# FireflyRenderEngine/GPUPathTracer

Hardware: AMD Instinct MI355X
Metric: Mrays/s (path segments = closest-hit queries, device-counted) at 1080p, 8 bounces, 1024 spp (higher is better)
Workload: dtype f32; 1 GPU; C2 wahoo.obj+cube.obj Cornell box (5184 triangles, 6 planes), 1920x1080, 8 bounces, 1024 spp, camera=inside, trace=bvh, seed 1234; scene=c2, rays_per_frame=11019120206, rays_untraversed=2123366400, rays_cut_last=721266356, primary_hits_kept_between_frames=False, partition=1080-row strips round-robin over 1 rank(s), gather=none

## Files before the change

gpupathtracer_amd/csrc/ff_api.cpp:

```cpp
#include <algorithm>
#include <chrono>
#include <cmath>
#include <cstdio>
#include <cstdlib>
#include <cstring>
#include <new>
#include <vector>

#include <hip/hip_runtime.h>
#include <hip/hip_gl_interop.h>

#include "ff_state.h"

using namespace ff;

namespace {

void free_scene(FfState* s)
{
    s->primary_valid = s->last_key_valid = false;
    if (s->d_geoms) (void)hipFree(s->d_geoms);
    if (s->d_tris) (void)hipFree(s->d_tris);
    if (s->d_normals) (void)hipFree(s->d_normals);
    if (s->d_uvs) (void)hipFree(s->d_uvs);
    if (s->d_nodes) (void)hipFree(s->d_nodes);
    if (s->d_nodes4) (void)hipFree(s->d_nodes4);
    s->top_count = s->top_depth = 0;
    s->num_scan = 0;
    if (s->d_parent) (void)hipFree(s->d_parent);
    if (s->d_role) (void)hipFree(s->d_role);
    s->d_nodes4 = nullptr;
    s->num_nodes4 = s->max_depth4 = 0;
    s->scene_block_threads = s->lds_cap = 0;
    s->d_geoms = nullptr;
    s->d_tris = nullptr;
    s->d_normals = nullptr;
    s->d_uvs = nullptr;
    s->d_nodes = nullptr;
    s->d_parent = nullptr;
    s->d_role = nullptr;
    s->h_geoms.clear();
    s->slots.clear();
    s->node_capacity = 0;
    s->has_scene = false;
    s->num_geoms = s->num_nodes = s->max_depth = 0;
    s->num_tris = 0;
}

hipError_t scene_alloc(FfState* s, void** ptr, size_t bytes)
{
    if (s->alloc_countdown >= 0 && s->alloc_countdown-- == 0) {
        *ptr = nullptr;
        return hipErrorOutOfMemory;
    }
    return hipMalloc(ptr, bytes);
}

}

namespace ff {

int ensure_bytes(void** ptr, size_t* cap, size_t need)
{
    if (*cap >= need && *ptr) return FF_OK;
    if (*ptr) (void)hipFree(*ptr);
    *ptr = nullptr;
    *cap = 0;
    hipError_t e = hipMalloc(ptr, need);
    if (e != hipSuccess) return fail(e == hipErrorOutOfMemory ? FF_ERR_OOM : FF_ERR_HIP, "hipMalloc(%zu) failed: %s", need, hipGetErrorString(e));
    *cap = need;
    return FF_OK;
}

int map_pbo(FfState* s, size_t need_bytes, void** out_ptr)
{
    size_t nbytes = 0;
    FF_HIP(hipGraphicsMapResources(1, &s->pbo_resource, s->stream));
    hipError_t e = hipGraphicsResourceGetMappedPointer(out_ptr, &nbytes, s->pbo_resource);
    if (e == hipSuccess && nbytes < need_bytes) e = hipErrorInvalidValue;
    if (e == hipSuccess) return FF_OK;
    const int st = fail(FF_ERR_HIP, "mapping the pixel buffer failed: %s", hipGetErrorString(e));
    (void)hipGraphicsUnmapResources(1, &s->pbo_resource, s->stream);
    return st;
}

int unmap_pbo(FfState* s, int status)
{
    const hipError_t ue = hipGraphicsUnmapResources(1, &s->pbo_resource, s->stream);
    if (status == FF_OK && ue != hipSuccess) return fail(FF_ERR_HIP, "hipGraphicsUnmapResources failed: %s", hipGetErrorString(ue));
    return status;
}

}

namespace {

int check_params(const FfRenderParams* p)
{
    if (!p) return fail(FF_ERR_INVALID_ARG, "render params are null");
    if (p->width <= 0 || p->height <= 0) return fail(FF_ERR_INVALID_ARG, "image size %dx%d is invalid", p->width, p->height);
    if (p->width > 65535 || p->height > 65535) return fail(FF_ERR_INVALID_ARG, "image size %dx%d exceeds 65535 per side", p->width, p->height);
    if (p->bounces < 1 || p->bounces > 255) return fail(FF_ERR_INVALID_ARG, "bounces must be in 1..255 (got %d)", p->bounces);
    if (p->spp < 1 || p->spp >= (1 << 24)) return fail(FF_ERR_INVALID_ARG, "spp must be in 1..2^24-1 (got %d)", p->spp);
    if (p->trace_mode != FF_TRACE_BRUTE_FORCE && p->trace_mode != FF_TRACE_BVH) return fail(FF_ERR_INVALID_ARG, "unknown trace_mode %d", p->trace_mode);
    if (p->shade_mode != FF_SHADE_NORMAL_DEBUG && p->shade_mode != FF_SHADE_DIFFUSE_PATH && p->shade_mode != FF_SHADE_DIFFUSE_PATH_SMOOTH &&
        p->shade_mode != FF_SHADE_DIFFUSE_PATH_NEE) return fail(FF_ERR_INVALID_ARG, "unknown shade_mode %d", p->shade_mode);
    if (p->grid_mode != FF_GRID_FULL && p->grid_mode != FF_GRID_REFERENCE_FLOOR) return fail(FF_ERR_INVALID_ARG, "unknown grid_mode %d", p->grid_mode);
    if (p->spp_per_launch < 0) return fail(FF_ERR_INVALID_ARG, "spp_per_launch must be >= 0");
    return FF_OK;
}

}

extern "C" int ff_check_render_params(const FfRenderParams* params)
{
    clear_error();
    return check_params(params);
}

namespace ff {

int check_render_call(const FfState* s, const FfCamera* camera, const FfRenderParams* params, const char* who)
{
    if (!s) return fail(FF_ERR_INVALID_ARG, "%s: state is null", who);
    if (!camera) return fail(FF_ERR_INVALID_ARG, "%s: camera is null", who);
    const int st = check_params(params);
    if (st != FF_OK) return st;
    if (!s->has_scene) return fail(FF_ERR_NO_SCENE, "%s: no scene uploaded", who);
    return FF_OK;
}

}

namespace {

int lds_records(const FfState* s) { return s->num_geoms > kMaxLdsRecords ? 0 : s->num_geoms; }

int bvh_block_threads(const FfState* s, int preferred, int stack_levels)
{
    const int sizes[3] = { 1024, 768, 512 };
    for (int b : sizes) {
        if (b > preferred) continue;
        if (bvh_lds_bytes(0, stack_levels, b, lds_records(s)) + (s->use_pool ? pool_lds_bytes(b) : 0) <= (size_t)kLdsBudgetBytes) return b;
    }
    return 0;
}

int finalize_layout(FfState* s)
{
    int nodes4 = 0, depth4 = 0;
    for (size_t i = 0; i < s->slots.size(); ++i) {
        if (s->h_geoms[i].type != FF_GEOM_TRIANGLEMESH || s->slots[i].node4_count == 0) continue;
        nodes4 += s->slots[i].node4_count;
        depth4 = std::max(depth4, s->slots[i].depth4);
    }
    s->num_nodes4 = nodes4;
    s->max_depth4 = depth4;
    s->top_count = s->top_depth = 0;
    if (s->num_geoms > kChunkGeometries) {
        std::vector<BvhNode> top2;
        std::vector<Bvh4Node> top4;
        s->num_scan = s->sw.no_scan_planes ? 0 : count_scan_planes(s->h_geoms, s->num_quads);
        build_geometry_tree(s->h_geoms, top2, s->num_scan);
        s->top_depth = collapse_geometry_tree(top2, top4);
        s->top_count = (int)top4.size();
        if (top4.size() > (size_t)s->num_geoms) return fail(FF_ERR_HIP, "geometry tree of %zu nodes for %d geometries", top4.size(), s->num_geoms);
        FF_HIP(hipMemcpyAsync(s->d_nodes4 + s->node_capacity, top4.data(), top4.size() * sizeof(Bvh4Node), hipMemcpyHostToDevice, s->stream));
        FF_HIP(hipStreamSynchronize(s->stream));
    }
    build_wall_table(s->h_geoms.data(), s->sw.no_wall_table ? 0 : (s->num_geoms > kChunkGeometries ? s->num_scan : s->num_quads), s->walls, !s->sw.no_wall_pairs);
    if (s->num_geoms <= kChunkGeometries) add_mesh_boxes(s->h_geoms.data(), s->num_planes, s->num_geoms, s->walls);
    s->stack_entries = depth4 + 1 + (s->top_depth > 0 ? s->top_depth + 1 : 0);
    if (!s->setup_threshold_forced) {
        int biggest = 1;
        for (size_t i = 0; i < s->slots.size(); ++i) biggest = std::max(biggest, s->slots[i].node4_count);
        s->setup_threshold = std::max(4, std::min(24, (int)std::lround(1.5 * std::log((double)biggest) / std::log(4.0) - 0.7)));
        s->setup_threshold = std::min(32, s->setup_threshold + 2 * s->top_depth);
    }
    s->use_pool = s->sw.pool > 0 && s->num_geoms <= kChunkGeometries && nodes4 > 0;
    constexpr int kPoolStackLevels = 5;
    const int pool_levels = std::min(s->stack_entries, s->sw.pool_stack_levels > 0 ? s->sw.pool_stack_levels : kPoolStackLevels);
    s->scene_block_threads = bvh_block_threads(s, s->block_threads, s->use_pool ? pool_levels : s->stack_entries);
    if (s->use_pool && s->scene_block_threads != 1024) {
        s->use_pool = false;
        s->scene_block_threads = bvh_block_threads(s, s->block_threads, s->stack_entries);
    }
    const int block = s->scene_block_threads > 0 ? s->scene_block_threads : kBlockThreads;
    constexpr int kMinLdsStack = 4;
    const size_t reserve = s->use_pool ? pool_lds_bytes(block) : 0;
    s->stack_lds_levels = s->stack_entries;
    if (s->use_pool) {
        s->stack_lds_levels = pool_levels;
        while (s->stack_lds_levels < s->stack_entries && max_lds_nodes(s->stack_lds_levels + 1, block, lds_records(s), reserve) >= nodes4) ++s->stack_lds_levels;
    } else if (s->scene_block_threads > 0 && !s->sw.no_stack_spill) {
        const int want = nodes4 + s->top_count;
        if (want > max_lds_nodes(s->stack_entries, block, lds_records(s))) {
            int levels = s->stack_entries;
            while (levels > kMinLdsStack && max_lds_nodes(levels, block, lds_records(s)) < want) --levels;
            if (max_lds_nodes(levels, block, lds_records(s)) >= want) s->stack_lds_levels = levels;
        }
    }
    int cap = s->scene_block_threads > 0 ? std::max(0, max_lds_nodes(s->stack_lds_levels, block, lds_records(s), reserve)) : 0;
    if (s->sw.lds_node_cap >= 0) cap = std::min(cap, s->sw.lds_node_cap);
    s->lds_cap = std::min(cap, nodes4 + s->top_count);
    s->top_lds_count = std::min(s->top_count, cap);
    const int mesh_cap = cap - s->top_lds_count;
    constexpr int kSmallTree = 8;
    std::vector<int> share(s->h_geoms.size(), 0);
    int left = mesh_cap, wanting = 0;
    for (size_t i = 0; i < s->h_geoms.size(); ++i) {
        if (s->h_geoms[i].type != FF_GEOM_TRIANGLEMESH || s->slots[i].node4_count == 0) continue;
        share[i] = std::min(std::min(s->slots[i].node4_count, kSmallTree), left);
        left -= share[i];
        wanting += s->slots[i].node4_count - share[i];
    }
    const int pool = left;
    for (size_t i = 0; i < s->h_geoms.size() && wanting > 0; ++i) {
        if (s->h_geoms[i].type != FF_GEOM_TRIANGLEMESH || s->slots[i].node4_count == 0) continue;
        const int want = s->slots[i].node4_count - share[i];
        share[i] += wanting <= pool ? want : (int)((int64_t)pool * want / wanting);
    }
    int next = s->top_lds_count;
    for (size_t i = 0; i < s->h_geoms.size(); ++i) {
        GeomRecord& r = s->h_geoms[i];
        r.node4_first = 0;
        r.lds_nodes = 0;
        r.wmin[3] = 0.0f;
        if (r.type != FF_GEOM_TRIANGLEMESH || s->slots[i].node4_count == 0) continue;
        r.node4_first = s->slots[i].node_first;
        r.lds_nodes = std::min(s->slots[i].node4_count, share[i]);
        std::memcpy(&r.wmin[3], &next, sizeof(int));
        next += r.lds_nodes;
    }
    FF_HIP(hipMemcpyAsync(s->d_geoms, s->h_geoms.data(), s->h_geoms.size() * sizeof(GeomRecord), hipMemcpyHostToDevice, s->stream));
    FF_HIP(hipStreamSynchronize(s->stream));
    return FF_OK;
}

int collapse_slot(FfState* s, size_t gi, bool with_info)
{
    FfState::MeshSlot& slot = s->slots[gi];
    if (slot.node_count <= 0) return FF_OK;
    int st = FF_OK;
    if (!slot.parents_linked) {
        st = gpu_link_parents(s->stream, s->d_nodes, slot.node_first, slot.node_count, s->d_parent + slot.node_first);
        if (st != FF_OK) return st;
        slot.parents_linked = true;
    }
    Collapse4Info info;
    st = gpu_collapse_mesh(s->stream, s->scratch, s->d_nodes, slot.node_first, slot.node_count, s->d_parent + slot.node_first, s->d_nodes4, slot.node_first, s->d_role + slot.node_first,
                           with_info ? &info : nullptr);
    if (st != FF_OK) return st;
    if (with_info) {
        if (info.node_count >= (1 << 22)) return fail(FF_ERR_UNSUPPORTED, "a mesh's tree has %d 4-wide nodes; the traversal stack encodes at most %d", info.node_count, (1 << 22) - 1);
        slot.node4_count = info.node_count;
        slot.depth4 = info.depth;
    }
    return FF_OK;
}

int fill_frame_mapping(const FfState* s, KParams& k, const FfCamera* camera, int W, int H, int grid_mode, int strip_rows, int part, int num_parts,
                       int local_rows, int x0, int y0, int win_w, int num_blocks, const char* who)
{
    FfMat4 cm;
    ff_camera_ray_matrix_jittered(camera, s->jitter_x, s->jitter_y, &cm);
    std::memcpy(k.cam_c0, &cm.m[0], 16);
    std::memcpy(k.cam_c1, &cm.m[4], 16);
    std::memcpy(k.cam_c2, &cm.m[8], 16);
    std::memcpy(k.cam_c3, &cm.m[12], 16);
    k.cam_pos[0] = camera->m_position.x;
    k.cam_pos[1] = camera->m_position.y;
    k.cam_pos[2] = camera->m_position.z;
    k.far_clip = camera->m_farClip;
    k.screen_w = camera->m_screenWidth;
    k.screen_h = camera->m_screenHeight;
    k.width = W;
    k.height = H;
    k.xlim = W;
    k.ylim = H;
    if (grid_mode == FF_GRID_REFERENCE_FLOOR) {
        k.xlim = (W / 16) * 16;
        k.ylim = (H / 16) * 16;
    }
    k.strip_rows = strip_rows;
    k.part = part;
    k.num_parts = num_parts;
    k.local_rows = local_rows;
    k.x0 = x0;
    k.y0 = y0;
    k.local_width = win_w;
    k.tiles_per_row = (win_w + 7) / 8;
    const uint64_t tiles = (uint64_t)k.tiles_per_row * (uint64_t)((local_rows + 7) / 8);
    if (tiles * 64 * (uint64_t)(num_blocks + 64) >= (1ull << 31)) return fail(FF_ERR_INVALID_ARG, "%simage too large for the work queue", who);
    k.pix_items = (unsigned)(tiles * 64);
    return FF_OK;
}

void fill_scene(const FfState* s, KParams& k, bool smooth, int lds_block_threads)
{
    k.setup_threshold = s->setup_threshold;
    k.leaf_threshold = s->leaf_threshold;
    k.num_geoms = s->num_geoms;
    k.num_planes = s->num_planes;
    k.num_quads = s->num_quads;
    k.has_specular = s->has_specular ? 1 : 0;
    k.geoms = s->d_geoms;
    k.tris = s->d_tris;
    k.trinormals = smooth ? reinterpret_cast<const float4*>(s->d_normals) : nullptr;
    k.nodes4 = s->d_nodes4;
    if (s->sw.lds_fill && lds_block_threads > 0) {
        const size_t bytes = bvh_lds_bytes(s->lds_cap, s->stack_lds_levels, lds_block_threads, lds_records(s));
        k.debug_lds_words = (unsigned)std::min<size_t>(s->sw.lds_fill_words, bytes / 4);
        k.debug_lds_pattern = (unsigned)s->sw.lds_fill_pattern;
    }
    k.stack_depth = s->stack_lds_levels;
    k.stack_spill = nullptr;
    k.lds_nodes = s->lds_cap;
    k.top_first = (int)s->node_capacity;
    k.top_lds_first = 0;
    k.top_lds_count = s->top_lds_count;
    k.num_scan = s->num_scan;
    k.walls = s->walls;
}

int attach_stack_spill(FfState* s, KParams& k, int grid, int block_threads)
{
    if (s->stack_lds_levels >= s->stack_entries) return FF_OK;
    const int st = ensure_bytes((void**)&s->d_stack_spill, &s->stack_spill_bytes,
                                (size_t)(s->stack_entries - s->stack_lds_levels) * (size_t)grid * (size_t)block_threads * sizeof(int));
    if (st == FF_OK) k.stack_spill = s->d_stack_spill;
    return st;
}

void size_work_queue(const FfState* s, KParams& k, int grid, int block_threads, int tail_per_wave)
{
    k.queue_counters = std::min(kQueueCountersDefault, grid);
    if (s->sw.queue_counters > 0) k.queue_counters = std::min(std::min(kQueueCounters, grid), s->sw.queue_counters);
    const int waves_per_counter = (grid * (block_threads / 64) + k.queue_counters - 1) / k.queue_counters;
    k.queue_tail_items = (unsigned)(waves_per_counter * (s->sw.queue_tail >= 0 ? s->sw.queue_tail : tail_per_wave));
}

FfState::PrimaryKey primary_key(const KParams& k, bool smooth)
{
    FfState::PrimaryKey key;
    std::memset(&key, 0, sizeof key);
    std::memcpy(key.cam, k.cam_c0, 16 * sizeof(float));
    std::memcpy(key.cam + 16, k.cam_pos, 3 * sizeof(float));
    key.cam[19] = k.far_clip; key.cam[20] = k.screen_w; key.cam[21] = k.screen_h;
    const int dims[12] = { k.width, k.height, k.xlim, k.ylim, k.strip_rows, k.part, k.num_parts, k.local_rows, k.x0, k.y0, k.local_width, smooth ? 1 : 0 };
    std::memcpy(key.dims, dims, sizeof dims);
    key.pix_items = k.pix_items;
    return key;
}

int enqueue_prepass(FfState* s, const KParams& k, float4* hits, unsigned long long* mask_out, int frame_blocks, int grid, int block_threads)
{
    KParams kp = k;
    kp.shade_mode = kShadePrimaryPass;
    kp.primary_hits = hits;
    kp.bounces = 1;
    kp.spp_total = 1;
    kp.block_spp = 1;
    kp.num_blocks = 1;
    kp.block_begin = 0;
    kp.block_end = 1;
    kp.whole_blocks = 1u;
    kp.total_items = kp.pix_items;
    kp.tail_block = -1;
    kp.cull_mask = nullptr;
    kp.cull_mask_out = mask_out;
    kp.frame_blocks = frame_blocks;
    kp.cut_last = 0;
    kp.timeline = nullptr;
    kp.queue_chunk = 32u;
    if (s->sw.queue_chunk > 0) kp.queue_chunk = (unsigned)s->sw.queue_chunk;
    FF_HIP(launch_trace(kp, FF_TRACE_BVH, false, grid, block_threads, s->stream, nullptr, false, true));
    FF_HIP(hipMemsetAsync(s->d_queue, 0, (size_t)k.queue_counters * kQueueStride * sizeof(unsigned), s->stream));
    return FF_OK;
}

}

namespace ff {

int render_enqueue(FfState* s, const FfCamera* camera, const FfRenderParams* prm, int strip_rows, int part, int num_parts, int local_rows,
                   unsigned char* rgb8_dev, float* radiance_dev, int x0, int y0, int win_w)
{
    const int W = prm->width, H = prm->height;
    if (win_w < 0) win_w = W;
    const size_t local_pixels = (size_t)local_rows * (size_t)win_w;
    s->stats = FfStats();
    s->pending = false;
    if (local_pixels == 0) return FF_OK;

    const bool debug = prm->shade_mode == FF_SHADE_NORMAL_DEBUG;
    const bool env = s->env_set && !debug;
    if (env && prm->shade_mode == FF_SHADE_DIFFUSE_PATH_SMOOTH)
        return fail(FF_ERR_UNSUPPORTED, "FF_SHADE_DIFFUSE_PATH_SMOOTH does not render under an environment light (ff_set_environment); "
                    "clear it or use FF_SHADE_DIFFUSE_PATH / FF_SHADE_DIFFUSE_PATH_NEE");
    const bool tex = s->tex_bound > 0 && !debug;
    if (tex && prm->shade_mode == FF_SHADE_DIFFUSE_PATH_SMOOTH)
        return fail(FF_ERR_UNSUPPORTED, "FF_SHADE_DIFFUSE_PATH_SMOOTH does not render albedo textures (ff_set_albedo_texture); "
                    "unbind them or use FF_SHADE_DIFFUSE_PATH / FF_SHADE_DIFFUSE_PATH_NEE");
    const bool glossy = s->glossy_applied > 0 && !debug;
    if (glossy && prm->shade_mode == FF_SHADE_DIFFUSE_PATH_SMOOTH)
// ... 1048 lines not shown
            if (st != FF_OK) return st;
            rgb8_dev = s->d_rgb8;
        }
    }
    if (radiance) {
        if (radiance_on_device) rad_dev = radiance;
        else {
            st = ensure_bytes((void**)&s->d_radiance, &s->radiance_bytes, pixels * 3 * sizeof(float) + 16);
            if (st != FF_OK) return st;
            rad_dev = s->d_radiance;
        }
    }
    st = render_local(s, camera, params, h, 0, 1, h, rgb8_dev, rad_dev, x0, y0, w);
    if (st != FF_OK) return st;
    if (rgb8 && !rgb8_on_device) FF_HIP(hipMemcpy(rgb8, rgb8_dev, pixels * 3, hipMemcpyDeviceToHost));
    if (radiance && !radiance_on_device) FF_HIP(hipMemcpy(radiance, rad_dev, pixels * 3 * sizeof(float), hipMemcpyDeviceToHost));
    s->stats.total_ms = std::chrono::duration<double, std::milli>(std::chrono::steady_clock::now() - t0).count();
    return FF_OK;
}

int ff_render(FfState* s, const FfCamera* camera, const FfRenderParams* params, void* rgb8, int rgb8_on_device, float* radiance,
              int radiance_on_device)
{
    const int h = params ? params->height : 1;
    return ff_render_strips(s, camera, params, h > 0 ? h : 1, 0, 1, rgb8, rgb8_on_device, radiance, radiance_on_device, nullptr);
}

int ff_deinterleave_strips(FfState* s, const void* src_dev, void* dst_dev, int width, int height, int strip_rows, int num_parts, int elem_bytes)
{
    clear_error();
    if (!s || !src_dev || !dst_dev) return fail(FF_ERR_INVALID_ARG, "ff_deinterleave_strips: null argument");
    if (width <= 0 || height <= 0 || strip_rows <= 0 || num_parts <= 0 || elem_bytes <= 0) return fail(FF_ERR_INVALID_ARG, "ff_deinterleave_strips: bad geometry");
    FF_HIP(hipSetDevice(s->device));
    FF_HIP(launch_deinterleave(src_dev, dst_dev, width, height, strip_rows, num_parts, elem_bytes, s->stream));
    FF_HIP(hipStreamSynchronize(s->stream));
    return FF_OK;
}

int ff_intersect_rays(FfState* s, const FfRay* rays, int n, FfIntersect* out, int trace_mode)
{
    clear_error();
    if (!s || !rays || !out) return fail(FF_ERR_INVALID_ARG, "ff_intersect_rays: null argument");
    if (n < 0) return fail(FF_ERR_INVALID_ARG, "ff_intersect_rays: negative count");
    if (trace_mode != FF_TRACE_BRUTE_FORCE && trace_mode != FF_TRACE_BVH) return fail(FF_ERR_INVALID_ARG, "unknown trace_mode %d", trace_mode);
    if (!s->has_scene) return fail(FF_ERR_NO_SCENE, "ff_intersect_rays: no scene uploaded");
    if (n == 0) return FF_OK;
    if (trace_mode == FF_TRACE_BVH && s->scene_block_threads == 0)
        return fail(FF_ERR_UNSUPPORTED, "ff_intersect_rays: 4-wide BVH of depth %d does not fit the LDS traversal stack; use FF_TRACE_BRUTE_FORCE or a host-built tree", s->max_depth4);
    FF_HIP(hipSetDevice(s->device));
    FfRay* d_rays = nullptr;
    FfIntersect* d_out = nullptr;
    FF_HIP(hipMalloc((void**)&d_rays, (size_t)n * sizeof(FfRay)));
    hipError_t e = hipMalloc((void**)&d_out, (size_t)n * sizeof(FfIntersect));
    if (e != hipSuccess) {
        (void)hipFree(d_rays);
        return fail(FF_ERR_HIP, "hipMalloc failed: %s", hipGetErrorString(e));
    }
    RayBatchParams p;
    p.rays = d_rays;
    p.out = d_out;
    p.n = n;
    p.num_geoms = s->num_geoms;
    p.num_planes = s->num_planes;
    p.num_quads = s->num_quads;
    p.geoms = s->d_geoms;
    p.tris = s->d_tris;
    p.nodes4 = s->d_nodes4;
    p.stack_depth = s->stack_lds_levels;
    p.stack_spill = nullptr;
    if (trace_mode == FF_TRACE_BVH && s->stack_lds_levels < s->stack_entries) {
        const size_t threads = (size_t)((n + kBlockThreads - 1) / kBlockThreads) * (size_t)kBlockThreads;
        const int sst = ensure_bytes((void**)&s->d_stack_spill, &s->stack_spill_bytes, (size_t)(s->stack_entries - s->stack_lds_levels) * threads * sizeof(int));
        if (sst != FF_OK) {
            (void)hipFree(d_rays);
            (void)hipFree(d_out);
            return sst;
        }
        p.stack_spill = s->d_stack_spill;
    }
    p.top_first = (int)s->node_capacity;
    p.top_lds_first = 0;
    p.top_lds_count = s->top_lds_count;
    p.num_scan = s->num_scan;
    p.walls = s->walls;
    p.guard_hits = s->d_counters;
    e = hipMemsetAsync(s->d_counters, 0, sizeof(unsigned long long), s->stream);
    p.lds_nodes = s->lds_cap;
    if (e == hipSuccess) e = hipMemcpy(d_rays, rays, (size_t)n * sizeof(FfRay), hipMemcpyHostToDevice);
    if (e == hipSuccess) e = launch_ray_batch(p, trace_mode, s->stream);
    if (e == hipSuccess) e = hipStreamSynchronize(s->stream);
    unsigned long long cut = 0;
    if (e == hipSuccess) e = hipMemcpy(&cut, s->d_counters, sizeof cut, hipMemcpyDeviceToHost);
    if (e == hipSuccess) e = hipMemcpy(out, d_out, (size_t)n * sizeof(FfIntersect), hipMemcpyDeviceToHost);
    (void)hipFree(d_rays);
    (void)hipFree(d_out);
    if (e != hipSuccess) return fail(FF_ERR_HIP, "ff_intersect_rays failed: %s", hipGetErrorString(e));
    if (cut != 0) return fail(FF_ERR_HIP, "ff_intersect_rays: the traversal loop guard cut %llu queries short (a malformed or absurdly deep tree)", cut);
    return FF_OK;
}


int ff_register_gl_pbo(FfState* s, unsigned int pbo, int width, int height)
{
    clear_error();
    if (!s) return fail(FF_ERR_INVALID_ARG, "ff_register_gl_pbo: state is null");
    if (width <= 0 || height <= 0) return fail(FF_ERR_INVALID_ARG, "ff_register_gl_pbo: bad size");
    (void)hipSetDevice(s->device);
    if (s->pbo_resource) {
        (void)hipGraphicsUnregisterResource(s->pbo_resource);
        s->pbo_resource = nullptr;
    }
    hipGraphicsResource* res = nullptr;
    hipError_t e = hipGraphicsGLRegisterBuffer(&res, (GLuint)pbo, hipGraphicsRegisterFlagsWriteDiscard);
    if (e != hipSuccess || !res) {
        (void)hipGetLastError();
        return fail(FF_ERR_GL_UNAVAILABLE, "hipGraphicsGLRegisterBuffer(%u) failed: %s (is a GL context current on this thread?)", pbo, hipGetErrorString(e));
    }
    s->pbo_resource = res;
    s->pbo_width = width;
    s->pbo_height = height;
    return FF_OK;
}

int ff_unregister_gl_pbo(FfState* s)
{
    clear_error();
    if (!s) return fail(FF_ERR_INVALID_ARG, "ff_unregister_gl_pbo: state is null");
    if (!s->pbo_resource) return FF_OK;
    (void)hipSetDevice(s->device);
    hipError_t e = hipGraphicsUnregisterResource(s->pbo_resource);
    s->pbo_resource = nullptr;
    if (e != hipSuccess) return fail(FF_ERR_HIP, "hipGraphicsUnregisterResource failed: %s", hipGetErrorString(e));
    return FF_OK;
}

int ff_render_to_pbo(FfState* s, const FfCamera* camera, const FfRenderParams* params)
{
    clear_error();
    const auto t0 = std::chrono::steady_clock::now();
    if (s && !s->pbo_resource) return fail(FF_ERR_GL_UNAVAILABLE, "ff_render_to_pbo: no pixel buffer registered");
    int st = check_render_call(s, camera, params, "ff_render_to_pbo");
    if (st != FF_OK) return st;
    if (params->width != s->pbo_width || params->height != s->pbo_height)
        return fail(FF_ERR_INVALID_ARG, "ff_render_to_pbo: params are %dx%d but the registered buffer is %dx%d", params->width, params->height, s->pbo_width, s->pbo_height);
    FF_HIP(hipSetDevice(s->device));
    void* dptr = nullptr;
    st = map_pbo(s, (size_t)params->width * (size_t)params->height * 3, &dptr);
    if (st == FF_OK) {
        st = render_local(s, camera, params, params->height, 0, 1, params->height, (unsigned char*)dptr, nullptr);
        st = unmap_pbo(s, st);
    }
    s->stats.total_ms = std::chrono::duration<double, std::milli>(std::chrono::steady_clock::now() - t0).count();
    return st;
}


namespace {

int progressive_frame(FfState* s, const FfCamera* camera, const FfRenderParams* params, int frame_index, unsigned char* rgb8_dev, float* mean_dev)
{
    if (frame_index < 0) return fail(FF_ERR_INVALID_ARG, "ff_render_progressive: frame index %d", frame_index);
    if (frame_index > 0 && (params->width != s->accum_width || params->height != s->accum_height || frame_index != s->accum_frames))
        return fail(FF_ERR_INVALID_ARG, "ff_render_progressive: frame %d does not continue the running sequence (%d frames of %dx%d); restart with frame 0",
                    frame_index, s->accum_frames, s->accum_width, s->accum_height);
    const size_t values = (size_t)params->width * (size_t)params->height * 3;
    int st = ensure_bytes((void**)&s->d_frame, &s->frame_bytes, values * sizeof(float) + 16);
    if (st == FF_OK) st = ensure_bytes((void**)&s->d_accum, &s->accum_bytes, values * sizeof(float) + 16);
// ... 133 lines not shown
```

gpupathtracer_amd/csrc/ff_internal.h:

```cpp
#pragma once

#include <cstdarg>
#include <cstdint>
#include <string>
#include <vector>

#include "../../include/firefly/ff_api.h"
#include "ff_texture.h"

namespace ff {

int fail(int status, const char* fmt, ...) __attribute__((format(printf, 2, 3)));
void clear_error();


struct TriRecord {
    float v0[3];
    int32_t orig_index;
    float e1[3];
    float cull_margin;
    float e2[3];
    int32_t pad1;
};
static_assert(sizeof(TriRecord) == 48, "48-byte triangle record");

struct TriNormals {
    float n0[3], pad0;
    float n1[3], pad1;
    float n2[3], pad2;
};
static_assert(sizeof(TriNormals) == 48, "48-byte vertex-normal record");

struct BvhNode {
    float lmin[3];
    int32_t left;
    float lmax[3];
    int32_t right;
    float rmin[3];
    int32_t pad0;
    float rmax[3];
    int32_t pad1;
};
static_assert(sizeof(BvhNode) == 64, "64-byte BVH node");

struct Bvh4Node {
    float mn[3][4];
    float mx[3][4];
    int32_t link[4];
};
static_assert(sizeof(Bvh4Node) == 112, "112-byte 4-wide BVH node");
constexpr int32_t kEmptyLink = 0x7fffffff;

struct GeomRecord {
    float inv_c0[4], inv_c1[4], inv_c2[4], inv_c3[4];
    float mod_c0[4], mod_c1[4], mod_c2[4], mod_c3[4];
    float nrm_c0[4], nrm_c1[4], nrm_c2[4];
    float plane_n[4];
    float albedo[4];
    float emission[4];
    float wmin[4], wmax[4];
    int32_t type;
    int32_t bxdf_type;
    int32_t tri_first;
    int32_t tri_count;
    int32_t bvh_root;
    int32_t orig_index;
    int32_t node4_first;
    int32_t lds_nodes;
};
static_assert(sizeof(GeomRecord) == 16 * 16 + 32, "GeomRecord layout");

constexpr int kMaxWalls = 16;
struct Wall {
    float c;
    float cu, hu;
    float cv, hv;
    int geom;
    int hi_geom1;
    float hi_c;
};
static_assert(sizeof(Wall) == 32, "32-byte wall");
struct WallTable {
    int count[3];
    unsigned mask;
    float margin_s;
    float graze;
    int num_boxes;
    int pad;
    Wall w[kMaxWalls];
    struct MeshBox {
        float mn[3];
        int geom;
        float mx[3];
        int pad;
    } box[32];
};

void build_wall_table(const struct GeomRecord* geoms, int limit, WallTable& out, bool pairing = true);
void add_mesh_boxes(const struct GeomRecord* geoms, int first, int n, WallTable& out);

struct CompiledScene {
    std::vector<GeomRecord> geoms;
    std::vector<TriRecord> tris;
    std::vector<TriNormals> normals;
    std::vector<TriUVs> uvs;
    std::vector<BvhNode> nodes;
    int max_depth = 0;
    uint64_t total_tris = 0;
};

struct BvhBuildParams {
    int max_leaf_tris = 2;
    int device_leaf_tris = 2;
    int max_depth = 30;
    int bins = 64;
    float c_trav = 1.2f;
    int opt_passes = 1;
    int opt_max_tris = 1 << 18;
};

BvhBuildParams default_bvh_params();

int build_mesh_bvh(const FfTriangle* triangles, int count, const BvhBuildParams& params, std::vector<BvhNode>& nodes,
                   std::vector<TriRecord>& tris, int* out_depth, std::vector<TriNormals>* normals = nullptr, std::vector<TriUVs>* uvs = nullptr);

int compile_scene(const FfGeometry* geoms, int n, const BvhBuildParams& params, CompiledScene& out, bool build_bvh = true);

int build_geometry_tree(const std::vector<GeomRecord>& geoms, std::vector<BvhNode>& nodes, int first);
constexpr int kMaxScanPlanes = 8;
int count_scan_planes(const std::vector<GeomRecord>& geoms, int num_quads);

constexpr int32_t kGeomLeafBit = 0x40000000;
int collapse_geometry_tree(const std::vector<BvhNode>& binary, std::vector<Bvh4Node>& out);

void set_world_box(GeomRecord& r, const float omn[3], const float omx[3]);

}
```

gpupathtracer_amd/csrc/ff_kernels.h:

```cpp
#pragma once

#include <hip/hip_runtime.h>

#include "ff_internal.h"

namespace ff {

constexpr int kBlockThreads = 512;
constexpr int kBlockThreadsMax = 1024;
constexpr int kLdsBudgetBytes = 160 * 1024;
constexpr int kMaxLdsRecords = 128;
constexpr int kChunkGeometries = 32;
constexpr int kBruteBatchTris = 1024;

struct KParams {
    float cam_c0[4], cam_c1[4], cam_c2[4], cam_c3[4];
    float cam_pos[3];
    float far_clip;
    float screen_w, screen_h;
    int width, height;
    int xlim, ylim;
    int strip_rows, part, num_parts, local_rows;
    int x0, y0, local_width;
    unsigned whole_blocks;
    unsigned total_items;
    unsigned queue_chunk;
    unsigned queue_tail_items;
    unsigned pix_items;
    int tiles_per_row;
    int bounces, spp_total, block_spp, block_begin, block_end, num_blocks;
    unsigned key;
    int shade_mode;
    int setup_threshold, leaf_threshold;
    int num_geoms;
    int num_planes;
    int num_quads;
    int has_specular;
    const GeomRecord* geoms;
    const TriRecord* tris;
    const float4* trinormals;
    int num_scan;
    const Bvh4Node* nodes4;
    int top_first, top_lds_first, top_lds_count;
    int lds_nodes;
    int stack_depth;
    int* stack_spill;
    float4* blocksums;
    unsigned char* rgb8;
    float* radiance;
    unsigned* queue;
    int queue_counters;
    int tail_block;
    int tail_groups;
    int tail_start[17];
    int tail_samples_in_block;
    unsigned tail_first_item;
    float4* tail_samples;
    unsigned long long* counters;
    unsigned debug_lds_words, debug_lds_pattern;
    const unsigned long long* cull_mask;
    unsigned long long* cull_mask_out;
    int frame_blocks;
    float4* primary_hits;
    int reuse_quorum;
    unsigned emitter_mask;
    int cut_last;
    float scene_min[3], scene_max[3];
    WallTable walls;
    float4* park;
    int pool_quorum, pool_quorum_min, pool_refill, pool_slice, pool_leave, pool_batch_min;
    unsigned* timeline;
    unsigned timeline_ticks;
    float4* start_records;
    int start_bounces;
};
constexpr int kRaySlots = 30, kRaySlotFirst = 2, kRaySlotStride = 16;
constexpr int kAnsweredWord = kRaySlotStride * kRaySlotFirst + 1;
constexpr int kCutShortWord = kRaySlotStride * kRaySlotFirst + 3;
constexpr int kCulledPixelsWord = kRaySlotStride * kRaySlotFirst + 2;
constexpr int kCounterWords = 512;
constexpr int kTimelineBuckets = 1024;
constexpr int kQueueCounters = 64;
constexpr int kQueueCountersDefault = 16;
constexpr int kQueueStride = 1024;
constexpr int kShadePrimaryPass = 100;
constexpr int kQueueStripe = 64;
constexpr int kQueueTailWord = 64;

struct RayBatchParams {
    const FfRay* rays;
    FfIntersect* out;
    int n;
    int num_geoms;
    int num_planes;
    int num_quads;
    const GeomRecord* geoms;
    const TriRecord* tris;
    const Bvh4Node* nodes4;
    int top_first, top_lds_first, top_lds_count;
    int lds_nodes;
    int stack_depth;
    int* stack_spill;
    int num_scan;
    WallTable walls;
    unsigned long long* guard_hits;
};

constexpr unsigned kNeeKeySelect = 0x6A09E667u;
constexpr unsigned kNeeKeyPoint = 0xBB67AE85u;
struct NeeParams {
    KParams k;
    const float4* lights;
    int num_lights;
    const float* light_pdf;
    unsigned items;
    const float4* env_texels;
    const float2* env_alias;
    const float* env_z;
    int env_w, env_h;
    float env_rotation;
    float p_env;
    float p_area;
    const TexBinding* tex_bind;
    const TexDesc* tex_desc;
    const TriUVs* uvs;
    const float* glossy_alpha;
    int cam_active, cam_box;
    float cam_lens_radius, cam_focus;
    float cam_fwd[3], cam_right[3], cam_up[3];
};
constexpr unsigned kEnvKeyChoose = 0x3C6EF372u;
constexpr unsigned kCameraKeyPixel = 0xA54FF53Au;
constexpr unsigned kCameraKeyLens = 0x510E527Fu;

size_t bvh_lds_bytes(int lds_nodes, int stack_depth, int block_threads, int num_geoms);
int max_lds_nodes(int stack_depth, int block_threads, int num_geoms, size_t reserve = 0);
size_t pool_lds_bytes(int block_threads);

hipError_t launch_trace(const KParams& p, int trace_mode, bool collect_stats, int grid_blocks, int block_threads, hipStream_t stream,
                        const char** kernel_name = nullptr, bool pool = false, bool prepass = false, bool start = false);
hipError_t launch_combine(const KParams& p, hipStream_t stream);
hipError_t launch_cull_mask(const KParams& p, unsigned long long* mask, hipStream_t stream);
hipError_t launch_accumulate(float* sum, const float* frame, float* mean, unsigned char* rgb8, size_t values, int first_frame, float inv_frames,
                             hipStream_t stream);
hipError_t launch_ray_batch(const RayBatchParams& p, int trace_mode, hipStream_t stream);
hipError_t launch_ieee_check(unsigned long long* mismatches2, hipStream_t stream);
hipError_t launch_deinterleave(const void* src, void* dst, int width, int height, int strip_rows, int num_parts, int elem_bytes,
                               hipStream_t stream);
hipError_t launch_unpack_strips(const void* src, unsigned char* rgb8, float* radiance, int width, int height, int strip_rows, int num_parts,
                                hipStream_t stream);
hipError_t launch_nee(const NeeParams& np, int trace_mode, bool env, bool tex, bool glossy, int grid_blocks, hipStream_t stream, const char** kernel_name);
hipError_t prepare_kernels();

}
```

gpupathtracer_amd/csrc/ff_kernels.hip:

```cpp
#include "ff_kernels.h"

namespace ff {
namespace {

constexpr float kInf = __builtin_huge_valf();
constexpr float kTriEpsilon = 0.000001f;
constexpr float kPlaneDenomMin = 1e-7f;
constexpr float kRayEps = 1.0e-4f;
constexpr int kWave = 64;

struct Ray {
    float ox, oy, oz, dx, dy, dz;
};

struct Best {
    float dist;
    int geom;
    int rec;
    float px, py, pz;
    float cx, cy, cz;
};

struct BestId {
    float dist;
// ... 174 lines not shown
}

__device__ __forceinline__ float plane_t(float nx, float ny, float nz, const Ray& r)
{
    const float denom = dot3(nx, ny, nz, r.dx, r.dy, r.dz);
    if (!(fabsf(denom) >= kPlaneDenomMin)) return -1.0f;
    const float t = dot3(-r.ox, -r.oy, -r.oz, nx, ny, nz) / denom;
    const float Px = r.ox + t * r.dx, Py = r.oy + t * r.dy;
    if (!(Px >= -0.5f && Px <= 0.5f && Py >= -0.5f && Py <= 0.5f)) return -1.0f;
    return t > 0.0f ? t : -1.0f;
}

__device__ __forceinline__ float sphere_t(float rad, const Ray& r)
{
    const float b = dot3(r.ox, r.oy, r.oz, r.dx, r.dy, r.dz);
    const float c = dot3(r.ox, r.oy, r.oz, r.ox, r.oy, r.oz) - rad * rad;
    const float disc = b * b - c;
    if (!(disc >= 0.0f)) return -1.0f;
    const float sq = ieee_sqrt(disc);
    float t = -b - sq;
    if (!(t > kTriEpsilon)) {
        t = -b + sq;
        if (!(t > kTriEpsilon)) return -1.0f;
    }
    return t;
}

__device__ __forceinline__ void sphere_normal(float rad, const Ray& r, float t, float& nx, float& ny, float& nz)
{
    const float inv = ieee_rcp(rad);
    nx = (r.ox + r.dx * t) * inv;
    ny = (r.oy + r.dy * t) * inv;
    nz = (r.oz + r.dz * t) * inv;
}

__device__ __forceinline__ void fill_sphere_normal(const GeomRecord* __restrict__ geoms, const Ray& wr, Best& best)
{
    if (best.geom < 0 || geoms[best.geom].type != FF_GEOM_SPHERE) return;
    const GeomRecord& G = geoms[best.geom];
    Ray osr;
    float len;
    object_space_ray(G, wr, osr, len);
    const float t = sphere_t(G.plane_n[3], osr);
    sphere_normal(G.plane_n[3], osr, t, best.cx, best.cy, best.cz);
}

__device__ __forceinline__ void fill_smooth_normal(const GeomRecord* __restrict__ geoms, const TriRecord* __restrict__ tris,
                                                   const float4* __restrict__ trinormals, const Ray& wr, Best& best)
{
    if (!trinormals || best.geom < 0 || best.rec < 0) return;
    Ray osr;
    float len;
    object_space_ray(geoms[best.geom], wr, osr, len);
    const float4* tp = reinterpret_cast<const float4*>(tris) + (size_t)best.rec * 3;
    smooth_normal(tp[0], tp[1], tp[2], trinormals + (size_t)best.rec * 3, osr, best.cx, best.cy, best.cz);
}

extern __shared__ uint4 ff_smem[];

constexpr int kGeomVec4 = (int)(sizeof(GeomRecord) / 16);
constexpr int kNodeVec4 = (int)(sizeof(Bvh4Node) / 16);
constexpr int kDone = 0x7fffffff;
constexpr int kMeshDone = 0x7ffffffe;
constexpr int kGeomLeaf = 0x40000000;
constexpr int kPackedEntry = 0x40000000;
constexpr unsigned kItemPixelMask = 0x1FFFFFFu;
constexpr int kItemBlockShift = 25;
constexpr unsigned kItemTail = 0x80000000u;
constexpr int kStartClassShift = 24;
constexpr unsigned kStartGeomMask = 0xFFFFFFu;
constexpr unsigned kStartGoesOn = 1u;
constexpr unsigned kStartEnds = 2u;
constexpr unsigned kStartGeneral = 3u;

struct LdsBase {
    int node_cap;
    int stack_base;
    int stack_slot;
    int stack_depth;
    int* spill;
    int block;
    int stride;
    int geom_base;
    int num_quads;
    const float4* smooth_normals;
    const float4* geoms_g;
    int top_first, top_lds_first, top_lds_count;
    int num_scan;
};
template <int BIG>
struct LdsT : LdsBase {
    static constexpr bool big = BIG != 0;
    static constexpr bool records_lds = BIG != 2;
};

template <int BIG = 0>
__device__ __forceinline__ LdsT<BIG> make_lds(int node_cap, int stack_depth, int block, int tid, int num_quads, const float4* smooth_normals = nullptr,
                                              const GeomRecord* geoms = nullptr, int top_first = 0, int top_lds_first = 0, int top_lds_count = 0,
                                              int num_scan = 0, int* spill = nullptr)
{
    LdsT<BIG> L;
    L.spill = spill;
    L.block = block;
    L.num_scan = num_scan;
    L.geoms_g = reinterpret_cast<const float4*>(geoms);
    L.top_first = top_first;
    L.top_lds_first = top_lds_first;
    L.top_lds_count = top_lds_count;
    L.num_quads = num_quads;
    L.smooth_normals = smooth_normals;
    L.node_cap = node_cap;
    L.stride = block;
    L.stack_base = node_cap * (kNodeVec4 * 4) + tid;
    L.stack_slot = tid;
    L.stack_depth = stack_depth;
    L.geom_base = node_cap * kNodeVec4 + (stack_depth * block) / 4;
    return L;
}

template <class LDS>
__device__ __forceinline__ void stage_scene(const LDS& L, const uint4* __restrict__ nodes4, const GeomRecord* __restrict__ geoms, int num_geoms,
                                            int num_planes, int tid, int block)
{
    for (int g = num_planes; g < num_geoms; ++g) {
        const int count = geoms[g].lds_nodes;
        if (count <= 0) continue;
        const int base = __float_as_int(geoms[g].wmin[3]);
        const uint4* src = nodes4 + (size_t)geoms[g].node4_first * kNodeVec4;
        for (int i = tid; i < count * kNodeVec4; i += block) {
            const int j = i / kNodeVec4, k = i - j * kNodeVec4;
            ff_smem[k * L.node_cap + base + j] = src[i];
        }
    }
    if constexpr (LDS::big) {
        const uint4* src = nodes4 + (size_t)L.top_first * kNodeVec4;
        for (int i = tid; i < L.top_lds_count * kNodeVec4; i += block) {
            const int j = i / kNodeVec4, k = i - j * kNodeVec4;
            ff_smem[k * L.node_cap + L.top_lds_first + j] = src[i];
        }
    }
    if constexpr (LDS::records_lds) {
        const uint4* gsrc = reinterpret_cast<const uint4*>(geoms);
        for (int i = tid; i < num_geoms * kGeomVec4; i += block) ff_smem[L.geom_base + i] = gsrc[i];
    }
    __syncthreads();
}

template <class LDS>
__device__ __forceinline__ float4 lds_geom4(const LDS& L, int g, int k)
{
    if constexpr (!LDS::records_lds) return L.geoms_g[(size_t)g * kGeomVec4 + k];
    return reinterpret_cast<const float4*>(ff_smem)[L.geom_base + g * kGeomVec4 + k];
}
template <class LDS>
__device__ __forceinline__ int4 lds_geom_i4(const LDS& L, int g, int k)
{
    if constexpr (!LDS::records_lds) return reinterpret_cast<const int4*>(L.geoms_g)[(size_t)g * kGeomVec4 + k];
    return reinterpret_cast<const int4*>(ff_smem)[L.geom_base + g * kGeomVec4 + k];
}
template <class LDS>
__device__ __forceinline__ void stack_push(const LDS& L, int sp, int v)
{
    if (__builtin_expect(sp < L.stack_depth, 1)) reinterpret_cast<int*>(ff_smem)[L.stack_base + sp * L.stride] = v;
    else L.spill[((size_t)(sp - L.stack_depth) * gridDim.x + blockIdx.x) * (size_t)L.block + (size_t)L.stack_slot] = v;
}
template <class LDS>
__device__ __forceinline__ int stack_pop(const LDS& L, int sp)
{
    int v;
    if (__builtin_expect(sp < L.stack_depth, 1)) {
        v = reinterpret_cast<const int*>(ff_smem)[L.stack_base + sp * L.stride];
        asm volatile("" : "+v"(v));
    } else {
        v = L.spill[((size_t)(sp - L.stack_depth) * gridDim.x + blockIdx.x) * (size_t)L.block + (size_t)L.stack_slot];
        asm volatile("" : "+v"(v));
    }
    return v;
}

template <class LDS>
__device__ __forceinline__ void object_space_ray_lds(const LDS& L, int g, const Ray& r, Ray& o, float& len)
{
    const float4 c0 = lds_geom4(L, g, 0), c1 = lds_geom4(L, g, 1), c2 = lds_geom4(L, g, 2), c3 = lds_geom4(L, g, 3);
    o.ox = (c0.x * r.ox + c1.x * r.oy) + (c2.x * r.oz + c3.x);
    o.oy = (c0.y * r.ox + c1.y * r.oy) + (c2.y * r.oz + c3.y);
    o.oz = (c0.z * r.ox + c1.z * r.oy) + (c2.z * r.oz + c3.z);
    const float tx = (c0.x * r.dx + c1.x * r.dy) + (c2.x * r.dz + c0.w);
    const float ty = (c0.y * r.dx + c1.y * r.dy) + (c2.y * r.dz + c1.w);
    const float tz = (c0.z * r.dx + c1.z * r.dy) + (c2.z * r.dz + c2.w);
    const float dd = (tx * tx + ty * ty) + tz * tz;
    len = ieee_sqrt(dd);
    const float inv = ieee_rcp(len);
    o.dx = tx * inv;
    o.dy = ty * inv;
    o.dz = tz * inv;
}

struct WorldSlab {
    float ix, iy, iz, ox, oy, oz;
    float inv_len;
};

__device__ __forceinline__ float safe_rcp(float d)
{
    const float s = fabsf(d) < 1e-30f ? copysignf(1e-30f, d) : d;
    return __builtin_amdgcn_rcpf(s);
}

__device__ __forceinline__ WorldSlab make_world_slab(const Ray& wr)
{
    WorldSlab w;
    w.ix = safe_rcp(wr.dx);
    w.iy = safe_rcp(wr.dy);
    w.iz = safe_rcp(wr.dz);
    w.ox = -wr.ox * w.ix;
    w.oy = -wr.oy * w.iy;
    w.oz = -wr.oz * w.iz;
    w.inv_len = __builtin_amdgcn_rsqf(__builtin_fmaf(wr.dx, wr.dx, __builtin_fmaf(wr.dy, wr.dy, wr.dz * wr.dz)));
    return w;
}

__device__ __forceinline__ bool slab_may_hit(float mnx, float mny, float mnz, float mxx, float mxy, float mxz, const WorldSlab& w, float limit)
{
    const float a0 = __builtin_fmaf(mnx, w.ix, w.ox), a1 = __builtin_fmaf(mxx, w.ix, w.ox);
    const float b0 = __builtin_fmaf(mny, w.iy, w.oy), b1 = __builtin_fmaf(mxy, w.iy, w.oy);
    const float c0 = __builtin_fmaf(mnz, w.iz, w.oz), c1 = __builtin_fmaf(mxz, w.iz, w.oz);
    const float bound = (limit * 1.001f + 1.0e-3f) * w.inv_len * 1.00001f;
// ... 129 lines not shown
        const float sdist = tt * wlen * __builtin_amdgcn_rcpf(len);
        if (tt > 0.0f && offer(sdist, g, -1, S.pend, S.best)) {
            HitPoint H;
            resolve_pending(L, tris, wr, S.pend, S.best, H);
            offer(sdist, g, -1, S.pend, S.best);
        }
        return;
    }
    const float4 c0 = lds_geom4(L, g, 0), c1 = lds_geom4(L, g, 1), c2 = lds_geom4(L, g, 2), c3 = lds_geom4(L, g, 3);
    const float4 pn = lds_geom4(L, g, 11);
    const float ox = __builtin_fmaf(c0.x, wr.ox, __builtin_fmaf(c1.x, wr.oy, __builtin_fmaf(c2.x, wr.oz, c3.x)));
    const float oy = __builtin_fmaf(c0.y, wr.ox, __builtin_fmaf(c1.y, wr.oy, __builtin_fmaf(c2.y, wr.oz, c3.y)));
    const float oz = __builtin_fmaf(c0.z, wr.ox, __builtin_fmaf(c1.z, wr.oy, __builtin_fmaf(c2.z, wr.oz, c3.z)));
    const float ux = __builtin_fmaf(c0.x, wr.dx, __builtin_fmaf(c1.x, wr.dy, c2.x * wr.dz));
    const float uy = __builtin_fmaf(c0.y, wr.dx, __builtin_fmaf(c1.y, wr.dy, c2.y * wr.dz));
    const float uz = __builtin_fmaf(c0.z, wr.dx, __builtin_fmaf(c1.z, wr.dy, c2.z * wr.dz));
    const float nx = pn.x, ny = pn.y, nz = pn.z;
    const float dn = __builtin_fmaf(nx, ux, __builtin_fmaf(ny, uy, nz * uz));
    const float num = -__builtin_fmaf(nx, ox, __builtin_fmaf(ny, oy, nz * oz));
    const float len2 = __builtin_fmaf(ux, ux, __builtin_fmaf(uy, uy, uz * uz));
    const float q = dn * dn, qlim = 1.0e-14f * len2;
    const float ta = num * __builtin_amdgcn_rcpf(dn);
    const float Pxa = __builtin_fmaf(ta, ux, ox), Pya = __builtin_fmaf(ta, uy, oy);
    const float omag = fabsf(ox) + fabsf(oy) + fabsf(oz);
    const float delta = 1.0e-5f * (1.0f + omag) * __builtin_fmaf(fabsf(ux) + fabsf(uy), fabsf(__builtin_amdgcn_rcpf(dn)), 1.0f);
    const float ex = fabsf(Pxa), ey = fabsf(Pya);
    const bool front_sure = ta > 0.0f && fabsf(num) > 1.0e-5f * omag * (fabsf(nx) + fabsf(ny) + fabsf(nz));
    bool hit = ex <= 0.5f - delta && ey <= 0.5f - delta && front_sure && q >= qlim * 1.01f;
    float dist = ta * wlen;
    if (!hit && ex <= 0.5f + delta && ey <= 0.5f + delta && q >= qlim * 0.99f && (front_sure || fabsf(num) <= 1.0e-5f * omag * (fabsf(nx) + fabsf(ny) + fabsf(nz)))) {
        if (STATS) cnt.plane_exact += 1;
        Ray osr;
        float len;
        object_space_ray_lds(L, g, wr, osr, len);
        const float tt = plane_t(nx, ny, nz, osr);
        hit = tt > 0.0f;
        dist = tt * wlen * __builtin_amdgcn_rcpf(len);
    }
    if (hit && offer(dist, g, -1, S.pend, S.best)) {
        HitPoint H;
        resolve_pending(L, tris, wr, S.pend, S.best, H);
        offer(dist, g, -1, S.pend, S.best);
    }
}

__device__ __forceinline__ void wall_test(const Wall& w, float ixk, float oxk, float ou, float du, float ov, float dv, float dl, float tt, bool steep,
                                          float wlen, float& best_d, int& best_g, bool& tie, unsigned& slow)
{
    const float t = __builtin_fmaf(w.c, ixk, oxk);
    const float pu = __builtin_fmaf(t, du, ou), pv = __builtin_fmaf(t, dv, ov);
    const float m = fmaxf(fabsf(pu - w.cu) - w.hu, fabsf(pv - w.cv) - w.hv);
    const bool hit = m <= -dl && t > tt && steep;
    const bool miss = m > dl || t < -tt;
    slow |= (!hit && !miss) ? 1u << w.geom : 0u;
    const float d = t * wlen;
    const bool nearer = hit && best_d > __builtin_fmaf(d, 1.0f + kRel, kAbs);
    const bool farther = d > __builtin_fmaf(best_d, 1.0f + kRel, kAbs);
    tie = tie || (hit && !nearer && !farther);
    best_d = nearer ? d : best_d;
    best_g = nearer ? w.geom : best_g;
}

__device__ __forceinline__ void wall_test_pair(const Wall& w, float ixk, float oxk, float ou, float du, float ov, float dv, float dl, float tt, bool steep,
                                               float wlen, float& best_d, int& best_g, bool& tie, unsigned& slow)
{
    const float tlo = __builtin_fmaf(w.c, ixk, oxk), thi = __builtin_fmaf(w.hi_c, ixk, oxk);
    const bool up = ixk > 0.0f;
    const float t = up ? thi : tlo, tother = up ? tlo : thi;
    const int g = up ? w.hi_geom1 - 1 : w.geom, gother = up ? w.geom : w.hi_geom1 - 1;
    slow |= !(tother < -tt) ? 1u << gother : 0u;
    const float pu = __builtin_fmaf(t, du, ou), pv = __builtin_fmaf(t, dv, ov);
    const float m = fmaxf(fabsf(pu - w.cu) - w.hu, fabsf(pv - w.cv) - w.hv);
    const bool hit = m <= -dl && t > tt && steep;
    const bool miss = m > dl || t < -tt;
    slow |= (!hit && !miss) ? 1u << g : 0u;
    const float d = t * wlen;
    const bool nearer = hit && best_d > __builtin_fmaf(d, 1.0f + kRel, kAbs);
    const bool farther = d > __builtin_fmaf(best_d, 1.0f + kRel, kAbs);
    tie = tie || (hit && !nearer && !farther);
    best_d = nearer ? d : best_d;
    best_g = nearer ? g : best_g;
}

template <bool STATS>
__device__ __forceinline__ void screen_walls(const WallTable& W, const Ray& wr, const WorldSlab& ws, float wlen, Segment& S, unsigned& slow, Counters& cnt)
{
    const int nx = W.count[0], ny = nx + W.count[1], nz = ny + W.count[2];
    if (nz == 0) return;
    if (STATS) { cnt.planes += (unsigned)nz; probe_round(cnt.wall_rounds); }
    const float D = 2.0e-5f * ((fabsf(wr.ox) + fabsf(wr.oy)) + (fabsf(wr.oz) + W.margin_s));
    const float th = 0.05f * D;
    const float ax = fabsf(wr.dx), ay = fabsf(wr.dy), az = fabsf(wr.dz);
    const float aix = fabsf(ws.ix), aiy = fabsf(ws.iy), aiz = fabsf(ws.iz);
    const float gmin = W.graze * wlen;
    float best_d = kInf;
    int best_g = -1;
    bool tie = false;
    Wall cur = W.w[0];
    int i = 0;
    {
        const float dl = D * __builtin_fmaf(fmaxf(ay, az), aix, 1.0f), tt = th * aix;
        const bool steep = ax >= gmin;
        for (; i < nx; ++i) {
            const Wall nxt = W.w[min(i + 1, kMaxWalls - 1)];
            if (cur.hi_geom1) wall_test_pair(cur, ws.ix, ws.ox, wr.oy, wr.dy, wr.oz, wr.dz, dl, tt, steep, wlen, best_d, best_g, tie, slow);
            else wall_test(cur, ws.ix, ws.ox, wr.oy, wr.dy, wr.oz, wr.dz, dl, tt, steep, wlen, best_d, best_g, tie, slow);
            cur = nxt;
        }
    }
    {
        const float dl = D * __builtin_fmaf(fmaxf(az, ax), aiy, 1.0f), tt = th * aiy;
        const bool steep = ay >= gmin;
        for (; i < ny; ++i) {
            const Wall nxt = W.w[min(i + 1, kMaxWalls - 1)];
            if (cur.hi_geom1) wall_test_pair(cur, ws.iy, ws.oy, wr.oz, wr.dz, wr.ox, wr.dx, dl, tt, steep, wlen, best_d, best_g, tie, slow);
            else wall_test(cur, ws.iy, ws.oy, wr.oz, wr.dz, wr.ox, wr.dx, dl, tt, steep, wlen, best_d, best_g, tie, slow);
            cur = nxt;
        }
    }
    {
        const float dl = D * __builtin_fmaf(fmaxf(ax, ay), aiz, 1.0f), tt = th * aiz;
        const bool steep = az >= gmin;
        for (; i < nz; ++i) {
            const Wall nxt = W.w[min(i + 1, kMaxWalls - 1)];
            if (cur.hi_geom1) wall_test_pair(cur, ws.iz, ws.oz, wr.ox, wr.dx, wr.oy, wr.dy, dl, tt, steep, wlen, best_d, best_g, tie, slow);
            else wall_test(cur, ws.iz, ws.oz, wr.ox, wr.dx, wr.oy, wr.dy, dl, tt, steep, wlen, best_d, best_g, tie, slow);
            cur = nxt;
        }
    }
    if (tie) {
        slow |= W.mask;
    } else if (best_g >= 0) {
        S.pend.dist = best_d;
        S.pend.geom = best_g;
        S.pend.rec = -1;
    }
}

__device__ __forceinline__ unsigned holds(const Segment& S)
{
    return (S.pend.geom >= 0 ? 1u << (S.pend.geom & 31) : 0u) | (S.best.geom >= 0 ? 1u << (S.best.geom & 31) : 0u);
}

template <bool STATS, class LDS>
__device__ __forceinline__ bool scan_records(const LDS& L, const WallTable& W, const GeomRecord* __restrict__ geoms, int num_geoms, int num_planes,
                                           const TriRecord* __restrict__ tris, const Ray& wr, Segment& S, Counters& cnt, bool cut, unsigned emitters)
{
    const int prim_end = num_planes;
    const float wlen = __builtin_amdgcn_rcpf(inv_length(wr));

    unsigned long long tb0 = 0, tb1 = 0, tb2 = 0;
    if (STATS) tb0 = __builtin_amdgcn_s_memtime();
    const WorldSlab ws = make_world_slab(wr);
    unsigned quads = 0u;
    screen_walls<STATS>(W, wr, ws, wlen, S, quads, cnt);
    for (int g = 0; g < prim_end; ++g) {
        if ((W.mask >> g) & 1u) continue;
        const float4 bmin = lds_geom4(L, g, 14), bmax = lds_geom4(L, g, 15);
        if (slab_may_hit(bmin.x, bmin.y, bmin.z, bmax.x, bmax.y, bmax.z, ws, kInf)) quads |= 1u << g;
    }
    if (STATS) tb1 = __builtin_amdgcn_s_memtime();
    for (int guard = 0; __ballot(quads != 0u) != 0ull && guard < 32; ++guard) {
        if (quads == 0u) continue;
        const int g = __ffs((int)quads) - 1;
        quads &= quads - 1u;
        screen_analytic<STATS>(L, g, tris, wr, wlen, S, cnt);
    }

    if (STATS) tb2 = __builtin_amdgcn_s_memtime();
    S.meshes = 0u;
    const float limit = fminf(S.best.dist, S.pend.dist);
    {
        typedef unsigned box_words __attribute__((ext_vector_type(8)));
        static_assert(sizeof(WallTable::MeshBox) == 32, "one box, one load");
        box_words cur = *reinterpret_cast<const box_words*>(&W.box[0]);
        for (int i = 0; i < W.num_boxes; ++i) {
            const box_words nxt = *reinterpret_cast<const box_words*>(&W.box[min(i + 1, 31)]);
            S.meshes |= slab_may_hit(__uint_as_float(cur.s0), __uint_as_float(cur.s1), __uint_as_float(cur.s2), __uint_as_float(cur.s4), __uint_as_float(cur.s5),
                                     __uint_as_float(cur.s6), ws, limit) ? 1u << cur.s3 : 0u;
            cur = nxt;
        }
    }
    const bool over = cut && (holds(S) & emitters) == 0u;
    if (over) S.meshes = 0u;
    if (STATS && S.meshes == 0u) cnt.no_mesh += 1;
    if (STATS) {
        const unsigned long long tb3 = __builtin_amdgcn_s_memtime();
        if ((threadIdx.x & 63) == __ffsll((long long)__ballot(true)) - 1) { cnt.t_b1 += tb1 - tb0; cnt.t_b2 += tb2 - tb1; cnt.t_b3 += tb3 - tb2; }
    }
    return over;
}

template <class LDS>
__device__ __forceinline__ void enter_top(const LDS& L, const Ray& wr, Segment& S);

template <bool STATS, class LDS>
__device__ __forceinline__ void scan_walls(const LDS& L, const WallTable& W, const TriRecord* __restrict__ tris, const Ray& wr, Segment& S, Counters& cnt)
{
    const float wlen = __builtin_amdgcn_rcpf(inv_length(wr));
    const WorldSlab ws = make_world_slab(wr);
    unsigned prims = 0u;
    screen_walls<STATS>(W, wr, ws, wlen, S, prims, cnt);
    for (int g = 0; g < L.num_scan; ++g) {
        if ((W.mask >> g) & 1u) continue;
        const float4 bmin = lds_geom4(L, g, 14), bmax = lds_geom4(L, g, 15);
        if (slab_may_hit(bmin.x, bmin.y, bmin.z, bmax.x, bmax.y, bmax.z, ws, kInf)) prims |= 1u << g;
    }
    for (int guard = 0; __ballot(prims != 0u) != 0ull && guard < 8; ++guard) {
        if (prims == 0u) continue;
        const int g = __ffs((int)prims) - 1;
        prims &= prims - 1u;
        screen_analytic<STATS>(L, g, tris, wr, wlen, S, cnt);
    }
}

template <bool STATS, class LDS>
__device__ __forceinline__ bool begin_segment(const LDS& L, const WallTable& W, const GeomRecord* __restrict__ geoms, int num_geoms, int num_planes,
                                              const TriRecord* __restrict__ tris, const Ray& wr, Segment& S, Counters& cnt, bool cut = false,
                                              unsigned emitters = 0u)
{
    S.best.dist = kInf;
    S.best.geom = -1;
    S.best.rec = -1;
    S.pend.dist = kInf;
    S.pend.geom = -1;
    S.pend.rec = -1;
    S.cur = kDone;
    S.sp = 0;
    S.tl_sp = 0;
    S.mesh = -1;
    S.resume = 0;
    if constexpr (LDS::big) {
        S.meshes = 0u;
        if (L.num_scan > 0) scan_walls<STATS>(L, W, tris, wr, S, cnt);
        const bool over = cut && (holds(S) & emitters) == 0u;
        if (over) return true;
        enter_top(L, wr, S);
        S.cur = 0;
        return false;
    }
    return scan_records<STATS>(L, W, geoms, num_geoms, num_planes, tris, wr, S, cnt, cut, emitters);
}

__device__ __forceinline__ void refresh_tbound(Segment& S)
{
    S.tbound = (fminf(S.best.dist, S.pend.dist) * 1.001f + 1.0e-3f) * S.scale * 1.00001f;
}

#define FF_PIN4(q) asm volatile("" : "+v"((q).x), "+v"((q).y), "+v"((q).z), "+v"((q).w))

__device__ __forceinline__ int select_slot(const uint4 q, int c)
{
    const unsigned m0 = (unsigned)((c << 31) >> 31), m1 = (unsigned)((c << 30) >> 31);
    const unsigned lo = (q.y & m0) | (q.x & ~m0), hi = (q.w & m0) | (q.z & ~m0);
    return (int)((hi & m1) | (lo & ~m1));
}

template <class LDS>
__device__ __forceinline__ void pop_entry(const LDS& L, const uint4* __restrict__ nodes4, Segment& S, int e)
{
    if (e >= 0 && (e & kPackedEntry) != 0) {
        const int node = (e >> 8) & 0x3FFFFF;
        uint4 lk;
        if ((unsigned)node < (unsigned)S.lds_count) {
            lk = ff_smem[S.lds_first + node + 6 * L.node_cap];
            FF_PIN4(lk);
        } else {
            lk = *reinterpret_cast<const uint4*>(reinterpret_cast<const char*>(nodes4) + ((unsigned)(S.node_base + node) * (unsigned)(kNodeVec4 * 16) + 96u));
            FF_PIN4(lk);
        }
        S.cur = select_slot(lk, (e >> 2) & 3);
        const int rest = (e & 3) == 2 ? select_slot(lk, (e >> 4) & 3)
                                      : ((e & ~0xFF) | (((e >> 4) & 0xF) << 2) | 2);
        stack_push(L, S.sp - 1, rest);
    } else {
        S.cur = e;
        --S.sp;
    }
}

template <class LDS>
__device__ __forceinline__ void pop_subtree(const LDS& L, const uint4* __restrict__ nodes4, Segment& S)
{
    if (S.sp == (LDS::big ? S.tl_sp : 0)) {
        S.cur = LDS::big && S.mesh >= 0 ? kMeshDone : kDone;
        return;
    }
    pop_entry(L, nodes4, S, stack_pop(L, S.sp - 1));
}

template <class LDS>
__device__ __forceinline__ void set_box_planes(const LDS& L, Segment& S)
{
    const int q = L.node_cap * 16;
    S.bnx = S.ix < 0.0f ? 3 * q : 0;
    S.bny = S.iy < 0.0f ? 4 * q : q;
    S.bnz = S.iz < 0.0f ? 5 * q : 2 * q;
    S.bfx = 3 * q - S.bnx;
    S.bfy = 5 * q - S.bny;
    S.bfz = 7 * q - S.bnz;
// ... 220 lines not shown
        if ((threadIdx.x & 63) == __ffsll((long long)__ballot(true)) - 1) cnt.t_l3 += tl3 - tl0;
    }
}

template <class LDS>
__device__ __forceinline__ void finish_segment(const LDS& L, const TriRecord* __restrict__ tris, const Ray& wr, Segment& S, Best& best)
{
    bool have_point = false;
    HitPoint H = { 0.f, 0.f, 0.f, 0.f, 0.f, 1.f };
    if (S.pend.geom >= 0) have_point = resolve_pending(L, tris, wr, S.pend, S.best, H);
    if (!have_point && S.best.geom >= 0) {
        float dist;
        int orig_tri;
        exact_hit(L, tris, wr, S.best.geom, S.best.rec, dist, H, orig_tri);
    }
    best.dist = S.best.dist;
    best.geom = S.best.geom;
    best.rec = S.best.rec;
    best.px = H.wx; best.py = H.wy; best.pz = H.wz;
    best.cx = H.cx; best.cy = H.cy; best.cz = H.cz;
}

__device__ __forceinline__ bool segment_done(const Segment& S) { return S.cur == kDone && S.meshes == 0u && S.resume == 0; }

template <bool STATS, class LDS>
__device__ __forceinline__ void traverse_budget(const LDS& L, const TriRecord* __restrict__ tris, const uint4* __restrict__ nodes4, const Ray& wr,
                                                Segment& S, Counters& cnt, int budget, int leaf_threshold, int num_planes = 0)
{
    const int limit = budget > 0 ? budget : kLoopGuard;
    int rounds = 0, guard = 0;
    for (;;) {
        unsigned long long ta = 0, tb = 0, tc = 0, td = 0;
        if (STATS) ta = __builtin_amdgcn_s_memtime();
        if constexpr (LDS::big) {
            {
                const bool back = S.cur == kMeshDone, geom = S.cur < 0 && ((~S.cur) & kGeomLeaf) != 0;
                if (__ballot(back || geom) != 0ull) {
                    if (back) leave_mesh(L, nodes4, wr, S);
                    else if (geom) geom_step<STATS>(L, num_planes, tris, nodes4, wr, S, cnt);
                }
            }
        } else {
            if (guard == 0 || budget <= 0 || __ballot(S.cur != kDone) == 0ull)
                while (S.cur == kDone && S.meshes != 0u) start_next_mesh(L, wr, S);
        }
        if (STATS) tb = __builtin_amdgcn_s_memtime();
        if (__ballot(S.cur != kDone) == 0ull) break;
        bool leaves_due = true;
        for (;;) {
            const bool inner = (unsigned)S.cur < (unsigned)kMeshDone;
            if (__ballot(inner) == 0ull) break;
            const bool tri_leaf = S.cur < 0 && !(LDS::big && ((~S.cur) & kGeomLeaf) != 0);
            if (__popcll(__ballot(tri_leaf)) >= leaf_threshold) break;
            if (rounds >= limit) break;
            if constexpr (LDS::big) {
                if (__popcll(__ballot(S.cur == kMeshDone || (S.cur < 0 && !tri_leaf))) >= leaf_threshold) {
                    leaves_due = false;
                    break;
                }
            }
            ++rounds;
            if (inner) inner_step<STATS>(L, nodes4, S, cnt);
        }
        if (STATS) tc = __builtin_amdgcn_s_memtime();
        if (leaves_due && S.cur < 0 && !(LDS::big && ((~S.cur) & kGeomLeaf) != 0)) leaf_step<STATS>(L, tris, nodes4, wr, S, cnt);
        if (STATS) {
            td = __builtin_amdgcn_s_memtime();
            if ((threadIdx.x & 63) == __ffsll((long long)__ballot(true)) - 1) { cnt.t_start += tb - ta; cnt.t_inner += tc - tb; cnt.t_leaf += td - tc; }
        }
        if (__ballot(S.resume > 0 && S.pend.geom >= 0) != 0ull) {
            if (S.resume > 0 && S.pend.geom >= 0) {
                HitPoint H;
                resolve_pending(L, tris, wr, S.pend, S.best, H);
                refresh_tbound(S);
            }
        }
        if (rounds >= limit) break;
        if (++guard > kLoopGuard) break;
    }
    if (budget <= 0 || guard > kLoopGuard) cnt.guard_hits |= __ballot(!segment_done(S));
}

template <bool STATS, class LDS>
__device__ __forceinline__ void closest_hit_deferred(const LDS& L, const WallTable& W, const GeomRecord* __restrict__ geoms, int num_geoms, int num_planes,
                                                     const TriRecord* __restrict__ tris, const uint4* __restrict__ nodes4, const Ray& wr,
                                                     Best& best, Counters& cnt)
{
    Segment S;
    if (STATS) probe_round(cnt.segment_rounds);
    begin_segment<STATS>(L, W, geoms, num_geoms, num_planes, tris, wr, S, cnt);
    traverse_budget<STATS>(L, tris, nodes4, wr, S, cnt, 0, 64, num_planes);
    finish_segment(L, tris, wr, S, best);
    cnt.rays += 1;
}

template <bool STATS>
__device__ __forceinline__ void closest_hit_brute(const GeomRecord* __restrict__ geoms, int num_geoms, const TriRecord* __restrict__ tris,
                                                  float4* batch, bool live, const Ray& wr, Best& best, Counters& cnt,
                                                  const float4* __restrict__ trinormals = nullptr)
{
    best.dist = kInf;
    best.geom = -1;
    best.rec = -1;
    best.px = best.py = best.pz = 0.0f;
    best.cx = best.cy = 0.0f;
    best.cz = 1.0f;
    for (int g = 0; g < num_geoms; ++g) {
        const GeomRecord& G = geoms[g];
        Ray osr;
        float len;
        object_space_ray(G, wr, osr, len);
        if (G.type == FF_GEOM_TRIANGLEMESH) {
            for (int base = 0; base < G.tri_count; base += kBruteBatchTris) {
                const int nb = min(kBruteBatchTris, G.tri_count - base);
                __syncthreads();
                const float4* src = reinterpret_cast<const float4*>(tris) + (size_t)(G.tri_first + base) * 3;
                for (int i = threadIdx.x; i < nb * 3; i += blockDim.x) batch[i] = src[i];
                __syncthreads();
                if (live) {
                    for (int k = 0; k < nb; ++k) {
                        const float4 a = batch[3 * k], b = batch[3 * k + 1], c = batch[3 * k + 2];
                        const float t = triangle_t(a, b, c, osr);
                        if (t > 0.0f) consider(G, g, G.tri_first + base + k, __float_as_int(a.w), t, osr, wr, geoms, tris, best);
                    }
                    if (STATS) cnt.tris += (unsigned)nb;
                }
            }
        } else if (live) {
            if (STATS) cnt.planes += 1;
            const float t = G.type == FF_GEOM_SPHERE ? sphere_t(G.plane_n[3], osr) : plane_t(G.plane_n[0], G.plane_n[1], G.plane_n[2], osr);
            if (t > 0.0f) consider(G, g, -1, -1, t, osr, wr, geoms, tris, best);
        }
    }
    if (live) {
        fill_object_normal(geoms, tris, best);
        fill_sphere_normal(geoms, wr, best);
        fill_smooth_normal(geoms, tris, trinormals, wr, best);
        cnt.rays += 1;
    }
}


struct MaterialRef {
    const GeomRecord* global;
    int geom_base;
    int g;
};

__device__ __forceinline__ float4 mat_f4(const MaterialRef& M, int k)
{
    if (M.global) return reinterpret_cast<const float4*>(M.global)[k];
    return reinterpret_cast<const float4*>(ff_smem)[M.geom_base + M.g * kGeomVec4 + k];
}
__device__ __forceinline__ int mat_bxdf(const MaterialRef& M)
{
    if (M.global) return M.global->bxdf_type;
    return reinterpret_cast<const int4*>(ff_smem)[M.geom_base + M.g * kGeomVec4 + 16].y;
}

__device__ __forceinline__ void world_normal(const MaterialRef& M, const Best& best, bool unit_object_normal, float& nx, float& ny, float& nz)
{
    float ox = best.cx, oy = best.cy, oz = best.cz;
    if (best.rec >= 0 && unit_object_normal) {
        const float inv = ieee_rcp(ieee_sqrt(dot3(ox, oy, oz, ox, oy, oz)));
        ox = ox * inv;
        oy = oy * inv;
        oz = oz * inv;
// ... 464 lines not shown
        ux = q1.x; uy = q1.y; uz = q1.z;
        ox = q0.x; oy = q0.y; oz = q0.z;
    }
    float wox, woy, woz;
    to_world_about(ux, uy, uz, wlx, wly, wlz, wox, woy, woz);
    P.ray.ox = ox;
    P.ray.oy = oy;
    P.ray.oz = oz;
    P.ray.dx = wox;
    P.ray.dy = woy;
    P.ray.dz = woz;
    ++P.b;
}

template <bool SPECULAR = true>
__device__ __forceinline__ bool shade_and_advance(const KParams& p, const Best& best, bool hit, const MaterialRef& M, Path& P)
{
    const int r = settle_hit<SPECULAR>(p, best, hit, M, P);
    if (r == kGoesOn) scatter<SPECULAR>(p, best, M, P);
    return r != kPixelDone;
}

__device__ __forceinline__ void flush_counters(const KParams& p, int lane, const Counters& cnt, bool stats)
{
    if (p.shade_mode == kShadePrimaryPass) {
        if (cnt.guard_hits != 0ull && lane == 0) atomicAdd(&p.counters[0], (unsigned long long)__popcll(cnt.guard_hits));
        return;
    }
    const unsigned long long rays = wave_sum((unsigned long long)cnt.rays);
    if (lane == 0 && rays) atomicAdd(&p.counters[kRaySlotStride * (kRaySlotFirst + (blockIdx.x * (blockDim.x / kWave) + threadIdx.x / kWave) % kRaySlots)], rays);
    if (lane == 0 && cnt.reused) atomicAdd(&p.counters[kAnsweredWord + kRaySlotStride * ((blockIdx.x * (blockDim.x / kWave) + threadIdx.x / kWave) % kRaySlots)], (unsigned long long)cnt.reused);
    if (lane == 0 && cnt.cut) atomicAdd(&p.counters[kCutShortWord + kRaySlotStride * ((blockIdx.x * (blockDim.x / kWave) + threadIdx.x / kWave) % kRaySlots)], (unsigned long long)cnt.cut);
    if (cnt.guard_hits != 0ull && lane == 0) atomicAdd(&p.counters[0], (unsigned long long)__popcll(cnt.guard_hits));
    if (stats) {
        const unsigned long long n = wave_sum((unsigned long long)cnt.nodes), t = wave_sum((unsigned long long)cnt.tris),
                                 pl = wave_sum((unsigned long long)cnt.planes);
        const unsigned long long r0 = wave_sum((unsigned long long)cnt.inner_rounds), r1 = wave_sum((unsigned long long)cnt.leaf_rounds),
                                 r2 = wave_sum((unsigned long long)cnt.tri_rounds), r3 = wave_sum((unsigned long long)cnt.plane_rounds),
                                 r4 = wave_sum((unsigned long long)cnt.segment_rounds), r5 = wave_sum((unsigned long long)cnt.no_mesh),
                                 r6 = wave_sum((unsigned long long)cnt.plane_exact), r7 = wave_sum((unsigned long long)cnt.stack_overflow),
                                 r8 = wave_sum((unsigned long long)cnt.wall_rounds);
        if (lane == 0) {
            if (n) atomicAdd(&p.counters[1], n);
            if (t) atomicAdd(&p.counters[2], t);
            if (pl) atomicAdd(&p.counters[3], pl);
            atomicAdd(&p.counters[8], r0);
            atomicAdd(&p.counters[9], r1);
            atomicAdd(&p.counters[10], r2);
            atomicAdd(&p.counters[11], r3);
            atomicAdd(&p.counters[12], r4);
            atomicAdd(&p.counters[14], r5);
            atomicAdd(&p.counters[15], r6);
            atomicAdd(&p.counters[26], r7);
            atomicAdd(&p.counters[31], r8);
        }
        {
            const unsigned long long u0 = wave_sum(cnt.t_start), u1 = wave_sum(cnt.t_inner), u2 = wave_sum(cnt.t_leaf);
            if (lane == 0) { atomicAdd(&p.counters[1 + 15], u0); atomicAdd(&p.counters[2 + 15], u1); atomicAdd(&p.counters[3 + 15], u2); }
            const unsigned long long w0 = wave_sum(cnt.t_b1), w1 = wave_sum(cnt.t_b2), w2 = wave_sum(cnt.t_b3);
            if (lane == 0) { atomicAdd(&p.counters[19], w0); atomicAdd(&p.counters[20], w1); atomicAdd(&p.counters[21], w2); }
            const unsigned long long l0 = wave_sum(cnt.t_l1), l1 = wave_sum(cnt.t_l2), l2 = wave_sum(cnt.t_l3);
            if (lane == 0) { atomicAdd(&p.counters[28], l0); atomicAdd(&p.counters[29], l1); atomicAdd(&p.counters[30], l2); }
        }
    }
}

__device__ __forceinline__ void init_path(Path& P)
{
    P.item = 0; P.send = 0; P.gxy = 0; P.s = 0; P.b = 0;
    P.pdx = P.pdy = 0.f; P.pdz = 1.f;
    P.ray = { 0.f, 0.f, 0.f, 0.f, 0.f, 1.f };
    P.bx = P.by = P.bz = 1.f;
    P.ax = P.ay = P.az = 0.f;
}


template <bool STATS, int BLOCK, bool EXTRAS, int BIG = 0, bool PREPASS = false, bool START = false>
__global__ __launch_bounds__(BLOCK) void trace_bvh_kernel(const KParams p)
{
    static_assert(!START || (!EXTRAS && BIG == 0 && !PREPASS), "start records: the diffuse small-scene kernel only");
    const int tid = threadIdx.x;
    const int lane = tid & (kWave - 1);
    const LdsT<BIG> L = make_lds<BIG>(p.lds_nodes, p.stack_depth, BLOCK, tid, EXTRAS ? p.num_quads : 0x7fffffff, EXTRAS ? p.trinormals : nullptr,
                                      p.geoms, p.top_first, p.top_lds_first, p.top_lds_count, BIG ? p.num_scan : 0, p.stack_spill);
    const uint4* nodes4 = reinterpret_cast<const uint4*>(p.nodes4);
    if (p.debug_lds_words != 0u) {
        for (unsigned i = tid; i < p.debug_lds_words; i += BLOCK) reinterpret_cast<unsigned*>(ff_smem)[i] = p.debug_lds_pattern;
        __syncthreads();
    }
    stage_scene(L, nodes4, p.geoms, p.num_geoms, p.num_planes, tid, BLOCK);

    Counters cnt = {};
    Path P;
    init_path(P);
    WaveQueue Q = make_wave_queue(p);
    Segment S;
    S.best = { kInf, -1, -1 };
    S.pend = { kInf, -1, -1 };
    S.meshes = 0u;
    S.cur = kDone; S.sp = 0; S.mesh = -1; S.resume = 0;
    S.osr = { 0.f, 0.f, 0.f, 0.f, 0.f, 1.f };
    S.ix = S.iy = S.iz = S.ox = S.oy = S.oz = 0.f;
    S.scale = 1.f;
    S.tbound = 0.f;
    S.node_base = 0; S.lds_first = 0; S.lds_count = 0; S.tl_sp = 0;
    S.bnx = S.bny = S.bnz = S.bfx = S.bfy = S.bfz = 0;
    bool active = false, exhausted = false, inflight = false;
    const bool reuse = START || (!PREPASS && p.primary_hits != nullptr);
    auto stored_hit = [&](int k) { return p.primary_hits + (size_t)k * p.pix_items + ((unsigned)P.item & kItemPixelMask); };
    unsigned long long tphase[5] = { 0, 0, 0, 0, 0 };
    const unsigned long long wave_t0 = STATS ? wall_clock64() : 0ull;
    unsigned long long epoch = 0ull;
    if (STATS && p.timeline) {
        if (lane == 0) {
            const unsigned long long seen = atomicCAS(&p.counters[27], 0ull, wave_t0);
            epoch = seen ? seen : wave_t0;
        }
        epoch = __shfl(epoch, 0);
    }
    unsigned* const tl_row = STATS && p.timeline ? p.timeline + (size_t)(blockIdx.x * (BLOCK / kWave) + tid / kWave) * kTimelineBuckets : nullptr;
    int tl_bucket = 0;
    unsigned tl_count = 0u;
    for (;;) {
        unsigned long long t0 = 0, t1 = 0, t2 = 0, t3 = 0, t4 = 0;
        if (STATS) t0 = __builtin_amdgcn_s_memtime();
        const bool setup = !inflight || segment_done(S);
        if (STATS && p.timeline) {
            const int finished = __popcll(__ballot(setup && inflight));
            if (finished) {
                const unsigned long long now = wall_clock64();
                const unsigned long long bb = now > epoch ? (now - epoch) / p.timeline_ticks : 0ull;
                const int b = bb < (unsigned long long)kTimelineBuckets ? (int)bb : kTimelineBuckets - 1;
                if (b != tl_bucket) {
                    if (lane == 0 && tl_count) tl_row[tl_bucket] += tl_count;
                    tl_bucket = b;
                    tl_count = 0u;
                }
                tl_count += (unsigned)finished;
            }
        }
        Best best;
        bool hit = false;
        bool shade_now = setup && inflight;
        if (shade_now) {
            finish_segment(L, p.tris, P.ray, S, best);
            hit = best.geom >= 0;
        }
        if (STATS) t1 = __builtin_amdgcn_s_memtime();
        if constexpr (START) {
            bool from_rec = setup && !inflight && active && P.b == 0;
            bool goes_on = false;
            MaterialRef M;
            M.global = nullptr;
            M.geom_base = L.geom_base;
            M.g = 0;
            if (shade_now) {
                M.g = best.geom;
                const int r = settle_hit<false, false>(p, best, hit, M, P);
                inflight = false;
                active = r != kPixelDone;
                goes_on = r == kGoesOn;
                from_rec = r == kNewSample;
            }
            float4 q0 = make_float4(0.f, 0.f, 0.f, 0.f), q1 = q0;
            if (from_rec) {
                const float4* rec = p.start_records + ((unsigned)P.item & kItemPixelMask);
                q0 = rec[0];
                q1 = rec[p.pix_items];
                cnt.rays += 1;
                goes_on = true;
            }
            {
                const unsigned reused_now = (unsigned)__popcll(__ballot(from_rec));
// ... 273 lines not shown
    const TriRecord* tris = static_cast<const TriRecord*>(uni_ptr(c0.x, c0.y));
    const uint4* nodes4 = static_cast<const uint4*>(uni_ptr(c0.z, c0.w));
    int* spill = static_cast<int*>(uni_ptr(c1.x, c1.y));
    const int slice = (int)uni(c1.z), leaf_threshold = (int)uni(c1.w), refill = (int)uni(c2.x), leave = (int)uni(c2.y), quorum = (int)uni(c2.z);
    const unsigned layout = uni(c2.w);
    const LdsT<0> L = make_lds<0>((int)(layout & 0xFFFFFFu), (int)(layout >> 24), BLOCK, tid, 0x7fffffff, nullptr, nullptr, 0, 0, 0, 0, spill);
    Counters cnt = {};
    PoolOccupancy occ = { 0u, 0u, 0u, 0u };
    bool stuck = false;
    Segment J;
    J.cur = kDone;
    J.resume = 0;
    J.sp = 0;
    J.mesh = 0;
    J.pend = { kInf, -1, kPendEmpty };
    J.best = { kInf, -1, -1 };
    int jslot = -1;
    bool tied = false;
    LdsT<0> Lj = L;
    bool leaving = false;
    for (int turns = 0;; ++turns) {
        if (turns > kPoolSpinLimit) { stuck = true; break; }
        const int held = __popcll(__ballot(jslot >= 0));
        if (leaving && held <= leave) {
            const bool down = jslot >= 0;
            if (down) ff_smem[Q.job_base + 2 * BLOCK + jslot] = job_state_quarter(J, 0u);
            pool_push(Q, lane, jslot, down);
            break;
        }
        if (!leaving && (kWave - held >= refill || held == 0) && (held == 0 || uni(pool_waiting(Q)) != 0u)) {
            const int got = pool_pop(Q, lane, jslot < 0, stuck);
            if (got >= 0) {
                jslot = got;
                Lj.stack_base = L.node_cap * (kNodeVec4 * 4) + got;
                Lj.stack_slot = got;
                job_load<BLOCK>(Q, Lj, got, J);
            }
        }
        if (__ballot(stuck) != 0ull) { stuck = true; break; }
        if (__ballot(jslot >= 0) == 0ull) break;
        pool_slice<STATS>(Lj, tris, nodes4, J, tied, cnt, slice, leaf_threshold, occ);
        const bool back = jslot >= 0 && (J.cur == kDone || tied);
        if (__ballot(back) != 0ull) {
            if (back) {
                const uint4 st = job_state_quarter(J, tied ? kJobTie : 0u);
                ff_smem[Q.job_base + 2 * BLOCK + jslot] = st;
                __builtin_amdgcn_fence(__ATOMIC_RELEASE, "workgroup");
                __hip_atomic_store(&pool_u32()[(Q.job_base + 2 * BLOCK + jslot) * 4 + 1], st.y | kJobReturned, __ATOMIC_RELAXED, __HIP_MEMORY_SCOPE_WORKGROUP);
                jslot = -1;
                tied = false;
                J.cur = kDone;
                J.resume = 0;
            }
        }
        if (!leaving) {
            bool ret2 = false;
            if (waiting) ret2 = (__hip_atomic_load(&pool_u32()[(Q.job_base + 2 * BLOCK + tid) * 4 + 1], __ATOMIC_RELAXED, __HIP_MEMORY_SCOPE_WORKGROUP) & kJobReturned) != 0u;
            leaving = __popcll(__ballot(ret2 || nojob_ready)) >= quorum;
        }
    }
    if (!STATS && lane == 0) {
        unsigned long long* t = reinterpret_cast<unsigned long long*>(&pool_u32()[Q.ctrl + 16]);
        __hip_atomic_fetch_add(&t[0], (unsigned long long)occ.inner_rounds, __ATOMIC_RELAXED, __HIP_MEMORY_SCOPE_WORKGROUP);
        __hip_atomic_fetch_add(&t[1], (unsigned long long)occ.inner_lanes, __ATOMIC_RELAXED, __HIP_MEMORY_SCOPE_WORKGROUP);
        __hip_atomic_fetch_add(&t[2], (unsigned long long)occ.leaf_rounds, __ATOMIC_RELAXED, __HIP_MEMORY_SCOPE_WORKGROUP);
        __hip_atomic_fetch_add(&t[3], (unsigned long long)occ.leaf_lanes, __ATOMIC_RELAXED, __HIP_MEMORY_SCOPE_WORKGROUP);
    }
    if (STATS && stats != nullptr) {
        stats->nodes += cnt.nodes; stats->tris += cnt.tris;
        stats->inner_rounds += cnt.inner_rounds; stats->leaf_rounds += cnt.leaf_rounds; stats->tri_rounds += cnt.tri_rounds;
        stats->stack_overflow += cnt.stack_overflow;
        stats->t_inner += cnt.t_inner; stats->t_leaf += cnt.t_leaf;
        stats->t_l1 += cnt.t_l1; stats->t_l2 += cnt.t_l2; stats->t_l3 += cnt.t_l3;
    }
    return __ballot(stuck) != 0ull;
}

template <bool STATS, int BLOCK, bool EXTRAS>
__global__ __launch_bounds__(BLOCK) void trace_pool_kernel(const KParams p)
{
    const int tid = threadIdx.x;
    const int lane = tid & (kWave - 1);
    const LdsT<0> L = make_lds<0>(p.lds_nodes, p.stack_depth, BLOCK, tid, EXTRAS ? p.num_quads : 0x7fffffff, EXTRAS ? p.trinormals : nullptr, p.geoms, 0, 0, 0,
                                  0, p.stack_spill);
    const uint4* nodes4 = reinterpret_cast<const uint4*>(p.nodes4);
    if (p.debug_lds_words != 0u) {
        for (unsigned i = tid; i < p.debug_lds_words; i += BLOCK) reinterpret_cast<unsigned*>(ff_smem)[i] = p.debug_lds_pattern;
        __syncthreads();
    }
    PoolRef Q;
    Q.job_base = L.geom_base + p.num_geoms * kGeomVec4;
    Q.ring_base = (Q.job_base + 3 * BLOCK) * 8;
    Q.ctrl = (Q.job_base + 3 * BLOCK) * 4 + kPoolRing / 2;
    for (int i = tid; i < kPoolRing / 2; i += BLOCK) pool_u32()[Q.ring_base / 2 + i] = 0xFFFFFFFFu;
    if (tid < 4) pool_u32()[Q.ctrl + tid] = 0u;
    if (tid < 16) pool_u32()[Q.ctrl + 16 + tid] = 0u;
    if (tid == 0) {
        const unsigned long long a = (unsigned long long)p.tris, b = (unsigned long long)p.nodes4, c = (unsigned long long)p.stack_spill;
        ff_smem[Q.ctrl / 4 + 1] = make_uint4((unsigned)a, (unsigned)(a >> 32), (unsigned)b, (unsigned)(b >> 32));
        ff_smem[Q.ctrl / 4 + 2] = make_uint4((unsigned)c, (unsigned)(c >> 32), (unsigned)p.pool_slice, (unsigned)p.leaf_threshold);
        ff_smem[Q.ctrl / 4 + 3] = make_uint4((unsigned)p.pool_refill, (unsigned)p.pool_leave, (unsigned)p.pool_quorum, (unsigned)p.lds_nodes | ((unsigned)p.stack_depth << 24));
    }
    ff_smem[Q.job_base + 2 * BLOCK + tid] = make_uint4((unsigned)kDone, 0u, 0u, (unsigned)kPendEmpty);
    stage_scene(L, nodes4, p.geoms, p.num_geoms, p.num_planes, tid, BLOCK);

    Counters cnt = {};
    WaveQueue WQ = make_wave_queue(p);
    auto park_slot = [&](int k, int me) { return p.park + ((size_t)k * gridDim.x + blockIdx.x) * (size_t)BLOCK + (size_t)me; };
    auto opaque = [](int v) { asm volatile("" : "+v"(v)); return v; };
    auto park_store = [&](int me, const Path& P, const BestId& obest, const Pending& opend, unsigned omeshes, unsigned rays) {
        *park_slot(0, me) = make_float4(__int_as_float(P.item), __int_as_float(P.send), __uint_as_float(P.gxy), __int_as_float(P.s));
        *park_slot(1, me) = make_float4(__int_as_float(P.b), P.pdx, P.pdy, P.pdz);
        *park_slot(2, me) = make_float4(P.ray.ox, P.ray.oy, P.ray.oz, P.ray.dx);
        *park_slot(3, me) = make_float4(P.ray.dy, P.ray.dz, P.bx, P.by);
        *park_slot(4, me) = make_float4(P.bz, P.ax, P.ay, P.az);
        *park_slot(5, me) = make_float4(obest.dist, __int_as_float(obest.geom), __int_as_float(obest.rec), opend.dist);
        *park_slot(6, me) = make_float4(__int_as_float(opend.geom), __int_as_float(opend.rec), __uint_as_float(omeshes), __uint_as_float(rays));
    };
    {
        Path P0;
        init_path(P0);
        park_store(tid, P0, BestId{ kInf, -1, -1 }, Pending{ kInf, -1, -1 }, 0u, 0u);
    }
    bool more_meshes = false;
    bool active = false, exhausted = false, inflight = false;
    bool waiting = false;
    const bool reuse = p.primary_hits != nullptr;
    unsigned long long tphase[5] = { 0, 0, 0, 0, 0 };
    const unsigned long long wave_t0 = STATS ? wall_clock64() : 0ull;
    const int quorum = p.pool_quorum, qmin = p.pool_quorum_min;
    int starved = 0;
    bool stuck = false;
    int idle_polls = 0;
    unsigned long long tw_setup = 0ull, tw_role = 0ull, tw_rest = 0ull, tw_mark = __builtin_amdgcn_s_memtime();
    unsigned n_setup = 0u, n_role = 0u;
    for (unsigned turns = 0;; ++turns) {
        if (stuck || idle_polls > kPoolSpinLimit || (FF_POOL_DEBUG && turns > (1u << 16))) {
            cnt.guard_hits |= 1ull;
            if (FF_POOL_DEBUG) {
                const unsigned long long bw = __ballot(waiting), bi = __ballot(inflight), ba = __ballot(active), be = __ballot(exhausted);
                if (lane == 0)
                    printf("pool watchdog: block %d wave %d stuck %d idle %d turns %u waiting %llx inflight %llx active %llx exhausted %llx head %u tail %u\n", (int)blockIdx.x,
                           tid / kWave, (int)stuck, idle_polls, turns, bw, bi, ba, be, pool_u32()[Q.ctrl], pool_u32()[Q.ctrl + 1]);
            }
            break;
        }
        const int me_d = opaque(tid);
        bool returned = false;
        if (waiting) returned = (__hip_atomic_load(&pool_u32()[(Q.job_base + 2 * BLOCK + me_d) * 4 + 1], __ATOMIC_RELAXED, __HIP_MEMORY_SCOPE_WORKGROUP) & kJobReturned) != 0u;
        const bool mine = returned || (!waiting && (inflight || active || !exhausted));
        const int nready = __popcll(__ballot(mine));
        const unsigned queued = (unsigned)__builtin_amdgcn_readfirstlane((int)pool_waiting(Q));
        const bool any_waiting = __ballot(waiting) != 0ull;
        bool do_setup = nready >= quorum || (nready > 0 && !any_waiting && queued == 0u);
        bool do_role = !do_setup && queued >= (unsigned)p.pool_batch_min;
        if (!do_setup && !do_role) {
            if (nready == 0 && !any_waiting && queued == 0u) break;
            if (nready >= qmin || (nready > 0 && starved >= 4)) do_setup = true;
            else if (queued > 0u && starved >= 4) do_role = true;
            else {
                ++starved;
                ++idle_polls;
                __builtin_amdgcn_s_sleep(4);
                continue;
            }
        }
        starved = 0;
        idle_polls = 0;
#ifdef FF_EXP_NO_SETUP
        if (do_setup) { active = false; exhausted = true; waiting = false; continue; }
#endif
        {
            const unsigned long long now = __builtin_amdgcn_s_memtime();
            tw_rest += now - tw_mark;
            tw_mark = now;
        }
        if (do_setup) {
            unsigned long long t0 = 0, t1 = 0, t2 = 0, t3 = 0, t4 = 0;
            if (STATS) t0 = __builtin_amdgcn_s_memtime();
            __builtin_amdgcn_fence(__ATOMIC_ACQUIRE, "workgroup");
            const int me = opaque(tid);
            Path P;
            BestId obest;
            Pending opend;
            unsigned omeshes;
            {
                const float4 a0 = *park_slot(0, me), a1 = *park_slot(1, me), a2 = *park_slot(2, me), a3 = *park_slot(3, me), a4 = *park_slot(4, me), a5 = *park_slot(5, me),
// ... 155 lines not shown
                tw_role += now - tw_mark;
                tw_mark = now;
                n_role += 1u;
            }
        }
    }
    if (STATS && lane == 0) {
        atomicAdd(&p.counters[4], tphase[0]);
        atomicAdd(&p.counters[5], tphase[1]);
        atomicAdd(&p.counters[6], tphase[2]);
        atomicAdd(&p.counters[7], tphase[3]);
        atomicAdd(&p.counters[13], tphase[4]);
        atomicMax(&p.counters[22], tphase[0] + tphase[1] + tphase[2] + tphase[3] + tphase[4]);
        atomicMax(&p.counters[24], ~(unsigned long long)wave_t0);
        atomicMax(&p.counters[25], (unsigned long long)wall_clock64());
    }
    flush_counters(p, lane, cnt, STATS);
    if (!STATS && lane == 0) {
        unsigned long long* t = reinterpret_cast<unsigned long long*>(&pool_u32()[Q.ctrl + 16]);
        __hip_atomic_fetch_add(&t[4], tw_setup, __ATOMIC_RELAXED, __HIP_MEMORY_SCOPE_WORKGROUP);
        __hip_atomic_fetch_add(&t[5], tw_role, __ATOMIC_RELAXED, __HIP_MEMORY_SCOPE_WORKGROUP);
        __hip_atomic_fetch_add(&t[6], tw_rest + (__builtin_amdgcn_s_memtime() - tw_mark), __ATOMIC_RELAXED, __HIP_MEMORY_SCOPE_WORKGROUP);
        __hip_atomic_fetch_add(&t[7], (unsigned long long)n_setup | ((unsigned long long)n_role << 32), __ATOMIC_RELAXED, __HIP_MEMORY_SCOPE_WORKGROUP);
    }
    if (!STATS) {
        __syncthreads();
        if (tid == 0) {
            const unsigned long long* t = reinterpret_cast<const unsigned long long*>(&pool_u32()[Q.ctrl + 16]);
            atomicAdd(&p.counters[8], t[0]);
            atomicAdd(&p.counters[1], t[1]);
            atomicAdd(&p.counters[9], t[2]);
            atomicAdd(&p.counters[14], t[3]);
            atomicAdd(&p.counters[16], t[4]);
            atomicAdd(&p.counters[17], t[5]);
            atomicAdd(&p.counters[18], t[6]);
            atomicAdd(&p.counters[11], t[7] & 0xFFFFFFFFull);
            atomicAdd(&p.counters[12], t[7] >> 32);
        }
    }
}


template <bool STATS>
__global__ __launch_bounds__(kBlockThreads) void trace_brute_kernel(const KParams p)
{
    const int tid = threadIdx.x;
    const int lane = tid & (kWave - 1);
    float4* batch = reinterpret_cast<float4*>(ff_smem);
    Counters cnt = {};
    Path P;
    init_path(P);
    WaveQueue Q = make_wave_queue(p);
    bool active = false, exhausted = false;
    for (;;) {
        {
            const bool need = !active && !exhausted;
            if (__ballot(need) != 0ull) {
                const bool got = acquire_pixel(p, lane, P, Q, need, cnt.rays);
                if (need) {
                    active = got;
                    exhausted = !got;
                }
            }
        }
        if (__syncthreads_or(active ? 1 : 0) == 0) break;
        Best best;
        closest_hit_brute<STATS>(p.geoms, p.num_geoms, p.tris, batch, active, P.ray, best, cnt, p.trinormals);
        if (!active) continue;
        const bool hit = best.geom >= 0;
        MaterialRef M;
        M.global = hit ? &p.geoms[best.geom] : p.geoms;
        M.geom_base = 0;
        M.g = 0;
        active = shade_and_advance(p, best, hit, M, P);
    }
    flush_counters(p, lane, cnt, STATS);
}

template <int MODE, int BIG = 0>
__global__ __launch_bounds__(kBlockThreads) void ray_batch_kernel(const RayBatchParams p)
{
    const int tid = threadIdx.x;
    const LdsT<BIG> L = make_lds<BIG>(p.lds_nodes, p.stack_depth, kBlockThreads, tid, p.num_quads, nullptr, p.geoms, p.top_first, p.top_lds_first,
                                      p.top_lds_count, BIG ? p.num_scan : 0, p.stack_spill);
    const uint4* nodes4 = reinterpret_cast<const uint4*>(p.nodes4);
    if (MODE == FF_TRACE_BVH) stage_scene(L, nodes4, p.geoms, p.num_geoms, p.num_planes, tid, kBlockThreads);
    float4* batch = reinterpret_cast<float4*>(ff_smem);
    const int i = blockIdx.x * kBlockThreads + tid;
    const bool live = i < p.n;
    Ray wr = { 0.f, 0.f, 0.f, 0.f, 0.f, 1.f };
    if (live) {
        const FfRay r = p.rays[i];
        wr.ox = r.m_origin.x; wr.oy = r.m_origin.y; wr.oz = r.m_origin.z;
        wr.dx = r.m_direction.x; wr.dy = r.m_direction.y; wr.dz = r.m_direction.z;
    }
    Best best;
    best.dist = kInf; best.geom = -1; best.rec = -1; best.px = best.py = best.pz = 0.f; best.cx = best.cy = 0.f; best.cz = 1.f;
    Counters cnt = {};
    if (MODE == FF_TRACE_BRUTE_FORCE) closest_hit_brute<false>(p.geoms, p.num_geoms, p.tris, batch, live, wr, best, cnt);
    else if (live) closest_hit_deferred<false>(L, p.walls, p.geoms, p.num_geoms, p.num_planes, p.tris, nodes4, wr, best, cnt);
    if (live && ((cnt.guard_hits >> (threadIdx.x & 63)) & 1ull) != 0ull && p.guard_hits) atomicAdd(p.guard_hits, 1ull);
    if (!live) return;
    FfIntersect out;
    out.m_intersectionPoint.x = 0.f; out.m_intersectionPoint.y = 0.f; out.m_intersectionPoint.z = 0.f;
    out.m_normal.x = 0.f; out.m_normal.y = 0.f; out.m_normal.z = 0.f;
    out.m_t = 0.f;
    out.m_hit = 0;
    out._pad[0] = out._pad[1] = out._pad[2] = 0;
    out.geometryIndex = -1;
    out.triangleIndex = -1;
    if (best.geom >= 0) {
        const GeomRecord& G = p.geoms[best.geom];
        MaterialRef M;
        M.global = &G;
        M.geom_base = L.geom_base;
        M.g = 0;
        float nx, ny, nz;
        world_normal(M, best, true, nx, ny, nz);
        out.m_intersectionPoint.x = best.px; out.m_intersectionPoint.y = best.py; out.m_intersectionPoint.z = best.pz;
        out.m_normal.x = nx; out.m_normal.y = ny; out.m_normal.z = nz;
        out.m_t = best.dist;
        out.m_hit = 1;
        out.geometryIndex = G.orig_index;
        out.triangleIndex = best.rec >= 0 ? p.tris[best.rec].orig_index : -1;
    }
    p.out[i] = out;
}

__global__ void cull_mask_kernel(const KParams p, unsigned long long* mask)
{
    const unsigned pitem = blockIdx.x * blockDim.x + threadIdx.x;
    bool culled = false;
    if (pitem < p.pix_items) {
        const int tile = (int)(pitem >> 6), in = (int)(pitem & 63u);
        const int lx = (tile % p.tiles_per_row) * 8 + (in & 7);
        const int ly = (tile / p.tiles_per_row) * 8 + (in >> 3);
        const int strip = ly / p.strip_rows;
        const int gy = p.y0 + (strip * p.num_parts + p.part) * p.strip_rows + (ly - strip * p.strip_rows);
        const int gx = p.x0 + lx;
        if (lx < p.local_width && gx < p.xlim && ly < p.local_rows && gy < p.ylim) {
            Ray r;
            primary_ray(p, (unsigned)gx | ((unsigned)gy << 16), r);
            culled = !slab_may_hit(p.scene_min[0], p.scene_min[1], p.scene_min[2], p.scene_max[0], p.scene_max[1], p.scene_max[2], make_world_slab(r), kInf);
            if (culled)
                for (int b = 0; b < p.num_blocks; ++b) p.blocksums[(size_t)pitem * p.num_blocks + b] = make_float4(0.f, 0.f, 0.f, 0.f);
        }
    }
    const unsigned long long word = __ballot(culled);
    if ((threadIdx.x & 63) == 0 && pitem < ((p.pix_items + 63u) & ~63u)) {
        mask[pitem >> 6] = word;
        if (word) atomicAdd(&p.counters[kCulledPixelsWord + kRaySlotStride * ((pitem >> 6) % kRaySlots)], (unsigned long long)__popcll(word));
    }
}

__global__ void combine_kernel(const KParams p)
{
    const int lx = blockIdx.x * blockDim.x + threadIdx.x;
    const int ly = blockIdx.y;
    if (lx >= p.local_width || ly >= p.local_rows) return;
    const int strip = ly / p.strip_rows;
    const int gy = p.y0 + (strip * p.num_parts + p.part) * p.strip_rows + (ly - strip * p.strip_rows);
    if (p.x0 + lx >= p.xlim || gy >= p.ylim) return;
    const unsigned pitem = (unsigned)(((ly >> 3) * p.tiles_per_row + (lx >> 3)) * 64 + ((ly & 7) * 8 + (lx & 7)));
    float ax = 0.f, ay = 0.f, az = 0.f;
    const bool culled = p.cull_mask != nullptr && ((p.cull_mask[pitem >> 6] >> (pitem & 63u)) & 1ull) != 0ull;
    for (int b = 0; b < (culled ? 0 : p.num_blocks); ++b) {
        float4 v;
        if (p.tail_block >= 0 && b >= p.tail_block) {
            float bx = 0.f, by = 0.f, bz = 0.f;
// ... 100 lines not shown
    const size_t local_row = (size_t)local_strip * (size_t)strip_rows + (size_t)(y - strip * strip_rows);
    const size_t stride = (size_t)gridDim.x * blockDim.x, first = (size_t)blockIdx.x * blockDim.x + threadIdx.x;
    if (radiance) {
        const float* s = reinterpret_cast<const float*>(src + base) + local_row * (size_t)width * 3;
        float* d = radiance + (size_t)y * (size_t)width * 3;
        for (size_t i = first; i < (size_t)width * 3; i += stride) d[i] = s[i];
    }
    if (rgb8) {
        const unsigned char* s = src + base + pad16(rows * (size_t)width * 12) + local_row * (size_t)width * 3;
        unsigned char* d = rgb8 + (size_t)y * (size_t)width * 3;
        for (size_t i = first; i < (size_t)width * 3; i += stride) d[i] = s[i];
    }
}


__device__ __forceinline__ float nee_u24(unsigned r) { return (float)(r >> 8) * 5.9604644775390625e-08f; }

__device__ __forceinline__ float4 env_lookup(const NeeParams& np, float dx, float dy, float dz)
{
    constexpr float kTwoPi = 6.28318530717958648f, kInvTwoPi = 0.15915494309189535f, kInvPi = 0.31830988618379067f;
    float phi = atan2f(dx, -dz) - np.env_rotation;
    if (phi < 0.f) phi = phi + kTwoPi;
    if (phi < 0.f) phi = phi + kTwoPi;
    const float theta = acosf(fminf(fmaxf(dy, -1.f), 1.f));
    const int c = min(max((int)((phi * kInvTwoPi) * (float)np.env_w), 0), np.env_w - 1);
    const int r = min(max((int)((theta * kInvPi) * (float)np.env_h), 0), np.env_h - 1);
    return np.env_texels[r * np.env_w + c];
}


template <int CAM>
__device__ __forceinline__ void nee_start_sample(const NeeParams& np, Path& P)
{
    const KParams& p = np.k;
    if (!CAM) start_sample(p, P);
    else {
        P.b = 0;
        P.bx = P.by = P.bz = 1.f;
        const CameraRays C = { p.cam_c0, p.cam_c1, p.cam_c2, p.cam_c3, p.cam_pos, p.far_clip, p.screen_w, p.screen_h,
                               np.cam_box, np.cam_lens_radius, np.cam_focus, np.cam_fwd, np.cam_right, np.cam_up };
        const unsigned gx = P.gxy & 0xFFFFu, gy = P.gxy >> 16;
        camera_sample_ray(C, (int)gx, (int)gy, gy * (unsigned)p.width + gx, (unsigned)P.s, p.key, P.ray.ox, P.ray.oy, P.ray.oz, P.ray.dx, P.ray.dy,
                          P.ray.dz);
    }
}

template <int CAM>
__device__ __forceinline__ bool nee_end_sample(const NeeParams& np, Path& P, float& Lx, float& Ly, float& Lz, float& prev_pdf)
{
    const KParams& p = np.k;
    P.ax = P.ax + Lx;
    P.ay = P.ay + Ly;
    P.az = P.az + Lz;
    Lx = Ly = Lz = 0.f;
    prev_pdf = 0.f;
    ++P.s;
    if (P.s < P.send) {
        nee_start_sample<CAM>(np, P);
        return true;
    }
    p.blocksums[(size_t)((unsigned)P.item & kItemPixelMask) * p.num_blocks + ((unsigned)P.item >> kItemBlockShift)] = make_float4(P.ax, P.ay, P.az, 0.f);
    return false;
}

__device__ __forceinline__ void to_local_about(float ux, float uy, float uz, float wx, float wy, float wz, float& lx, float& ly, float& lz)
{
    const float sign = copysignf(1.0f, uz);
    const float aa = -ieee_rcp(sign + uz);
    const float bb = (ux * uy) * aa;
    const float t0 = 1.0f + ((sign * ux) * ux) * aa, t1 = sign * bb, t2 = -sign * ux;
    const float s0 = bb, s1 = sign + (uy * uy) * aa, s2 = -uy;
    lx = dot3(t0, t1, t2, wx, wy, wz);
    ly = dot3(s0, s1, s2, wx, wy, wz);
    lz = dot3(ux, uy, uz, wx, wy, wz);
}

template <int MODE, int BIG = 0, int ENV = 0, int TEX = 0, int GLOSSY = 0, int CAM = 0>
__global__ __launch_bounds__(kBlockThreads) void nee_path_kernel(const NeeParams np)
{
    const KParams& p = np.k;
    const int tid = threadIdx.x;
    const int lane = tid & (kWave - 1);
    const LdsT<BIG> L = make_lds<BIG>(p.lds_nodes, p.stack_depth, kBlockThreads, tid, p.num_quads, nullptr, p.geoms, p.top_first, p.top_lds_first,
                                      p.top_lds_count, BIG ? p.num_scan : 0, p.stack_spill);
    const uint4* nodes4 = reinterpret_cast<const uint4*>(p.nodes4);
    if (MODE == FF_TRACE_BVH) stage_scene(L, nodes4, p.geoms, p.num_geoms, p.num_planes, tid, kBlockThreads);
    float4* batch = reinterpret_cast<float4*>(ff_smem);
    constexpr float kInvPi = 0.31830988618379067f;
    Counters cnt = {};
    Path P;
    init_path(P);
    unsigned next = blockIdx.x * kBlockThreads + tid;
    const unsigned stride = gridDim.x * kBlockThreads;
    bool active = false;
    float Lx = 0.f, Ly = 0.f, Lz = 0.f;
    float prev_pdf = 0.f;
    bool shadow = false;
    Ray sray = { 0.f, 0.f, 0.f, 0.f, 0.f, 1.f };
    int sgeom = -1, sprim = -1;
    float scx = 0.f, scy = 0.f, scz = 0.f;
    bool dead = false;
    for (;;) {
        while (!active && next < np.items) {
            const unsigned item = next;
            next += stride;
            const unsigned blk = item / p.pix_items, pitem = item - blk * p.pix_items;
            const int tile = (int)(pitem >> 6), in = (int)(pitem & 63u);
            const int lx = (tile % p.tiles_per_row) * 8 + (in & 7);
            const int ly = (tile / p.tiles_per_row) * 8 + (in >> 3);
            const int strip = ly / p.strip_rows;
            const int gy = p.y0 + (strip * p.num_parts + p.part) * p.strip_rows + (ly - strip * p.strip_rows);
            const int gx = p.x0 + lx;
            if (lx < p.local_width && gx < p.xlim && ly < p.local_rows && gy < p.ylim) {
                const int block = p.block_begin + (int)blk;
                active = true;
                P.gxy = (unsigned)gx | ((unsigned)gy << 16);
                P.item = (int)(((unsigned)block << kItemBlockShift) | pitem);
                P.s = block * p.block_spp;
                P.send = min(p.spp_total, P.s + p.block_spp);
                P.ax = P.ay = P.az = 0.f;
                if (!CAM) {
                    primary_ray(p, P.gxy, P.ray);
                    P.pdx = P.ray.dx;
                    P.pdy = P.ray.dy;
                    P.pdz = P.ray.dz;
                }
                nee_start_sample<CAM>(np, P);
                Lx = Ly = Lz = 0.f;
                prev_pdf = 0.f;
                shadow = false;
            }
        }
        Best best;
        if (MODE == FF_TRACE_BRUTE_FORCE) {
            if (__syncthreads_or(active ? 1 : 0) == 0) break;
            closest_hit_brute<false>(p.geoms, p.num_geoms, p.tris, batch, active, shadow ? sray : P.ray, best, cnt);
        } else {
            if (__ballot(active) == 0ull) break;
            if (active) closest_hit_deferred<false>(L, p.walls, p.geoms, p.num_geoms, p.num_planes, p.tris, nodes4, shadow ? sray : P.ray, best, cnt);
        }
        if (!active) continue;
        if (shadow) {
            shadow = false;
            if (best.geom == sgeom && (sprim < 0 || (best.rec >= 0 && p.tris[best.rec].orig_index == sprim))) {
                Lx = Lx + scx;
                Ly = Ly + scy;
                Lz = Lz + scz;
            }
            if (GLOSSY && dead) {
                dead = false;
                active = nee_end_sample<CAM>(np, P, Lx, Ly, Lz, prev_pdf);
            }
            continue;
        }
        const bool hit = best.geom >= 0;
        MaterialRef M;
        M.global = p.geoms + (hit ? best.geom : 0);
        M.geom_base = 0;
        M.g = 0;
        bool goes_on = false;
        float galpha = 0.f;
        if (hit) {
            const int bxdf = mat_bxdf(M);
            if (GLOSSY && bxdf == FF_BXDF_MIRROR) galpha = np.glossy_alpha[best.geom];
            if (bxdf == FF_BXDF_EMITTER) {
                const float4 emission = mat_f4(M, 13);
                float cx = P.bx * emission.x, cy = P.by * emission.y, cz = P.bz * emission.z;
                const float area_pdf = ((ENV || TEX || GLOSSY || CAM) && np.num_lights == 0) ? 0.f : np.light_pdf[best.geom];
                if (prev_pdf > 0.f && area_pdf > 0.f) {
// ... 153 lines not shown
                            const GlossyLobe gl = glossy_eval(galpha, f0.x, f0.y, f0.z, gox, goy, goz, lx, ly, cos_x);
                            const float f = (cos_x * (pl2 / (pl2 + gl.pdf * gl.pdf))) / pl;
                            scx = ((P.bx * le.x) * gl.fr) * f;
                            scy = ((P.by * le.y) * gl.fg) * f;
                            scz = ((P.bz * le.z) * gl.fb) * f;
                        } else {
                            const float pb = cos_x * kInvPi;
                            const float f = (pb * (pl2 / (pl2 + pb * pb))) / pl;
                            scx = (P.bx * le.x) * f;
                            scy = (P.by * le.y) * f;
                            scz = (P.bz * le.z) * f;
                        }
                        sgeom = g;
                        sprim = prim;
                        sray.ox = best.px + ux * kRayEps;
                        sray.oy = best.py + uy * kRayEps;
                        sray.oz = best.pz + uz * kRayEps;
                        sray.dx = wx;
                        sray.dy = wy;
                        sray.dz = wz;
                        shadow = true;
                    }
                }
            }
            if (glossy) {
                const unsigned gpix = (P.gxy >> 16) * (unsigned)p.width + (P.gxy & 0xFFFFu);
                unsigned r0, r1;
                philox2x32_10(gpix, ((unsigned)P.s << 8) | ((unsigned)P.b & 0xFFu), p.key, r0, r1);
                float lx, ly, lz;
                const GlossyLobe gl = glossy_sample(galpha, f0.x, f0.y, f0.z, gox, goy, goz, r0 >> 8, nee_u24(r1), lx, ly, lz);
                if (lz > 0.f) {
                    P.bx = P.bx * gl.wr;
                    P.by = P.by * gl.wg;
                    P.bz = P.bz * gl.wb;
                    float wox, woy, woz;
                    to_world_about(ux, uy, uz, lx, ly, lz, wox, woy, woz);
                    P.ray.ox = best.px + ux * kRayEps;
                    P.ray.oy = best.py + uy * kRayEps;
                    P.ray.oz = best.pz + uz * kRayEps;
                    P.ray.dx = wox;
                    P.ray.dy = woy;
                    P.ray.dz = woz;
                    ++P.b;
                    prev_pdf = gl.pdf;
                    continue;
                }
                if (shadow) {
                    dead = true;
                    continue;
                }
            } else {
                scatter<true>(p, best, M, P);
                prev_pdf = diffuse ? dot3(ux, uy, uz, P.ray.dx, P.ray.dy, P.ray.dz) * kInvPi : 0.f;
                continue;
            }
        }
        P.ax = P.ax + Lx;
        P.ay = P.ay + Ly;
        P.az = P.az + Lz;
        Lx = Ly = Lz = 0.f;
        prev_pdf = 0.f;
        ++P.s;
        if (P.s < P.send) {
            nee_start_sample<CAM>(np, P);
        } else {
            p.blocksums[(size_t)((unsigned)P.item & kItemPixelMask) * p.num_blocks + ((unsigned)P.item >> kItemBlockShift)] = make_float4(P.ax, P.ay, P.az, 0.f);
            active = false;
        }
    }
    flush_counters(p, lane, cnt, false);
}

}

#if defined(FF_PROBE) || defined(FF_PROBE_NEE)
namespace {
#ifdef FF_PROBE
template __global__ void FF_PROBE(const KParams);
#else
template __global__ void FF_PROBE_NEE(const NeeParams);
#endif
}
#else
size_t bvh_lds_bytes(int lds_nodes, int stack_depth, int block_threads, int num_geoms)
{
    return (size_t)lds_nodes * sizeof(Bvh4Node) + (size_t)stack_depth * (size_t)block_threads * sizeof(unsigned) +
           (size_t)num_geoms * sizeof(GeomRecord);
}

int max_lds_nodes(int stack_depth, int block_threads, int num_geoms, size_t reserve)
{
    const long avail = (long)kLdsBudgetBytes - (long)reserve - (long)stack_depth * (long)block_threads * (long)sizeof(unsigned) -
                       (long)num_geoms * (long)sizeof(GeomRecord);
    return avail > 0 ? (int)(avail / (long)sizeof(Bvh4Node)) : 0;
}

hipError_t prepare_kernels()
{
    hipError_t e;
#define FF_SET_LDS(K)                                                                                                     \
    e = hipFuncSetAttribute(reinterpret_cast<const void*>(&K), hipFuncAttributeMaxDynamicSharedMemorySize, kLdsBudgetBytes); \
    if (e != hipSuccess) return e;
    FF_SET_LDS((trace_bvh_kernel<false, 512, false>))
    FF_SET_LDS((trace_bvh_kernel<false, 512, true>))
    FF_SET_LDS((trace_bvh_kernel<true, 512, false>))
    FF_SET_LDS((trace_bvh_kernel<true, 512, true>))
    FF_SET_LDS((trace_bvh_kernel<false, 768, false>))
    FF_SET_LDS((trace_bvh_kernel<false, 768, true>))
    FF_SET_LDS((trace_bvh_kernel<true, 768, false>))
    FF_SET_LDS((trace_bvh_kernel<true, 768, true>))
    FF_SET_LDS((trace_bvh_kernel<false, 1024, false>))
    FF_SET_LDS((trace_bvh_kernel<false, 1024, true>))
    FF_SET_LDS((trace_bvh_kernel<true, 1024, false>))
    FF_SET_LDS((trace_bvh_kernel<true, 1024, true>))
    FF_SET_LDS((trace_bvh_kernel<false, 512, true, 1>))
    FF_SET_LDS((trace_bvh_kernel<true, 512, true, 1>))
    FF_SET_LDS((trace_bvh_kernel<false, 768, true, 1>))
    FF_SET_LDS((trace_bvh_kernel<true, 768, true, 1>))
    FF_SET_LDS((trace_bvh_kernel<false, 1024, true, 1>))
    FF_SET_LDS((trace_bvh_kernel<true, 1024, true, 1>))
    FF_SET_LDS((trace_bvh_kernel<false, 512, true, 2>))
    FF_SET_LDS((trace_bvh_kernel<true, 512, true, 2>))
    FF_SET_LDS((trace_bvh_kernel<false, 768, true, 2>))
    FF_SET_LDS((trace_bvh_kernel<true, 768, true, 2>))
    FF_SET_LDS((trace_bvh_kernel<false, 1024, true, 2>))
    FF_SET_LDS((trace_bvh_kernel<true, 1024, true, 2>))
    FF_SET_LDS((trace_bvh_kernel<false, 512, true, 0, true>))
    FF_SET_LDS((trace_bvh_kernel<false, 768, true, 0, true>))
    FF_SET_LDS((trace_bvh_kernel<false, 1024, true, 0, true>))
    FF_SET_LDS((trace_bvh_kernel<false, 512, true, 1, true>))
    FF_SET_LDS((trace_bvh_kernel<false, 768, true, 1, true>))
    FF_SET_LDS((trace_bvh_kernel<false, 1024, true, 1, true>))
    FF_SET_LDS((trace_bvh_kernel<false, 512, true, 2, true>))
    FF_SET_LDS((trace_bvh_kernel<false, 768, true, 2, true>))
    FF_SET_LDS((trace_bvh_kernel<false, 1024, true, 2, true>))
    FF_SET_LDS((trace_bvh_kernel<false, 512, false, 0, false, true>))
    FF_SET_LDS((trace_bvh_kernel<true, 512, false, 0, false, true>))
    FF_SET_LDS((trace_bvh_kernel<false, 768, false, 0, false, true>))
    FF_SET_LDS((trace_bvh_kernel<true, 768, false, 0, false, true>))
    FF_SET_LDS((trace_bvh_kernel<false, 1024, false, 0, false, true>))
    FF_SET_LDS((trace_bvh_kernel<true, 1024, false, 0, false, true>))
    FF_SET_LDS((trace_pool_kernel<false, 1024, false>))
    FF_SET_LDS((trace_pool_kernel<false, 1024, true>))
    FF_SET_LDS((trace_pool_kernel<true, 1024, false>))
    FF_SET_LDS((trace_pool_kernel<true, 1024, true>))
    FF_SET_LDS((ray_batch_kernel<FF_TRACE_BVH>))
    FF_SET_LDS((ray_batch_kernel<FF_TRACE_BVH, 1>))
    FF_SET_LDS((ray_batch_kernel<FF_TRACE_BVH, 2>))
    FF_SET_LDS((nee_path_kernel<FF_TRACE_BVH>))
    FF_SET_LDS((nee_path_kernel<FF_TRACE_BVH, 1>))
    FF_SET_LDS((nee_path_kernel<FF_TRACE_BVH, 2>))
    FF_SET_LDS((nee_path_kernel<FF_TRACE_BVH, 0, 1>))
    FF_SET_LDS((nee_path_kernel<FF_TRACE_BVH, 1, 1>))
    FF_SET_LDS((nee_path_kernel<FF_TRACE_BVH, 2, 1>))
    FF_SET_LDS((nee_path_kernel<FF_TRACE_BVH, 0, 0, 1>))
    FF_SET_LDS((nee_path_kernel<FF_TRACE_BVH, 1, 0, 1>))
    FF_SET_LDS((nee_path_kernel<FF_TRACE_BVH, 2, 0, 1>))
    FF_SET_LDS((nee_path_kernel<FF_TRACE_BVH, 0, 1, 1>))
    FF_SET_LDS((nee_path_kernel<FF_TRACE_BVH, 1, 1, 1>))
    FF_SET_LDS((nee_path_kernel<FF_TRACE_BVH, 2, 1, 1>))
    FF_SET_LDS((nee_path_kernel<FF_TRACE_BVH, 0, 0, 0, 1>))
    FF_SET_LDS((nee_path_kernel<FF_TRACE_BVH, 1, 0, 0, 1>))
    FF_SET_LDS((nee_path_kernel<FF_TRACE_BVH, 2, 0, 0, 1>))
    FF_SET_LDS((nee_path_kernel<FF_TRACE_BVH, 0, 0, 1, 1>))
    FF_SET_LDS((nee_path_kernel<FF_TRACE_BVH, 1, 0, 1, 1>))
    FF_SET_LDS((nee_path_kernel<FF_TRACE_BVH, 2, 0, 1, 1>))
    FF_SET_LDS((nee_path_kernel<FF_TRACE_BVH, 0, 1, 0, 1>))
    FF_SET_LDS((nee_path_kernel<FF_TRACE_BVH, 1, 1, 0, 1>))
    FF_SET_LDS((nee_path_kernel<FF_TRACE_BVH, 2, 1, 0, 1>))
    FF_SET_LDS((nee_path_kernel<FF_TRACE_BVH, 0, 1, 1, 1>))
    FF_SET_LDS((nee_path_kernel<FF_TRACE_BVH, 1, 1, 1, 1>))
    FF_SET_LDS((nee_path_kernel<FF_TRACE_BVH, 2, 1, 1, 1>))
#define FF_SET_LDS_CAM(ENV, TEX, GLOSSY) \
    FF_SET_LDS((nee_path_kernel<FF_TRACE_BVH, 0, ENV, TEX, GLOSSY, 1>)) \
    FF_SET_LDS((nee_path_kernel<FF_TRACE_BVH, 1, ENV, TEX, GLOSSY, 1>)) \
    FF_SET_LDS((nee_path_kernel<FF_TRACE_BVH, 2, ENV, TEX, GLOSSY, 1>))
    FF_SET_LDS_CAM(0, 0, 0)
    FF_SET_LDS_CAM(0, 0, 1)
    FF_SET_LDS_CAM(0, 1, 0)
    FF_SET_LDS_CAM(0, 1, 1)
    FF_SET_LDS_CAM(1, 0, 0)
    FF_SET_LDS_CAM(1, 0, 1)
    FF_SET_LDS_CAM(1, 1, 0)
    FF_SET_LDS_CAM(1, 1, 1)
#undef FF_SET_LDS_CAM
#undef FF_SET_LDS
    return hipSuccess;
}

size_t pool_lds_bytes(int block_threads) { return (size_t)block_threads * 48 + (size_t)kPoolRing * 2 + 128; }

hipError_t launch_trace(const KParams& p, int trace_mode, bool collect_stats, int grid_blocks, int block_threads, hipStream_t stream,
                        const char** kernel_name, bool pool, bool prepass, bool start)
{
    const dim3 grid(grid_blocks);
    const char* name = "";
    if (prepass) {
        const dim3 block(block_threads);
        const int big = p.num_geoms <= kChunkGeometries ? 0 : (p.num_geoms <= kMaxLdsRecords ? 1 : 2);
        const size_t lds = bvh_lds_bytes(p.lds_nodes, p.stack_depth, block_threads, big == 2 ? 0 : p.num_geoms);
#define FF_LAUNCH_PRE(B)                                                                                                  \
    do {                                                                                                                  \
        if (big == 0) hipLaunchKernelGGL((trace_bvh_kernel<false, B, true, 0, true>), grid, block, lds, stream, p);      \
        else if (big == 1) hipLaunchKernelGGL((trace_bvh_kernel<false, B, true, 1, true>), grid, block, lds, stream, p); \
        else hipLaunchKernelGGL((trace_bvh_kernel<false, B, true, 2, true>), grid, block, lds, stream, p);               \
    } while (0)
        if (block_threads == 1024) FF_LAUNCH_PRE(1024);
        else if (block_threads == 768) FF_LAUNCH_PRE(768);
        else FF_LAUNCH_PRE(512);
#undef FF_LAUNCH_PRE
        if (kernel_name) *kernel_name = "trace_bvh_kernel<false, B, true, big, true>";
        return hipGetLastError();
    }
    if (trace_mode == FF_TRACE_BVH && pool && p.num_geoms <= kChunkGeometries && block_threads == 1024) {
        const dim3 block(block_threads);
        const size_t lds = bvh_lds_bytes(p.lds_nodes, p.stack_depth, block_threads, p.num_geoms) + pool_lds_bytes(block_threads);
        const bool extras = p.num_planes > p.num_quads || p.has_specular != 0 || p.trinormals != nullptr;
#define FF_LAUNCH_POOL(B)                                                                                                 \
    do {                                                                                                                  \
        if (collect_stats) {                                                                                              \
            if (extras) { hipLaunchKernelGGL((trace_pool_kernel<true, B, true>), grid, block, lds, stream, p); name = "trace_pool_kernel<true, " #B ", true>"; } \
            else { hipLaunchKernelGGL((trace_pool_kernel<true, B, false>), grid, block, lds, stream, p); name = "trace_pool_kernel<true, " #B ", false>"; } \
        } else {                                                                                                          \
            if (extras) { hipLaunchKernelGGL((trace_pool_kernel<false, B, true>), grid, block, lds, stream, p); name = "trace_pool_kernel<false, " #B ", true>"; } \
            else { hipLaunchKernelGGL((trace_pool_kernel<false, B, false>), grid, block, lds, stream, p); name = "trace_pool_kernel<false, " #B ", false>"; } \
        }                                                                                                                 \
    } while (0)
        FF_LAUNCH_POOL(1024);
#undef FF_LAUNCH_POOL
    } else if (trace_mode == FF_TRACE_BVH) {
        const dim3 block(block_threads);
        const int big = p.num_geoms <= kChunkGeometries ? 0 : (p.num_geoms <= kMaxLdsRecords ? 1 : 2);
        const size_t lds = bvh_lds_bytes(p.lds_nodes, p.stack_depth, block_threads, big == 2 ? 0 : p.num_geoms);
        const bool spheres = p.num_planes > p.num_quads || p.has_specular != 0 || p.trinormals != nullptr;
        if (start && (big != 0 || spheres || p.start_records == nullptr)) return hipErrorInvalidValue;
#define FF_LAUNCH_BVH(B)                                                                                                  \
    do {                                                                                                                  \
        if (start) {                                                                                                      \
            if (collect_stats) { hipLaunchKernelGGL((trace_bvh_kernel<true, B, false, 0, false, true>), grid, block, lds, stream, p); name = "trace_bvh_kernel<true, " #B ", false, 0, false, true>"; } \
            else { hipLaunchKernelGGL((trace_bvh_kernel<false, B, false, 0, false, true>), grid, block, lds, stream, p); name = "trace_bvh_kernel<false, " #B ", false, 0, false, true>"; } \
        } else if (big == 1) {                                                                                                   \
            if (collect_stats) { hipLaunchKernelGGL((trace_bvh_kernel<true, B, true, 1>), grid, block, lds, stream, p); name = "trace_bvh_kernel<true, " #B ", true, 1, false>"; } \
            else { hipLaunchKernelGGL((trace_bvh_kernel<false, B, true, 1>), grid, block, lds, stream, p); name = "trace_bvh_kernel<false, " #B ", true, 1, false>"; } \
        } else if (big == 2) {                                                                                            \
            if (collect_stats) { hipLaunchKernelGGL((trace_bvh_kernel<true, B, true, 2>), grid, block, lds, stream, p); name = "trace_bvh_kernel<true, " #B ", true, 2, false>"; } \
            else { hipLaunchKernelGGL((trace_bvh_kernel<false, B, true, 2>), grid, block, lds, stream, p); name = "trace_bvh_kernel<false, " #B ", true, 2, false>"; } \
        } else if (collect_stats) {                                                                                       \
            if (spheres) { hipLaunchKernelGGL((trace_bvh_kernel<true, B, true>), grid, block, lds, stream, p); name = "trace_bvh_kernel<true, " #B ", true, 0, false>"; } \
            else { hipLaunchKernelGGL((trace_bvh_kernel<true, B, false>), grid, block, lds, stream, p); name = "trace_bvh_kernel<true, " #B ", false, 0, false>"; } \
        } else {                                                                                                          \
            if (spheres) { hipLaunchKernelGGL((trace_bvh_kernel<false, B, true>), grid, block, lds, stream, p); name = "trace_bvh_kernel<false, " #B ", true, 0, false>"; } \
            else { hipLaunchKernelGGL((trace_bvh_kernel<false, B, false>), grid, block, lds, stream, p); name = "trace_bvh_kernel<false, " #B ", false, 0, false>"; } \
        }                                                                                                                 \
    } while (0)
        if (block_threads == 1024) FF_LAUNCH_BVH(1024);
        else if (block_threads == 768) FF_LAUNCH_BVH(768);
        else FF_LAUNCH_BVH(512);
#undef FF_LAUNCH_BVH
    } else {
        const size_t lds = (size_t)kBruteBatchTris * sizeof(TriRecord);
        const dim3 block(kBlockThreads);
        if (collect_stats) hipLaunchKernelGGL((trace_brute_kernel<true>), grid, block, lds, stream, p);
        else hipLaunchKernelGGL((trace_brute_kernel<false>), grid, block, lds, stream, p);
        name = collect_stats ? "trace_brute_kernel<true>" : "trace_brute_kernel<false>";
    }
    if (kernel_name) *kernel_name = name;
    return hipGetLastError();
}

hipError_t launch_combine(const KParams& p, hipStream_t stream)
{
    if (p.local_width <= 0 || p.local_rows <= 0) return hipSuccess;
    const dim3 block(256), grid((p.local_width + 255) / 256, p.local_rows);
    hipLaunchKernelGGL(combine_kernel, grid, block, 0, stream, p);
    return hipGetLastError();
}

hipError_t launch_cull_mask(const KParams& p, unsigned long long* mask, hipStream_t stream)
{
    if (p.pix_items == 0) return hipSuccess;
    hipLaunchKernelGGL(cull_mask_kernel, dim3((p.pix_items + 255) / 256), dim3(256), 0, stream, p, mask);
    return hipGetLastError();
}

hipError_t launch_ieee_check(unsigned long long* mismatches2, hipStream_t stream)
{
    hipLaunchKernelGGL(ieee_check_kernel, dim3(256 * 8), dim3(256), 0, stream, mismatches2);
    return hipGetLastError();
}

hipError_t launch_accumulate(float* sum, const float* frame, float* mean, unsigned char* rgb8, size_t values, int first_frame, float inv_frames,
                             hipStream_t stream)
{
    if (values == 0) return hipSuccess;
    hipLaunchKernelGGL(accumulate_kernel, dim3((unsigned)((values + 255) / 256)), dim3(256), 0, stream, sum, frame, mean, rgb8, values, first_frame,
                       inv_frames);
    return hipGetLastError();
}

hipError_t launch_ray_batch(const RayBatchParams& p, int trace_mode, hipStream_t stream)
{
    if (p.n <= 0) return hipSuccess;
    const int big = p.num_geoms <= kChunkGeometries ? 0 : (p.num_geoms <= kMaxLdsRecords ? 1 : 2);
    const size_t lds = trace_mode == FF_TRACE_BVH ? bvh_lds_bytes(p.lds_nodes, p.stack_depth, kBlockThreads, big == 2 ? 0 : p.num_geoms)
                                                  : (size_t)kBruteBatchTris * sizeof(TriRecord);
    const dim3 grid((p.n + kBlockThreads - 1) / kBlockThreads), block(kBlockThreads);
    if (trace_mode == FF_TRACE_BVH && big == 1) hipLaunchKernelGGL((ray_batch_kernel<FF_TRACE_BVH, 1>), grid, block, lds, stream, p);
    else if (trace_mode == FF_TRACE_BVH && big == 2) hipLaunchKernelGGL((ray_batch_kernel<FF_TRACE_BVH, 2>), grid, block, lds, stream, p);
    else if (trace_mode == FF_TRACE_BVH) hipLaunchKernelGGL((ray_batch_kernel<FF_TRACE_BVH>), grid, block, lds, stream, p);
    else hipLaunchKernelGGL((ray_batch_kernel<FF_TRACE_BRUTE_FORCE>), grid, block, lds, stream, p);
    return hipGetLastError();
}

hipError_t launch_nee(const NeeParams& np, int trace_mode, bool env, bool tex, bool glossy, int grid_blocks, hipStream_t stream, const char** kernel_name)
{
    if (np.items == 0u) return hipSuccess;
    const KParams& p = np.k;
    const int big = p.num_geoms <= kChunkGeometries ? 0 : (p.num_geoms <= kMaxLdsRecords ? 1 : 2);
    const size_t lds = trace_mode == FF_TRACE_BVH ? bvh_lds_bytes(p.lds_nodes, p.stack_depth, kBlockThreads, big == 2 ? 0 : p.num_geoms)
                                                  : (size_t)kBruteBatchTris * sizeof(TriRecord);
    const dim3 grid(grid_blocks), block(kBlockThreads);
    const char* name;
    if (np.cam_active != 0) {
#define FF_LAUNCH_CAM(MODE, BIG, ENV, TEX, GLOSSY) \
    do { hipLaunchKernelGGL((nee_path_kernel<MODE, BIG, ENV, TEX, GLOSSY, 1>), grid, block, lds, stream, np); name = "nee_path_kernel<" #MODE ", " #BIG ", " #ENV ", " #TEX ", " #GLOSSY ", 1>"; } while (0)
#define FF_LAUNCH_CAM_MODE(ENV, TEX, GLOSSY) \
    do { \
        if (trace_mode == FF_TRACE_BVH && big == 1) FF_LAUNCH_CAM(1, 1, ENV, TEX, GLOSSY); \
        else if (trace_mode == FF_TRACE_BVH && big == 2) FF_LAUNCH_CAM(1, 2, ENV, TEX, GLOSSY); \
        else if (trace_mode == FF_TRACE_BVH) FF_LAUNCH_CAM(1, 0, ENV, TEX, GLOSSY); \
        else FF_LAUNCH_CAM(0, 0, ENV, TEX, GLOSSY); \
    } while (0)
        switch ((env ? 4 : 0) | (tex ? 2 : 0) | (glossy ? 1 : 0)) {
        case 0: FF_LAUNCH_CAM_MODE(0, 0, 0); break;
        case 1: FF_LAUNCH_CAM_MODE(0, 0, 1); break;
        case 2: FF_LAUNCH_CAM_MODE(0, 1, 0); break;
        case 3: FF_LAUNCH_CAM_MODE(0, 1, 1); break;
        case 4: FF_LAUNCH_CAM_MODE(1, 0, 0); break;
        case 5: FF_LAUNCH_CAM_MODE(1, 0, 1); break;
        case 6: FF_LAUNCH_CAM_MODE(1, 1, 0); break;
        default: FF_LAUNCH_CAM_MODE(1, 1, 1); break;
        }
#undef FF_LAUNCH_CAM_MODE
#undef FF_LAUNCH_CAM
    }
    else if (glossy) {
#define FF_LAUNCH_GLOSSY(MODE, BIG, ENV, TEX) \
    do { hipLaunchKernelGGL((nee_path_kernel<MODE, BIG, ENV, TEX, 1>), grid, block, lds, stream, np); name = "nee_path_kernel<" #MODE ", " #BIG ", " #ENV ", " #TEX ", 1>"; } while (0)
#define FF_LAUNCH_GLOSSY_MODE(ENV, TEX) \
    do { \
        if (trace_mode == FF_TRACE_BVH && big == 1) FF_LAUNCH_GLOSSY(1, 1, ENV, TEX); \
        else if (trace_mode == FF_TRACE_BVH && big == 2) FF_LAUNCH_GLOSSY(1, 2, ENV, TEX); \
        else if (trace_mode == FF_TRACE_BVH) FF_LAUNCH_GLOSSY(1, 0, ENV, TEX); \
        else FF_LAUNCH_GLOSSY(0, 0, ENV, TEX); \
    } while (0)
        if (env && tex) FF_LAUNCH_GLOSSY_MODE(1, 1);
        else if (env) FF_LAUNCH_GLOSSY_MODE(1, 0);
        else if (tex) FF_LAUNCH_GLOSSY_MODE(0, 1);
        else FF_LAUNCH_GLOSSY_MODE(0, 0);
#undef FF_LAUNCH_GLOSSY_MODE
#undef FF_LAUNCH_GLOSSY
    }
    else if (tex) {
#define FF_LAUNCH_TEX(MODE, BIG, ENV) \
    do { hipLaunchKernelGGL((nee_path_kernel<MODE, BIG, ENV, 1>), grid, block, lds, stream, np); name = "nee_path_kernel<" #MODE ", " #BIG ", " #ENV ", 1>"; } while (0)
        if (env) {
            if (trace_mode == FF_TRACE_BVH && big == 1) FF_LAUNCH_TEX(1, 1, 1);
            else if (trace_mode == FF_TRACE_BVH && big == 2) FF_LAUNCH_TEX(1, 2, 1);
            else if (trace_mode == FF_TRACE_BVH) FF_LAUNCH_TEX(1, 0, 1);
            else FF_LAUNCH_TEX(0, 0, 1);
        } else {
            if (trace_mode == FF_TRACE_BVH && big == 1) FF_LAUNCH_TEX(1, 1, 0);
            else if (trace_mode == FF_TRACE_BVH && big == 2) FF_LAUNCH_TEX(1, 2, 0);
            else if (trace_mode == FF_TRACE_BVH) FF_LAUNCH_TEX(1, 0, 0);
            else FF_LAUNCH_TEX(0, 0, 0);
        }
#undef FF_LAUNCH_TEX
    }
    else if (env) {
        if (trace_mode == FF_TRACE_BVH && big == 1) { hipLaunchKernelGGL((nee_path_kernel<FF_TRACE_BVH, 1, 1>), grid, block, lds, stream, np); name = "nee_path_kernel<1, 1, 1>"; }
        else if (trace_mode == FF_TRACE_BVH && big == 2) { hipLaunchKernelGGL((nee_path_kernel<FF_TRACE_BVH, 2, 1>), grid, block, lds, stream, np); name = "nee_path_kernel<1, 2, 1>"; }
        else if (trace_mode == FF_TRACE_BVH) { hipLaunchKernelGGL((nee_path_kernel<FF_TRACE_BVH, 0, 1>), grid, block, lds, stream, np); name = "nee_path_kernel<1, 0, 1>"; }
        else { hipLaunchKernelGGL((nee_path_kernel<FF_TRACE_BRUTE_FORCE, 0, 1>), grid, block, lds, stream, np); name = "nee_path_kernel<0, 0, 1>"; }
    }
    else if (trace_mode == FF_TRACE_BVH && big == 1) { hipLaunchKernelGGL((nee_path_kernel<FF_TRACE_BVH, 1>), grid, block, lds, stream, np); name = "nee_path_kernel<1, 1>"; }
    else if (trace_mode == FF_TRACE_BVH && big == 2) { hipLaunchKernelGGL((nee_path_kernel<FF_TRACE_BVH, 2>), grid, block, lds, stream, np); name = "nee_path_kernel<1, 2>"; }
    else if (trace_mode == FF_TRACE_BVH) { hipLaunchKernelGGL((nee_path_kernel<FF_TRACE_BVH>), grid, block, lds, stream, np); name = "nee_path_kernel<1, 0>"; }
    else { hipLaunchKernelGGL((nee_path_kernel<FF_TRACE_BRUTE_FORCE>), grid, block, lds, stream, np); name = "nee_path_kernel<0, 0>"; }
    if (kernel_name) *kernel_name = name;
    return hipGetLastError();
}

hipError_t launch_deinterleave(const void* src, void* dst, int width, int height, int strip_rows, int num_parts, int elem_bytes,
                               hipStream_t stream)
{
    if (width <= 0 || height <= 0) return hipSuccess;
    const dim3 grid(4, height), block(256);
    hipLaunchKernelGGL(deinterleave_kernel, grid, block, 0, stream, (const unsigned char*)src, (unsigned char*)dst, width, height,
                       strip_rows, num_parts, elem_bytes);
    return hipGetLastError();
}

// ... 12 lines not shown
```

gpupathtracer_amd/csrc/ff_scene.cpp:

```cpp
#include <algorithm>
#include <atomic>
#include <cfloat>
#include <cmath>
#include <cstdio>
#include <cstdlib>
#include <cstring>
#include <limits>
#include <numeric>
#include <queue>
#include <system_error>
#include <thread>

#include "ff_internal.h"
#include "ff_math.h"

namespace ff {

namespace {

struct Box {
    float mn[3], mx[3];
    void reset()
    {
        for (int k = 0; k < 3; ++k) {
// ... 783 lines not shown
        GeomRecord& r = out.geoms[i];
        std::memset(&r, 0, sizeof r);
        if (g.m_geometryType != FF_GEOM_PLANE && g.m_geometryType != FF_GEOM_TRIANGLEMESH && g.m_geometryType != FF_GEOM_SPHERE)
            return fail(FF_ERR_UNSUPPORTED, "geometry %d: type %d is not a geometry type (kernel.cu:170-173)", i, g.m_geometryType);
        if (g.m_geometryType == FF_GEOM_SPHERE && !(g.m_sphereRadius > 0.f))
            return fail(FF_ERR_INVALID_ARG, "geometry %d: sphere radius %g", i, (double)g.m_sphereRadius);
        if (!g.m_bxdf) return fail(FF_ERR_INVALID_ARG, "geometry %d: m_bxdf is null (the reference copies it unconditionally, kernel.cu:282)", i);
        const M4 inv = load(g.m_inverseModelMatrix.m), mod = load(g.m_modelMatrix.m);
        if (inv.c[0].w != 0.f || inv.c[1].w != 0.f || inv.c[2].w != 0.f || mod.c[0].w != 0.f || mod.c[1].w != 0.f || mod.c[2].w != 0.f)
            return fail(FF_ERR_UNSUPPORTED, "geometry %d: model matrix is not affine", i);
        const M4 nrm = inverse(transpose(mod));
        std::memcpy(r.inv_c0, &inv.c[0], 16); std::memcpy(r.inv_c1, &inv.c[1], 16);
        std::memcpy(r.inv_c2, &inv.c[2], 16); std::memcpy(r.inv_c3, &inv.c[3], 16);
        std::memcpy(r.mod_c0, &mod.c[0], 16); std::memcpy(r.mod_c1, &mod.c[1], 16);
        std::memcpy(r.mod_c2, &mod.c[2], 16); std::memcpy(r.mod_c3, &mod.c[3], 16);
        std::memcpy(r.nrm_c0, &nrm.c[0], 16); std::memcpy(r.nrm_c1, &nrm.c[1], 16); std::memcpy(r.nrm_c2, &nrm.c[2], 16);
        r.inv_c0[3] = inv.c[3].x * 0.0f; r.inv_c1[3] = inv.c[3].y * 0.0f; r.inv_c2[3] = inv.c[3].z * 0.0f;
        r.nrm_c0[3] = nrm.c[3].x * 0.0f; r.nrm_c1[3] = nrm.c[3].y * 0.0f; r.nrm_c2[3] = nrm.c[3].z * 0.0f;
        r.plane_n[0] = g.m_normal.x; r.plane_n[1] = g.m_normal.y; r.plane_n[2] = g.m_normal.z;
        r.plane_n[3] = g.m_geometryType == FF_GEOM_SPHERE ? g.m_sphereRadius : 0.f;
        const FfBXDF& b = *g.m_bxdf;
        const FfVec3& tint = b.m_type == FF_BXDF_MIRROR ? b.m_specularColor : b.m_albedo;
        r.albedo[0] = tint.x; r.albedo[1] = tint.y; r.albedo[2] = tint.z;
        r.emission[0] = b.m_emissiveColor.x * b.m_intensity;
        r.emission[1] = b.m_emissiveColor.y * b.m_intensity;
        r.emission[2] = b.m_emissiveColor.z * b.m_intensity;
        if (b.m_type == FF_BXDF_GLASS) {
            if (!(b.m_refractiveIndex > 0.f)) return fail(FF_ERR_INVALID_ARG, "geometry %d: glass needs a positive m_refractiveIndex", i);
            r.albedo[0] = b.m_specularColor.x; r.albedo[1] = b.m_specularColor.y; r.albedo[2] = b.m_specularColor.z;
            r.albedo[3] = b.m_refractiveIndex;
            r.emission[0] = b.m_transmittanceColor.x; r.emission[1] = b.m_transmittanceColor.y; r.emission[2] = b.m_transmittanceColor.z;
        }
        r.type = g.m_geometryType;
        r.bxdf_type = b.m_type;
        r.bvh_root = -1;
        r.orig_index = i;
        float omn[3] = { -0.5f, -0.5f, 0.f }, omx[3] = { 0.5f, 0.5f, 0.f };
        if (g.m_geometryType == FF_GEOM_SPHERE)
            for (int k = 0; k < 3; ++k) { omn[k] = -g.m_sphereRadius; omx[k] = g.m_sphereRadius; }
        if (g.m_geometryType == FF_GEOM_TRIANGLEMESH) {
            Box ob;
            ob.reset();
            const int cnt0 = g.m_triangles ? g.m_numberOfTriangles : 0;
            for (int t = 0; t < cnt0; ++t) {
                ob.grow(&g.m_triangles[t].m_v0.x);
                ob.grow(&g.m_triangles[t].m_v1.x);
                ob.grow(&g.m_triangles[t].m_v2.x);
            }
            for (int k = 0; k < 3; ++k) { omn[k] = ob.mn[k]; omx[k] = ob.mx[k]; }
        }
        set_world_box(r, omn, omx);
        if (g.m_geometryType == FF_GEOM_TRIANGLEMESH) {
            const int cnt = g.m_triangles ? g.m_numberOfTriangles : 0;
            if (cnt < 0) return fail(FF_ERR_INVALID_ARG, "geometry %d: negative triangle count", i);
            if ((uint64_t)out.tris.size() + (uint64_t)cnt >= (1ull << 28))
                return fail(FF_ERR_UNSUPPORTED, "scene exceeds 2^28 triangles");
            if ((uint64_t)out.total_tris + (uint64_t)cnt >= (1ull << 28)) return fail(FF_ERR_UNSUPPORTED, "scene exceeds 2^28 triangles");
            r.tri_first = (int)out.total_tris;
            r.tri_count = cnt;
            if (build_bvh) {
                int depth = 0;
                r.bvh_root = build_mesh_bvh(g.m_triangles, cnt, params, out.nodes, out.tris, &depth, &out.normals, &out.uvs);
                out.max_depth = std::max(out.max_depth, depth);
            }
            out.total_tris += (uint64_t)cnt;
        }
    }
    std::stable_sort(out.geoms.begin(), out.geoms.end(), [](const GeomRecord& a, const GeomRecord& b) {
        const bool pa = a.type != FF_GEOM_TRIANGLEMESH, pb = b.type != FF_GEOM_TRIANGLEMESH;
        if (pa != pb) return pa;
        if (pa) {
            if (a.type != b.type) return a.type == FF_GEOM_PLANE;
            return a.type == FF_GEOM_PLANE && box_half_area(a.wmin, a.wmax) > box_half_area(b.wmin, b.wmax);
        }
        return a.tri_count < b.tri_count;
    });
    return FF_OK;
}

}


namespace ff {
size_t bvh_lds_bytes(int lds_nodes, int stack_depth, int block_threads, int num_geoms);
int max_lds_nodes(int stack_depth, int block_threads, int num_geoms, size_t reserve = 0);

namespace {

bool check_bvh(const CompiledScene& cs, int* out_max_leaf)
{
    std::vector<int> seen(cs.tris.size(), 0);
    int max_leaf = 0;
    bool ok = true;
    struct Item {
        int link;
        float mn[3], mx[3];
    };
    for (const GeomRecord& g : cs.geoms) {
        if (g.type != FF_GEOM_TRIANGLEMESH || g.bvh_root < 0) continue;
        std::vector<Item> todo;
        Item root;
        root.link = g.bvh_root;
        for (int k = 0; k < 3; ++k) { root.mn[k] = -std::numeric_limits<float>::infinity(); root.mx[k] = std::numeric_limits<float>::infinity(); }
        todo.push_back(root);
        const bool single_leaf = cs.nodes[g.bvh_root].left < 0 && cs.nodes[g.bvh_root].left == cs.nodes[g.bvh_root].right;
        while (!todo.empty()) {
            const Item it = todo.back();
            todo.pop_back();
            if (it.link >= 0) {
                if (it.link >= (int)cs.nodes.size()) return false;
                const BvhNode& n = cs.nodes[it.link];
                Item l, r;
                l.link = n.left; r.link = n.right;
                for (int k = 0; k < 3; ++k) {
                    l.mn[k] = n.lmin[k]; l.mx[k] = n.lmax[k]; r.mn[k] = n.rmin[k]; r.mx[k] = n.rmax[k];
                    if (n.lmin[k] < it.mn[k] - 1e-3f || n.lmax[k] > it.mx[k] + 1e-3f) ok = false;
                    if (n.rmin[k] < it.mn[k] - 1e-3f || n.rmax[k] > it.mx[k] + 1e-3f) ok = false;
                }
                todo.push_back(l);
                if (!(single_leaf && it.link == g.bvh_root)) todo.push_back(r);
            } else {
                const int ref = ~it.link, first = ref >> 3, count = (ref & 7) + 1;
                max_leaf = std::max(max_leaf, count);
                if (first < g.tri_first || first + count > g.tri_first + g.tri_count) return false;
                for (int i = first; i < first + count; ++i) {
                    ++seen[i];
                    const TriRecord& t = cs.tris[i];
                    const float v1[3] = { t.v0[0] + t.e1[0], t.v0[1] + t.e1[1], t.v0[2] + t.e1[2] };
                    const float v2[3] = { t.v0[0] + t.e2[0], t.v0[1] + t.e2[1], t.v0[2] + t.e2[2] };
                    for (const float* v : { t.v0, v1, v2 })
                        for (int k = 0; k < 3; ++k)
                            if (!(v[k] >= it.mn[k] && v[k] <= it.mx[k])) ok = false;
                }
            }
        }
        std::vector<int> orig(g.tri_count, 0);
        for (int i = g.tri_first; i < g.tri_first + g.tri_count; ++i) {
            const int o = cs.tris[i].orig_index;
            if (o < 0 || o >= g.tri_count) return false;
            ++orig[o];
        }
        for (int c : orig) if (c != 1) ok = false;
    }
    for (int c : seen) if (c != 1) ok = false;
    if (out_max_leaf) *out_max_leaf = max_leaf;
    return ok;
}

}
}

extern "C" int ff_scene_info(const FfGeometry* host_geometries, int n, FfSceneInfo* out)
{
    using namespace ff;
    clear_error();
    if (!out) return fail(FF_ERR_INVALID_ARG, "ff_scene_info: out_info is null");
    std::memset(out, 0, sizeof *out);
    CompiledScene cs;
    const BvhBuildParams bp = default_bvh_params();
    const int st = compile_scene(host_geometries, n, bp, cs);
    if (st != FF_OK) return st;
    out->num_geometries = (int)cs.geoms.size();
    for (const GeomRecord& g : cs.geoms) {
        if (g.type == FF_GEOM_TRIANGLEMESH) ++out->num_meshes;
        else ++out->num_planes;
    }
    out->bvh_nodes = (int)cs.nodes.size();
    out->bvh_max_depth = cs.max_depth;
    out->num_triangles = cs.tris.size();
    const int stack_depth = cs.max_depth + 1;
    out->lds_nodes = std::min((int)cs.nodes.size(), std::max(0, max_lds_nodes(stack_depth, 512, (int)cs.geoms.size())));
    out->lds_bytes = (int)bvh_lds_bytes(out->lds_nodes, stack_depth, 512, (int)cs.geoms.size());
    out->device_bytes = cs.geoms.size() * sizeof(GeomRecord) + cs.tris.size() * sizeof(TriRecord) + cs.nodes.size() * sizeof(BvhNode);
    int max_leaf = 0;
    out->valid = check_bvh(cs, &max_leaf) ? 1 : 0;
    out->bvh_max_leaf = max_leaf;
    double area = 0.0;
    for (const BvhNode& nd : cs.nodes) {
        const float* lo[2] = { nd.lmin, nd.rmin };
        const float* hi[2] = { nd.lmax, nd.rmax };
        for (int c = 0; c < 2; ++c) {
            const double dx = (double)hi[c][0] - lo[c][0], dy = (double)hi[c][1] - lo[c][1], dz = (double)hi[c][2] - lo[c][2];
            if (dx >= 0.0 && dy >= 0.0 && dz >= 0.0) area += dx * dy + dy * dz + dz * dx;
        }
    }
    out->bvh_child_area = (float)area;
    return FF_OK;
}

extern "C" int ff_debug_wall_table(const FfGeometry* host_geometries, int n, float* out_walls7, int max_walls)
{
    using namespace ff;
    clear_error();
    CompiledScene cs;
    const int st = compile_scene(host_geometries, n, default_bvh_params(), cs, false);
    if (st != FF_OK) return -st;
    int num_quads = 0;
    for (const GeomRecord& g : cs.geoms) num_quads += g.type == FF_GEOM_PLANE ? 1 : 0;
    WallTable t;
    build_wall_table(cs.geoms.data(), num_quads, t, std::getenv("FF_NO_WALL_PAIRS") == nullptr);
    int count = 0, i = 0;
    for (int axis = 0; axis < 3; ++axis)
        for (int k = 0; k < t.count[axis]; ++k, ++i) {
            const Wall& w = t.w[i];
            for (int side = 0; side < (w.hi_geom1 ? 2 : 1); ++side) {
                if (out_walls7 && count < max_walls) {
                    float* o = out_walls7 + (size_t)count * 7;
                    o[0] = (float)cs.geoms[side ? w.hi_geom1 - 1 : w.geom].orig_index;
                    o[1] = (float)axis;
                    o[2] = side ? w.hi_c : w.c; o[3] = w.cu; o[4] = w.hu; o[5] = w.cv; o[6] = w.hv;
                }
                ++count;
            }
        }
    return count;
}

extern "C" int ff_debug_wall_entries(const FfGeometry* host_geometries, int n)
{
    using namespace ff;
    clear_error();
    CompiledScene cs;
    const int st = compile_scene(host_geometries, n, default_bvh_params(), cs, false);
    if (st != FF_OK) return -st;
    int num_quads = 0;
    for (const GeomRecord& g : cs.geoms) num_quads += g.type == FF_GEOM_PLANE ? 1 : 0;
    WallTable t;
    build_wall_table(cs.geoms.data(), num_quads, t, std::getenv("FF_NO_WALL_PAIRS") == nullptr);
    return t.count[0] + t.count[1] + t.count[2];
}
```

gpupathtracer_amd/csrc/ff_state.h:

```cpp
#pragma once

#include <vector>

#include <hip/hip_runtime.h>

#include "ff_build.h"
#include "ff_image.h"
#include "ff_internal.h"
#include "ff_kernels.h"
#include "ff_texture.h"

struct FfDistContext;

struct FfState {
    int device = 0;
    int num_cus = 0;
    size_t device_mem_bytes = 0;
    hipStream_t stream = nullptr;
    ff::GeomRecord* d_geoms = nullptr;
    ff::TriRecord* d_tris = nullptr;
    ff::TriNormals* d_normals = nullptr;
    ff::TriUVs* d_uvs = nullptr;
    ff::BvhNode* d_nodes = nullptr;
    ff::WallTable walls = {};
    int num_scan = 0;
    ff::Bvh4Node* d_nodes4 = nullptr;
    int num_geoms = 0, num_planes = 0, num_quads = 0, num_nodes = 0, max_depth = 0;
    int num_nodes4 = 0, max_depth4 = 0;
    int top_count = 0, top_depth = 0, top_lds_count = 0;
    int stack_entries = 1;
    int stack_lds_levels = 1;
    unsigned long long* d_cull_mask = nullptr;
    size_t cull_mask_bytes = 0;
    float4* d_primary_cache = nullptr;
    size_t primary_cache_bytes = 0;
    float4* d_start_records = nullptr;
    size_t start_records_bytes = 0;
    bool primary_has_start = false;
    int start_bounces = 0, start_shade = 0;
    struct PrimaryKey {
        float cam[24];
        int dims[12];
        unsigned pix_items;
    } primary_key = {};
    bool primary_valid = false;
    PrimaryKey last_key = {};
    bool last_key_valid = false;
    bool primary_has_mask = false;
    unsigned long long primary_culled_pixels = 0;
    bool pending_mask_reused = false, pending_mask_built = false;
    float4* d_park = nullptr;
    size_t park_bytes = 0;
    int* d_stack_spill = nullptr;
    size_t stack_spill_bytes = 0;
    bool use_pool = false;
    int scene_block_threads = 0, lds_cap = 0;
    bool has_specular = false;
    uint64_t num_tris = 0;
    bool has_scene = false;
    struct MeshSlot {
        int node_first = 0, node_count = 0, node_capacity = 0, depth = 0;
        int node4_count = 0, depth4 = 0;
        bool parents_linked = false;
    };
    int builder = FF_BUILD_HOST_SAH;
    int scene_builder = FF_BUILD_HOST_SAH;
    std::vector<ff::GeomRecord> h_geoms;
    std::vector<MeshSlot> slots;
    size_t node_capacity = 0;
    int* d_parent = nullptr;
    unsigned char* d_role = nullptr;
    FfTriangle* d_stage = nullptr;
    size_t stage_bytes = 0;
    ff::BuildScratch scratch;
    FfBuildStats build_stats = {};
    float* d_blocksums = nullptr;
    size_t blocksums_bytes = 0;
    unsigned char* d_rgb8 = nullptr;
    size_t rgb8_bytes = 0;
    float* d_radiance = nullptr;
    size_t radiance_bytes = 0;
    float4* d_tail_samples = nullptr;
    size_t tail_samples_bytes = 0;
    bool tail_forced = false;
    int tail_min_blocks = 4;
    int tail_group_spp = 8;
    float* d_accum = nullptr;
    size_t accum_bytes = 0;
    float* d_frame = nullptr;
    size_t frame_bytes = 0;
    float* d_mean = nullptr;
    size_t mean_bytes = 0;
    int accum_width = 0, accum_height = 0, accum_frames = 0;
    float4* d_gb_hits = nullptr;
    size_t gb_hits_bytes = 0;
    void* d_img_stage = nullptr;
    size_t img_stage_bytes = 0;
    float4* d_dn_work = nullptr;
    size_t dn_work_bytes = 0;
    enum { kHistoryTemporal = 0, kHistoryTaa = 1 };
    ff::ReprojectionHistory history[2];
    float jitter_x = 0.f, jitter_y = 0.f;
    FfCameraSampling cam_sampling = { FF_PIXEL_CORNER, 0.f, 1.f, 0 };
    bool cam_active() const { return cam_sampling.pixel_filter == FF_PIXEL_BOX || cam_sampling.lens_radius > 0.f; }
    std::vector<FfGeometry> nee_geoms;
    std::vector<FfBXDF> nee_bxdfs;
    std::vector<std::vector<FfTriangle>> nee_tris;
// ... 133 lines not shown
```

Baseline: 15340 Mrays/s.

## Stage wall and mesh-box tables in LDS instead of kernel arguments

Removes the large WallTable (walls plus mesh boxes) from the kernel parameter struct, keeping only a 32-byte header there. The packed entries are uploaded to a device buffer and staged into LDS at block start next to the geometry records. Wall screening and mesh-box tests now read from LDS, and the pair-test branch uses readfirstlane. This shrinks the kernarg and scalar-load footprint, but it uses extra LDS that the node-cap budgeting now subtracts, which may leave fewer BVH nodes resident in LDS.

```diff
diff --git a/gpupathtracer_amd/csrc/ff_api.cpp b/gpupathtracer_amd/csrc/ff_api.cpp
--- a/gpupathtracer_amd/csrc/ff_api.cpp
+++ b/gpupathtracer_amd/csrc/ff_api.cpp
@@ -20,6 +20,9 @@
 {
     s->primary_valid = s->last_key_valid = false;
     if (s->d_geoms) (void)hipFree(s->d_geoms);
+    if (s->d_wall_tables) (void)hipFree(s->d_wall_tables);
+    s->d_wall_tables = nullptr;
+    s->wall_tables_bytes = 0;
     if (s->d_tris) (void)hipFree(s->d_tris);
     if (s->d_normals) (void)hipFree(s->d_normals);
     if (s->d_uvs) (void)hipFree(s->d_uvs);
@@ -135,13 +138,14 @@
 namespace {
 
 int lds_records(const FfState* s) { return s->num_geoms > kMaxLdsRecords ? 0 : s->num_geoms; }
+size_t lds_table_bytes(const FfState* s) { return (size_t)wall_table_entries(s->walls) * sizeof(Wall); }
 
 int bvh_block_threads(const FfState* s, int preferred, int stack_levels)
 {
     const int sizes[3] = { 1024, 768, 512 };
     for (int b : sizes) {
         if (b > preferred) continue;
-        if (bvh_lds_bytes(0, stack_levels, b, lds_records(s)) + (s->use_pool ? pool_lds_bytes(b) : 0) <= (size_t)kLdsBudgetBytes) return b;
+        if (bvh_lds_bytes(0, stack_levels, b, lds_records(s), wall_table_entries(s->walls)) + (s->use_pool ? pool_lds_bytes(b) : 0) <= (size_t)kLdsBudgetBytes) return b;
     }
     return 0;
 }
@@ -187,17 +191,18 @@
     }
     const int block = s->scene_block_threads > 0 ? s->scene_block_threads : kBlockThreads;
     constexpr int kMinLdsStack = 4;
-    const size_t reserve = s->use_pool ? pool_lds_bytes(block) : 0;
+    const size_t tables = lds_table_bytes(s);
+    const size_t reserve = tables + (s->use_pool ? pool_lds_bytes(block) : 0);
     s->stack_lds_levels = s->stack_entries;
     if (s->use_pool) {
         s->stack_lds_levels = pool_levels;
         while (s->stack_lds_levels < s->stack_entries && max_lds_nodes(s->stack_lds_levels + 1, block, lds_records(s), reserve) >= nodes4) ++s->stack_lds_levels;
     } else if (s->scene_block_threads > 0 && !s->sw.no_stack_spill) {
         const int want = nodes4 + s->top_count;
-        if (want > max_lds_nodes(s->stack_entries, block, lds_records(s))) {
+        if (want > max_lds_nodes(s->stack_entries, block, lds_records(s), tables)) {
             int levels = s->stack_entries;
-            while (levels > kMinLdsStack && max_lds_nodes(levels, block, lds_records(s)) < want) --levels;
-            if (max_lds_nodes(levels, block, lds_records(s)) >= want) s->stack_lds_levels = levels;
+            while (levels > kMinLdsStack && max_lds_nodes(levels, block, lds_records(s), tables) < want) --levels;
+            if (max_lds_nodes(levels, block, lds_records(s), tables) >= want) s->stack_lds_levels = levels;
         }
     }
     int cap = s->scene_block_threads > 0 ? std::max(0, max_lds_nodes(s->stack_lds_levels, block, lds_records(s), reserve)) : 0;
@@ -233,6 +238,14 @@
         next += r.lds_nodes;
     }
     FF_HIP(hipMemcpyAsync(s->d_geoms, s->h_geoms.data(), s->h_geoms.size() * sizeof(GeomRecord), hipMemcpyHostToDevice, s->stream));
+    const int nwalls = s->walls.count[0] + s->walls.count[1] + s->walls.count[2];
+    static_assert(sizeof(Wall) == 32 && sizeof(WallTable::MeshBox) == 32, "one table of 32-byte entries");
+    unsigned char packed[kMaxWallTableBytes];
+    std::memcpy(packed, s->walls.w, (size_t)nwalls * sizeof(Wall));
+    std::memcpy(packed + (size_t)nwalls * sizeof(Wall), s->walls.box, (size_t)s->walls.num_boxes * sizeof(WallTable::MeshBox));
+    const int st = ensure_bytes((void**)&s->d_wall_tables, &s->wall_tables_bytes, kMaxWallTableBytes);
+    if (st != FF_OK) return st;
+    if (tables > 0) FF_HIP(hipMemcpyAsync(s->d_wall_tables, packed, tables, hipMemcpyHostToDevice, s->stream));
     FF_HIP(hipStreamSynchronize(s->stream));
     return FF_OK;
 }
@@ -309,7 +322,7 @@
     k.trinormals = smooth ? reinterpret_cast<const float4*>(s->d_normals) : nullptr;
     k.nodes4 = s->d_nodes4;
     if (s->sw.lds_fill && lds_block_threads > 0) {
-        const size_t bytes = bvh_lds_bytes(s->lds_cap, s->stack_lds_levels, lds_block_threads, lds_records(s));
+        const size_t bytes = bvh_lds_bytes(s->lds_cap, s->stack_lds_levels, lds_block_threads, lds_records(s), wall_table_entries(s->walls));
         k.debug_lds_words = (unsigned)std::min<size_t>(s->sw.lds_fill_words, bytes / 4);
         k.debug_lds_pattern = (unsigned)s->sw.lds_fill_pattern;
     }
@@ -320,7 +333,8 @@
     k.top_lds_first = 0;
     k.top_lds_count = s->top_lds_count;
     k.num_scan = s->num_scan;
-    k.walls = s->walls;
+    k.walls = static_cast<const WallHead&>(s->walls);
+    k.wall_tables = s->d_wall_tables;
 }
 
 int attach_stack_spill(FfState* s, KParams& k, int grid, int block_threads)
@@ -1535,7 +1549,8 @@
     p.top_lds_first = 0;
     p.top_lds_count = s->top_lds_count;
     p.num_scan = s->num_scan;
-    p.walls = s->walls;
+    p.walls = static_cast<const WallHead&>(s->walls);
+    p.wall_tables = s->d_wall_tables;
     p.guard_hits = s->d_counters;
     e = hipMemsetAsync(s->d_counters, 0, sizeof(unsigned long long), s->stream);
     p.lds_nodes = s->lds_cap;
diff --git a/gpupathtracer_amd/csrc/ff_internal.h b/gpupathtracer_amd/csrc/ff_internal.h
--- a/gpupathtracer_amd/csrc/ff_internal.h
+++ b/gpupathtracer_amd/csrc/ff_internal.h
@@ -80,13 +80,16 @@
     float hi_c;
 };
 static_assert(sizeof(Wall) == 32, "32-byte wall");
-struct WallTable {
+struct WallHead {
     int count[3];
     unsigned mask;
     float margin_s;
     float graze;
     int num_boxes;
     int pad;
+};
+static_assert(sizeof(WallHead) == 32, "32-byte table head");
+struct WallTable : WallHead {
     Wall w[kMaxWalls];
     struct MeshBox {
         float mn[3];
@@ -95,6 +98,9 @@
         int pad;
     } box[32];
 };
+static_assert(sizeof(WallTable::MeshBox) == 32, "32-byte mesh box");
+constexpr int wall_table_entries(const WallHead& h) { return h.count[0] + h.count[1] + h.count[2] + h.num_boxes; }
+constexpr int kMaxWallTableBytes = (kMaxWalls + 32) * 32;
 
 void build_wall_table(const struct GeomRecord* geoms, int limit, WallTable& out, bool pairing = true);
 void add_mesh_boxes(const struct GeomRecord* geoms, int first, int n, WallTable& out);
diff --git a/gpupathtracer_amd/csrc/ff_kernels.h b/gpupathtracer_amd/csrc/ff_kernels.h
--- a/gpupathtracer_amd/csrc/ff_kernels.h
+++ b/gpupathtracer_amd/csrc/ff_kernels.h
@@ -66,13 +66,14 @@
     unsigned emitter_mask;
     int cut_last;
     float scene_min[3], scene_max[3];
-    WallTable walls;
     float4* park;
     int pool_quorum, pool_quorum_min, pool_refill, pool_slice, pool_leave, pool_batch_min;
     unsigned* timeline;
     unsigned timeline_ticks;
     float4* start_records;
     int start_bounces;
+    WallHead walls;
+    const uint4* wall_tables;
 };
 constexpr int kRaySlots = 30, kRaySlotFirst = 2, kRaySlotStride = 16;
 constexpr int kAnsweredWord = kRaySlotStride * kRaySlotFirst + 1;
@@ -102,8 +103,9 @@
     int stack_depth;
     int* stack_spill;
     int num_scan;
-    WallTable walls;
     unsigned long long* guard_hits;
+    WallHead walls;
+    const uint4* wall_tables;
 };
 
 constexpr unsigned kNeeKeySelect = 0x6A09E667u;
@@ -133,8 +135,8 @@
 constexpr unsigned kCameraKeyPixel = 0xA54FF53Au;
 constexpr unsigned kCameraKeyLens = 0x510E527Fu;
 
-size_t bvh_lds_bytes(int lds_nodes, int stack_depth, int block_threads, int num_geoms);
-int max_lds_nodes(int stack_depth, int block_threads, int num_geoms, size_t reserve = 0);
+size_t bvh_lds_bytes(int lds_nodes, int stack_depth, int block_threads, int num_geoms, int table_entries);
+int max_lds_nodes(int stack_depth, int block_threads, int num_geoms, size_t reserve);
 size_t pool_lds_bytes(int block_threads);
 
 hipError_t launch_trace(const KParams& p, int trace_mode, bool collect_stats, int grid_blocks, int block_threads, hipStream_t stream,
diff --git a/gpupathtracer_amd/csrc/ff_kernels.hip b/gpupathtracer_amd/csrc/ff_kernels.hip
--- a/gpupathtracer_amd/csrc/ff_kernels.hip
+++ b/gpupathtracer_amd/csrc/ff_kernels.hip
@@ -280,6 +280,7 @@
     int block;
     int stride;
     int geom_base;
+    int wall_base;
     int num_quads;
     const float4* smooth_normals;
     const float4* geoms_g;
@@ -295,7 +296,7 @@
 template <int BIG = 0>
 __device__ __forceinline__ LdsT<BIG> make_lds(int node_cap, int stack_depth, int block, int tid, int num_quads, const float4* smooth_normals = nullptr,
                                               const GeomRecord* geoms = nullptr, int top_first = 0, int top_lds_first = 0, int top_lds_count = 0,
-                                              int num_scan = 0, int* spill = nullptr)
+                                              int num_scan = 0, int* spill = nullptr, int num_geoms = 0)
 {
     LdsT<BIG> L;
     L.spill = spill;
@@ -313,12 +314,13 @@
     L.stack_slot = tid;
     L.stack_depth = stack_depth;
     L.geom_base = node_cap * kNodeVec4 + (stack_depth * block) / 4;
+    L.wall_base = L.geom_base + (LdsT<BIG>::records_lds ? num_geoms * kGeomVec4 : 0);
     return L;
 }
 
 template <class LDS>
 __device__ __forceinline__ void stage_scene(const LDS& L, const uint4* __restrict__ nodes4, const GeomRecord* __restrict__ geoms, int num_geoms,
-                                            int num_planes, int tid, int block)
+                                            int num_planes, int tid, int block, const WallHead& W, const uint4* __restrict__ wall_tables)
 {
     for (int g = num_planes; g < num_geoms; ++g) {
         const int count = geoms[g].lds_nodes;
@@ -341,6 +343,7 @@
         const uint4* gsrc = reinterpret_cast<const uint4*>(geoms);
         for (int i = tid; i < num_geoms * kGeomVec4; i += block) ff_smem[L.geom_base + i] = gsrc[i];
     }
+    for (int i = tid; i < wall_table_entries(W) * 2; i += block) ff_smem[L.wall_base + i] = wall_tables[i];
     __syncthreads();
 }
 
@@ -636,8 +639,18 @@
     best_g = nearer ? g : best_g;
 }
 
-template <bool STATS>
-__device__ __forceinline__ void screen_walls(const WallTable& W, const Ray& wr, const WorldSlab& ws, float wlen, Segment& S, unsigned& slow, Counters& cnt)
+template <class LDS>
+__device__ __forceinline__ Wall lds_wall(const LDS& L, int i)
+{
+    const float4 a = reinterpret_cast<const float4*>(ff_smem)[L.wall_base + 2 * i], b = reinterpret_cast<const float4*>(ff_smem)[L.wall_base + 2 * i + 1];
+    Wall w;
+    w.c = a.x; w.cu = a.y; w.hu = a.z; w.cv = a.w;
+    w.hv = b.x; w.geom = __float_as_int(b.y); w.hi_geom1 = __float_as_int(b.z); w.hi_c = b.w;
+    return w;
+}
+
+template <bool STATS, class LDS>
+__device__ __forceinline__ void screen_walls(const LDS& L, const WallHead& W, const Ray& wr, const WorldSlab& ws, float wlen, Segment& S, unsigned& slow, Counters& cnt)
 {
     const int nx = W.count[0], ny = nx + W.count[1], nz = ny + W.count[2];
     if (nz == 0) return;
@@ -650,14 +663,14 @@
     float best_d = kInf;
     int best_g = -1;
     bool tie = false;
-    Wall cur = W.w[0];
+    Wall cur = lds_wall(L, 0);
     int i = 0;
     {
         const float dl = D * __builtin_fmaf(fmaxf(ay, az), aix, 1.0f), tt = th * aix;
         const bool steep = ax >= gmin;
         for (; i < nx; ++i) {
-            const Wall nxt = W.w[min(i + 1, kMaxWalls - 1)];
-            if (cur.hi_geom1) wall_test_pair(cur, ws.ix, ws.ox, wr.oy, wr.dy, wr.oz, wr.dz, dl, tt, steep, wlen, best_d, best_g, tie, slow);
+            const Wall nxt = lds_wall(L, min(i + 1, nz - 1));
+            if (__builtin_amdgcn_readfirstlane(cur.hi_geom1)) wall_test_pair(cur, ws.ix, ws.ox, wr.oy, wr.dy, wr.oz, wr.dz, dl, tt, steep, wlen, best_d, best_g, tie, slow);
             else wall_test(cur, ws.ix, ws.ox, wr.oy, wr.dy, wr.oz, wr.dz, dl, tt, steep, wlen, best_d, best_g, tie, slow);
             cur = nxt;
         }
@@ -666,8 +679,8 @@
         const float dl = D * __builtin_fmaf(fmaxf(az, ax), aiy, 1.0f), tt = th * aiy;
         const bool steep = ay >= gmin;
         for (; i < ny; ++i) {
-            const Wall nxt = W.w[min(i + 1, kMaxWalls - 1)];
-            if (cur.hi_geom1) wall_test_pair(cur, ws.iy, ws.oy, wr.oz, wr.dz, wr.ox, wr.dx, dl, tt, steep, wlen, best_d, best_g, tie, slow);
+            const Wall nxt = lds_wall(L, min(i + 1, nz - 1));
+            if (__builtin_amdgcn_readfirstlane(cur.hi_geom1)) wall_test_pair(cur, ws.iy, ws.oy, wr.oz, wr.dz, wr.ox, wr.dx, dl, tt, steep, wlen, best_d, best_g, tie, slow);
             else wall_test(cur, ws.iy, ws.oy, wr.oz, wr.dz, wr.ox, wr.dx, dl, tt, steep, wlen, best_d, best_g, tie, slow);
             cur = nxt;
         }
@@ -676,8 +689,8 @@
         const float dl = D * __builtin_fmaf(fmaxf(ax, ay), aiz, 1.0f), tt = th * aiz;
         const bool steep = az >= gmin;
         for (; i < nz; ++i) {
-            const Wall nxt = W.w[min(i + 1, kMaxWalls - 1)];
-            if (cur.hi_geom1) wall_test_pair(cur, ws.iz, ws.oz, wr.ox, wr.dx, wr.oy, wr.dy, dl, tt, steep, wlen, best_d, best_g, tie, slow);
+            const Wall nxt = lds_wall(L, min(i + 1, nz - 1));
+            if (__builtin_amdgcn_readfirstlane(cur.hi_geom1)) wall_test_pair(cur, ws.iz, ws.oz, wr.ox, wr.dx, wr.oy, wr.dy, dl, tt, steep, wlen, best_d, best_g, tie, slow);
             else wall_test(cur, ws.iz, ws.oz, wr.ox, wr.dx, wr.oy, wr.dy, dl, tt, steep, wlen, best_d, best_g, tie, slow);
             cur = nxt;
         }
@@ -697,7 +710,7 @@
 }
 
 template <bool STATS, class LDS>
-__device__ __forceinline__ bool scan_records(const LDS& L, const WallTable& W, const GeomRecord* __restrict__ geoms, int num_geoms, int num_planes,
+__device__ __forceinline__ bool scan_records(const LDS& L, const WallHead& W, const GeomRecord* __restrict__ geoms, int num_geoms, int num_planes,
                                            const TriRecord* __restrict__ tris, const Ray& wr, Segment& S, Counters& cnt, bool cut, unsigned emitters)
 {
     const int prim_end = num_planes;
@@ -707,7 +720,7 @@
     if (STATS) tb0 = __builtin_amdgcn_s_memtime();
     const WorldSlab ws = make_world_slab(wr);
     unsigned quads = 0u;
-    screen_walls<STATS>(W, wr, ws, wlen, S, quads, cnt);
+    screen_walls<STATS>(L, W, wr, ws, wlen, S, quads, cnt);
     for (int g = 0; g < prim_end; ++g) {
         if ((W.mask >> g) & 1u) continue;
         const float4 bmin = lds_geom4(L, g, 14), bmax = lds_geom4(L, g, 15);
@@ -724,15 +737,15 @@
     if (STATS) tb2 = __builtin_amdgcn_s_memtime();
     S.meshes = 0u;
     const float limit = fminf(S.best.dist, S.pend.dist);
-    {
-        typedef unsigned box_words __attribute__((ext_vector_type(8)));
-        static_assert(sizeof(WallTable::MeshBox) == 32, "one box, one load");
-        box_words cur = *reinterpret_cast<const box_words*>(&W.box[0]);
+    if (W.num_boxes > 0) {
+        const float4* box = reinterpret_cast<const float4*>(ff_smem) + L.wall_base + 2 * ((W.count[0] + W.count[1]) + W.count[2]);
+        float4 cmn = box[0], cmx = box[1];
         for (int i = 0; i < W.num_boxes; ++i) {
-            const box_words nxt = *reinterpret_cast<const box_words*>(&W.box[min(i + 1, 31)]);
-            S.meshes |= slab_may_hit(__uint_as_float(cur.s0), __uint_as_float(cur.s1), __uint_as_float(cur.s2), __uint_as_float(cur.s4), __uint_as_float(cur.s5),
-                                     __uint_as_float(cur.s6), ws, limit) ? 1u << cur.s3 : 0u;
-            cur = nxt;
+            const int n = min(i + 1, W.num_boxes - 1);
+            const float4 nmn = box[2 * n], nmx = box[2 * n + 1];
+            S.meshes |= slab_may_hit(cmn.x, cmn.y, cmn.z, cmx.x, cmx.y, cmx.z, ws, limit) ? 1u << __float_as_uint(cmn.w) : 0u;
+            cmn = nmn;
+            cmx = nmx;
         }
     }
     const bool over = cut && (holds(S) & emitters) == 0u;
@@ -749,12 +762,12 @@
 __device__ __forceinline__ void enter_top(const LDS& L, const Ray& wr, Segment& S);
 
 template <bool STATS, class LDS>
-__device__ __forceinline__ void scan_walls(const LDS& L, const WallTable& W, const TriRecord* __restrict__ tris, const Ray& wr, Segment& S, Counters& cnt)
+__device__ __forceinline__ void scan_walls(const LDS& L, const WallHead& W, const TriRecord* __restrict__ tris, const Ray& wr, Segment& S, Counters& cnt)
 {
     const float wlen = __builtin_amdgcn_rcpf(inv_length(wr));
     const WorldSlab ws = make_world_slab(wr);
     unsigned prims = 0u;
-    screen_walls<STATS>(W, wr, ws, wlen, S, prims, cnt);
+    screen_walls<STATS>(L, W, wr, ws, wlen, S, prims, cnt);
     for (int g = 0; g < L.num_scan; ++g) {
         if ((W.mask >> g) & 1u) continue;
         const float4 bmin = lds_geom4(L, g, 14), bmax = lds_geom4(L, g, 15);
@@ -769,7 +782,7 @@
 }
 
 template <bool STATS, class LDS>
-__device__ __forceinline__ bool begin_segment(const LDS& L, const WallTable& W, const GeomRecord* __restrict__ geoms, int num_geoms, int num_planes,
+__device__ __forceinline__ bool begin_segment(const LDS& L, const WallHead& W, const GeomRecord* __restrict__ geoms, int num_geoms, int num_planes,
                                               const TriRecord* __restrict__ tris, const Ray& wr, Segment& S, Counters& cnt, bool cut = false,
                                               unsigned emitters = 0u)
 {
@@ -1156,7 +1169,7 @@
 }
 
 template <bool STATS, class LDS>
-__device__ __forceinline__ void closest_hit_deferred(const LDS& L, const WallTable& W, const GeomRecord* __restrict__ geoms, int num_geoms, int num_planes,
+__device__ __forceinline__ void closest_hit_deferred(const LDS& L, const WallHead& W, const GeomRecord* __restrict__ geoms, int num_geoms, int num_planes,
                                                      const TriRecord* __restrict__ tris, const uint4* __restrict__ nodes4, const Ray& wr,
                                                      Best& best, Counters& cnt)
 {
@@ -1787,13 +1800,13 @@
     const int tid = threadIdx.x;
     const int lane = tid & (kWave - 1);
     const LdsT<BIG> L = make_lds<BIG>(p.lds_nodes, p.stack_depth, BLOCK, tid, EXTRAS ? p.num_quads : 0x7fffffff, EXTRAS ? p.trinormals : nullptr,
-                                      p.geoms, p.top_first, p.top_lds_first, p.top_lds_count, BIG ? p.num_scan : 0, p.stack_spill);
+                                      p.geoms, p.top_first, p.top_lds_first, p.top_lds_count, BIG ? p.num_scan : 0, p.stack_spill, p.num_geoms);
     const uint4* nodes4 = reinterpret_cast<const uint4*>(p.nodes4);
     if (p.debug_lds_words != 0u) {
         for (unsigned i = tid; i < p.debug_lds_words; i += BLOCK) reinterpret_cast<unsigned*>(ff_smem)[i] = p.debug_lds_pattern;
         __syncthreads();
     }
-    stage_scene(L, nodes4, p.geoms, p.num_geoms, p.num_planes, tid, BLOCK);
+    stage_scene(L, nodes4, p.geoms, p.num_geoms, p.num_planes, tid, BLOCK, p.walls, p.wall_tables);
 
     Counters cnt = {};
     Path P;
@@ -2233,14 +2246,14 @@
     const int tid = threadIdx.x;
     const int lane = tid & (kWave - 1);
     const LdsT<0> L = make_lds<0>(p.lds_nodes, p.stack_depth, BLOCK, tid, EXTRAS ? p.num_quads : 0x7fffffff, EXTRAS ? p.trinormals : nullptr, p.geoms, 0, 0, 0,
-                                  0, p.stack_spill);
+                                  0, p.stack_spill, p.num_geoms);
     const uint4* nodes4 = reinterpret_cast<const uint4*>(p.nodes4);
     if (p.debug_lds_words != 0u) {
         for (unsigned i = tid; i < p.debug_lds_words; i += BLOCK) reinterpret_cast<unsigned*>(ff_smem)[i] = p.debug_lds_pattern;
         __syncthreads();
     }
     PoolRef Q;
-    Q.job_base = L.geom_base + p.num_geoms * kGeomVec4;
+    Q.job_base = L.wall_base + wall_table_entries(p.walls) * 2;
     Q.ring_base = (Q.job_base + 3 * BLOCK) * 8;
     Q.ctrl = (Q.job_base + 3 * BLOCK) * 4 + kPoolRing / 2;
     for (int i = tid; i < kPoolRing / 2; i += BLOCK) pool_u32()[Q.ring_base / 2 + i] = 0xFFFFFFFFu;
@@ -2253,7 +2266,7 @@
         ff_smem[Q.ctrl / 4 + 3] = make_uint4((unsigned)p.pool_refill, (unsigned)p.pool_leave, (unsigned)p.pool_quorum, (unsigned)p.lds_nodes | ((unsigned)p.stack_depth << 24));
     }
     ff_smem[Q.job_base + 2 * BLOCK + tid] = make_uint4((unsigned)kDone, 0u, 0u, (unsigned)kPendEmpty);
-    stage_scene(L, nodes4, p.geoms, p.num_geoms, p.num_planes, tid, BLOCK);
+    stage_scene(L, nodes4, p.geoms, p.num_geoms, p.num_planes, tid, BLOCK, p.walls, p.wall_tables);
 
     Counters cnt = {};
     WaveQueue WQ = make_wave_queue(p);
@@ -2575,9 +2588,9 @@
 {
     const int tid = threadIdx.x;
     const LdsT<BIG> L = make_lds<BIG>(p.lds_nodes, p.stack_depth, kBlockThreads, tid, p.num_quads, nullptr, p.geoms, p.top_first, p.top_lds_first,
-                                      p.top_lds_count, BIG ? p.num_scan : 0, p.stack_spill);
+                                      p.top_lds_count, BIG ? p.num_scan : 0, p.stack_spill, p.num_geoms);
     const uint4* nodes4 = reinterpret_cast<const uint4*>(p.nodes4);
-    if (MODE == FF_TRACE_BVH) stage_scene(L, nodes4, p.geoms, p.num_geoms, p.num_planes, tid, kBlockThreads);
+    if (MODE == FF_TRACE_BVH) stage_scene(L, nodes4, p.geoms, p.num_geoms, p.num_planes, tid, kBlockThreads, p.walls, p.wall_tables);
     float4* batch = reinterpret_cast<float4*>(ff_smem);
     const int i = blockIdx.x * kBlockThreads + tid;
     const bool live = i < p.n;
@@ -2844,9 +2857,9 @@
     const int tid = threadIdx.x;
     const int lane = tid & (kWave - 1);
     const LdsT<BIG> L = make_lds<BIG>(p.lds_nodes, p.stack_depth, kBlockThreads, tid, p.num_quads, nullptr, p.geoms, p.top_first, p.top_lds_first,
-                                      p.top_lds_count, BIG ? p.num_scan : 0, p.stack_spill);
+                                      p.top_lds_count, BIG ? p.num_scan : 0, p.stack_spill, p.num_geoms);
     const uint4* nodes4 = reinterpret_cast<const uint4*>(p.nodes4);
-    if (MODE == FF_TRACE_BVH) stage_scene(L, nodes4, p.geoms, p.num_geoms, p.num_planes, tid, kBlockThreads);
+    if (MODE == FF_TRACE_BVH) stage_scene(L, nodes4, p.geoms, p.num_geoms, p.num_planes, tid, kBlockThreads, p.walls, p.wall_tables);
     float4* batch = reinterpret_cast<float4*>(ff_smem);
     constexpr float kInvPi = 0.31830988618379067f;
     Counters cnt = {};
@@ -3166,10 +3179,10 @@
 #endif
 }
 #else
-size_t bvh_lds_bytes(int lds_nodes, int stack_depth, int block_threads, int num_geoms)
+size_t bvh_lds_bytes(int lds_nodes, int stack_depth, int block_threads, int num_geoms, int table_entries)
 {
     return (size_t)lds_nodes * sizeof(Bvh4Node) + (size_t)stack_depth * (size_t)block_threads * sizeof(unsigned) +
-           (size_t)num_geoms * sizeof(GeomRecord);
+           (size_t)num_geoms * sizeof(GeomRecord) + (size_t)table_entries * sizeof(Wall);
 }
 
 int max_lds_nodes(int stack_depth, int block_threads, int num_geoms, size_t reserve)
@@ -3282,7 +3295,7 @@
     if (prepass) {
         const dim3 block(block_threads);
         const int big = p.num_geoms <= kChunkGeometries ? 0 : (p.num_geoms <= kMaxLdsRecords ? 1 : 2);
-        const size_t lds = bvh_lds_bytes(p.lds_nodes, p.stack_depth, block_threads, big == 2 ? 0 : p.num_geoms);
+        const size_t lds = bvh_lds_bytes(p.lds_nodes, p.stack_depth, block_threads, big == 2 ? 0 : p.num_geoms, wall_table_entries(p.walls));
 #define FF_LAUNCH_PRE(B)                                                                                                  \
     do {                                                                                                                  \
         if (big == 0) hipLaunchKernelGGL((trace_bvh_kernel<false, B, true, 0, true>), grid, block, lds, stream, p);      \
@@ -3298,7 +3311,7 @@
     }
     if (trace_mode == FF_TRACE_BVH && pool && p.num_geoms <= kChunkGeometries && block_threads == 1024) {
         const dim3 block(block_threads);
-        const size_t lds = bvh_lds_bytes(p.lds_nodes, p.stack_depth, block_threads, p.num_geoms) + pool_lds_bytes(block_threads);
+        const size_t lds = bvh_lds_bytes(p.lds_nodes, p.stack_depth, block_threads, p.num_geoms, wall_table_entries(p.walls)) + pool_lds_bytes(block_threads);
         const bool extras = p.num_planes > p.num_quads || p.has_specular != 0 || p.trinormals != nullptr;
 #define FF_LAUNCH_POOL(B)                                                                                                 \
     do {                                                                                                                  \
@@ -3315,7 +3328,7 @@
     } else if (trace_mode == FF_TRACE_BVH) {
         const dim3 block(block_threads);
         const int big = p.num_geoms <= kChunkGeometries ? 0 : (p.num_geoms <= kMaxLdsRecords ? 1 : 2);
-        const size_t lds = bvh_lds_bytes(p.lds_nodes, p.stack_depth, block_threads, big == 2 ? 0 : p.num_geoms);
+        const size_t lds = bvh_lds_bytes(p.lds_nodes, p.stack_depth, block_threads, big == 2 ? 0 : p.num_geoms, wall_table_entries(p.walls));
         const bool spheres = p.num_planes > p.num_quads || p.has_specular != 0 || p.trinormals != nullptr;
         if (start && (big != 0 || spheres || p.start_records == nullptr)) return hipErrorInvalidValue;
 #define FF_LAUNCH_BVH(B)                                                                                                  \
@@ -3386,7 +3399,7 @@
 {
     if (p.n <= 0) return hipSuccess;
     const int big = p.num_geoms <= kChunkGeometries ? 0 : (p.num_geoms <= kMaxLdsRecords ? 1 : 2);
-    const size_t lds = trace_mode == FF_TRACE_BVH ? bvh_lds_bytes(p.lds_nodes, p.stack_depth, kBlockThreads, big == 2 ? 0 : p.num_geoms)
+    const size_t lds = trace_mode == FF_TRACE_BVH ? bvh_lds_bytes(p.lds_nodes, p.stack_depth, kBlockThreads, big == 2 ? 0 : p.num_geoms, wall_table_entries(p.walls))
                                                   : (size_t)kBruteBatchTris * sizeof(TriRecord);
     const dim3 grid((p.n + kBlockThreads - 1) / kBlockThreads), block(kBlockThreads);
     if (trace_mode == FF_TRACE_BVH && big == 1) hipLaunchKernelGGL((ray_batch_kernel<FF_TRACE_BVH, 1>), grid, block, lds, stream, p);
@@ -3401,7 +3414,7 @@
     if (np.items == 0u) return hipSuccess;
     const KParams& p = np.k;
     const int big = p.num_geoms <= kChunkGeometries ? 0 : (p.num_geoms <= kMaxLdsRecords ? 1 : 2);
-    const size_t lds = trace_mode == FF_TRACE_BVH ? bvh_lds_bytes(p.lds_nodes, p.stack_depth, kBlockThreads, big == 2 ? 0 : p.num_geoms)
+    const size_t lds = trace_mode == FF_TRACE_BVH ? bvh_lds_bytes(p.lds_nodes, p.stack_depth, kBlockThreads, big == 2 ? 0 : p.num_geoms, wall_table_entries(p.walls))
                                                   : (size_t)kBruteBatchTris * sizeof(TriRecord);
     const dim3 grid(grid_blocks), block(kBlockThreads);
     const char* name;
diff --git a/gpupathtracer_amd/csrc/ff_scene.cpp b/gpupathtracer_amd/csrc/ff_scene.cpp
--- a/gpupathtracer_amd/csrc/ff_scene.cpp
+++ b/gpupathtracer_amd/csrc/ff_scene.cpp
@@ -889,8 +889,8 @@
 
 
 namespace ff {
-size_t bvh_lds_bytes(int lds_nodes, int stack_depth, int block_threads, int num_geoms);
-int max_lds_nodes(int stack_depth, int block_threads, int num_geoms, size_t reserve = 0);
+size_t bvh_lds_bytes(int lds_nodes, int stack_depth, int block_threads, int num_geoms, int table_entries);
+int max_lds_nodes(int stack_depth, int block_threads, int num_geoms, size_t reserve);
 
 namespace {
 
@@ -976,8 +976,8 @@
     out->bvh_max_depth = cs.max_depth;
     out->num_triangles = cs.tris.size();
     const int stack_depth = cs.max_depth + 1;
-    out->lds_nodes = std::min((int)cs.nodes.size(), std::max(0, max_lds_nodes(stack_depth, 512, (int)cs.geoms.size())));
-    out->lds_bytes = (int)bvh_lds_bytes(out->lds_nodes, stack_depth, 512, (int)cs.geoms.size());
+    out->lds_nodes = std::min((int)cs.nodes.size(), std::max(0, max_lds_nodes(stack_depth, 512, (int)cs.geoms.size(), 0)));
+    out->lds_bytes = (int)bvh_lds_bytes(out->lds_nodes, stack_depth, 512, (int)cs.geoms.size(), 0);
     out->device_bytes = cs.geoms.size() * sizeof(GeomRecord) + cs.tris.size() * sizeof(TriRecord) + cs.nodes.size() * sizeof(BvhNode);
     int max_leaf = 0;
     out->valid = check_bvh(cs, &max_leaf) ? 1 : 0;
diff --git a/gpupathtracer_amd/csrc/ff_state.h b/gpupathtracer_amd/csrc/ff_state.h
--- a/gpupathtracer_amd/csrc/ff_state.h
+++ b/gpupathtracer_amd/csrc/ff_state.h
@@ -23,6 +23,8 @@
     ff::TriUVs* d_uvs = nullptr;
     ff::BvhNode* d_nodes = nullptr;
     ff::WallTable walls = {};
+    uint4* d_wall_tables = nullptr;
+    size_t wall_tables_bytes = 0;
     int num_scan = 0;
     ff::Bvh4Node* d_nodes4 = nullptr;
     int num_geoms = 0, num_planes = 0, num_quads = 0, num_nodes = 0, max_depth = 0;
```

Result: no change. 15330 Mrays/s (-0.0%).
